# huyhoang17/DB_text_minimal

Measured on AMD Instinct MI355X. Metric: train images/sec @640x640 bs=16/GPU, higher is better.
Workload: dtype f32

## Files before the change

### db_text_minimal_amd/_lib.py

```python
import ctypes
import os
import subprocess

_HERE = os.path.dirname(os.path.abspath(__file__))
LIB_PATH = os.environ.get('DBN_LIB_PATH') or os.path.join(_HERE, 'libdbnet_hip.so')
CSRC = os.path.join(_HERE, 'csrc')

_P, _I, _L, _F, _D = ctypes.c_void_p, ctypes.c_int, ctypes.c_long, ctypes.c_float, ctypes.c_double

SIGNATURES = {
    'dbn_pack_weights': 'piiiiiipp',
    'dbn_igemm_panel_floats': 'iiiiii',
    'dbn_igemm_packed_floats': 'ii',
    'dbn_igemm_f32': 'pppp' + 'i' * 14 + 'p',
    'dbn_igemm_tile_config': 'ii',
    'dbn_igemm_tile_config_ns': 'iii',
    'dbn_conv_bn_ws_floats': 'iiiiii',
    'dbn_pack_weights_batched': 'piip',
    'dbn_igemm_splitk_plan': 'iiii',
    'dbn_igemm_splitk_plan_ns': 'iiiii',
    'dbn_igemm_splitk_f32': 'pppp' + 'i' * 16 + 'pp',
    'dbn_deform_im2col': 'ppp' + 'i' * 11 + 'p',
    'dbn_deform_col2im': 'ppppp' + 'i' + 'p' + 'i' * 11 + 'p',
    'dbn_deform_col2im_ws_bytes': 'i' * 8,
# ... 17 lines not shown
    'dbn_render_minmax': 'ppilplliifpp',
    'dbn_render_paint': 'ppppilplliifppfp',
    'dbn_minmax_scale_u8': 'piiippp',
    'dbn_words_to_input': 'ipllii' + 'ppp',
    'dbn_greedy_decode_ws_bytes': 'ii',
    'dbn_greedy_decode': 'ip' + 'iii' + 'pi' + 'ppppp',
    'dbn_jpeg_info': 'plp',
    'dbn_jpeg_coef_elems': 'ppip',
    'dbn_jpeg_entropy_batch': 'ppiplpppi',
    'dbn_jpeg_pixels': 'plppipipipplp',
    'dbn_jpeg_info_ex': 'plip',
    'dbn_jpeg_coef_elems_ex': 'ppiip',
    'dbn_jpeg_entropy_batch_ex': 'ppiplppppii',
    'dbn_jpeg_pixels_ex': 'plppipipippipplp',
    'dbn_jpeg_forward': 'plppipipipplp',
    'dbn_jpeg_encode_bound': 'piip',
    'dbn_jpeg_encode_batch': 'plppiiplpppi',
    'dbn_jpeg_optimal_table': 'pppp',
    'dbn_jpeg_encode_batch_opt': 'plppiiplpppii',
    'dbn_jpeg_huff_plan': 'ppilipppp',
    'dbn_jpeg_huff_hist': 'plpiplippp',
    'dbn_jpeg_huff_annex_k': 'pp',
    'dbn_jpeg_huff_tables': 'ppipppi',
    'dbn_jpeg_huff_code': 'plpippllipiplplpp',
    'dbn_jpeg_huff_headers': 'ppiipippp',
    'dbn_jpeg_stream_plan': 'ppipppppplpplp',
    'dbn_jpeg_dhuff_ws_bytes': 'l',
    'dbn_jpeg_dhuff': 'plppppppilliiplplpp',
    'dbn_detect_poly_ws_bytes': 'iiii',
    'dbn_detect_poly_verts_cap': 'iii',
    'dbn_detect_poly': 'piiiifi' + 'pppppp',
    'dbn_detect_poly_host': 'ppppp' + 'iiii' + 'pp' + 'pppi' + 'pppp',
    'dbn_det_eval_ws_bytes': 'i',
    'dbn_det_eval_overlaps': 'ppipilippppp',
    'dbn_det_eval_match_host': 'ii' + 'p' * 12,
    'dbn_pyramid_conv_ws_floats': 'iiii',
    'dbn_pyramid_conv_f32': 'p' * 10 + 'i' * 7 + 'pp' + 'ff' + 'ppppppp' + 'p',
    'dbn_conv_bn_f32': 'pppp' + 'i' * 15 + 'pp' + 'ff' + 'ppppppp' + 'p',
    'dbn_pack_weights_bf16s': 'piiiiiiipp',
    'dbn_igemm_bf16s_panel_floats': 'iiiiiii',
    'dbn_igemm_bf16s': 'pppp' + 'i' * 15 + 'p',
    'dbn_wgrad_bf16s': 'pppp' + 'i' * 12 + 'fip',
    'dbn_wgrad_splitk': 'iiiiiii',
    'dbn_wgrad_slab_floats': 'iiiiiii',
    'dbn_wgrad_splitk_hw': 'iiiiiiiii',
    'dbn_wgrad_slab_floats_hw': 'iiiiiiiiii',
    'dbn_set_index_limits': 'lll',
    'dbn_wgrad_f32': 'pppp' + 'i' * 12 + 'fp',
    'dbn_reduce_ws_floats': 'i',
    'dbn_bn_train_stats': 'piippffppppppp' + 'p',
    'dbn_bn_eval_coef': 'ippppfppp',
    'dbn_bn_apply': 'pppppppliip',
    'dbn_bn_backward': 'pppppppp' + 'pp' + 'i' + 'pp' + 'ii' + 'f' + 'pp',
    'dbn_bn_backward_from_sums': 'ppppppppp' + 'pp' + 'i' + 'pp' + 'ii' + 'f' + 'pp',
    'dbn_bn_backward_ex': 'ppppppppp' + 'pp' + 'i' + 'ppp' + 'ii' + 'f' + 'pp',
    'dbn_col_sum': 'piipfpp',
    'dbn_bnrelu_maxpool_fwd': 'ppppiiiip',
    'dbn_bnrelu_maxpool_bwd': 'ppppppiiiip',
    'dbn_nearest_up_fwd': 'ppp' + 'i' * 8 + 'p',
    'dbn_nearest_up_bwd': 'pp' + 'i' * 9 + 'p',
    'dbn_bilinear_fwd': 'ppliiiip',
    'dbn_bilinear_bwd': 'ppliiiip',
    'dbn_fpn_combine_weights': 'piiiipp',
    'dbn_fpn_scatter_wgrad': 'ppppiipp',
    'dbn_nchw3_to_nhwc4': 'ppiiip',
    'dbn_add_inplace': 'pplp',
    'dbn_head_tail_fwd': 'p' * 11 + 'iiii' + 'f' + 'p',
    'dbn_head_tail_bwd_ws_floats': '',
    'dbn_head_tail_bwd': 'p' * 21 + 'iiii' + 'ff' + 'pp',
    'dbn_db_loss_ws_bytes': '',
    'dbn_db_loss_fwd': 'pp' + 'iiii' + 'ffdf' + 'pppp',
    'dbn_db_loss_sum_fwd': 'pp' + 'iiii' + 'ffdf' + 'pppp',
    'dbn_db_loss_frac_fwd': 'pp' + 'iiii' + 'ffdf' + 'i' + 'pppp',
    'dbn_db_loss_bwd': 'pppp' + 'ff' + 'iiii' + 'pp',
    'dbn_db_loss_ohem_ws_bytes': 'iii',
    'dbn_db_loss_ohem_fwd': 'pp' + 'iiii' + 'ffdf' + 'pppp',
    'dbn_db_loss_ohem_bwd': 'ppppp' + 'ff' + 'iiii' + 'pp',
    'dbn_pixel_confusion': 'plppiiifpp',
    'dbn_adam_step': 'pppp' + 'l' + 'ffff' + 'i' + 'f' + 'p',
    'dbn_clock_probe': 'pip',
    'dbn_has_experiments': '',
    'dbn_wall_clock_khz': '',
}
SIGNATURES.update({
    'dbn_igemm_t': 'ii' + 'pppp' + 'i' * 14 + 'i' + 'p' + 'p',
    'dbn_conv_bn_t': 'i' + SIGNATURES['dbn_conv_bn_f32'],
    'dbn_pyramid_conv_t': 'i' + SIGNATURES['dbn_pyramid_conv_f32'],
    'dbn_pyramid_conv_from_t': 'ii' + SIGNATURES['dbn_pyramid_conv_f32'],
    'dbn_igemm_bn_rows': 'i' * 15,
    'dbn_igemm_bnsums_t': 'ii' + 'pppp' + 'i' * 14 + 'ppppppp' + 'pppp' + 'p' + 'p',
    'dbn_igemm_bn_final_counters': 'ii',
    'dbn_igemm_bn_final_group_floats': 'ii',
    'dbn_wgrad_t': 'ii' + 'pppp' + 'i' * 12 + 'f' + 'p',
    'dbn_wgrad_phase_t': 'iii' + 'pppp' + 'i' * 12 + 'f' + 'p',
    'dbn_wgrad_reduce_describe': 'ii' + 'pppp' + 'i' * 12 + 'f' + 'p',
    'dbn_wgrad_reduce_many': 'ppiiip',
    'dbn_wgrad_tile_config': 'ii',
    'dbn_set_wgrad_variant': 'i',
    'dbn_set_convt_kernel': 'i',
    'dbn_igemm_splitk_slab_floats': 'iiiii',
    'dbn_wgrad_kernel_config': 'iiiii',
    'dbn_wgrad_kernel_config_hw': 'i' * 12,
    'dbn_set_patch_conv': 'i',
    'dbn_set_wres16': 'i',
    'dbn_set_pyramid_wide': 'i',
    'dbn_pyramid_wide_would_run': 'iiiiii',
    'dbn_conv_bn_set_final': 'pp',
    'dbn_conv_bn_final_group_doubles': 'ii',
    'dbn_wres16_would_run': 'iiiiiiiii',
    'dbn_mfma_sustained': 'ippip',
    'dbn_mfma_sustained_flops': 'ii',
    'dbn_set_stagger': 'i',
    'dbn_winograd_eligible': 'iiiii',
    'dbn_winograd_panel_floats': 'ii',
    'dbn_winograd_pack': 'piiiipp',
    'dbn_winograd_rows': 'iii',
    'dbn_winograd_pack_batched': 'pip',
    'dbn_winograd_dgrad_bnsums_f32': 'ppp' + 'iiiiii' + 'pppp' + 'ppp' + 'pppp' + 'p' + 'p',
    'dbn_winograd_ws_floats': 'iiii',
    'dbn_winograd_wgrad_eligible': 'iiiiii',
    'dbn_winograd_wgrad_linear': 'ii',
    'dbn_winograd_wgrad_slab_floats': 'iiiii',
    'dbn_winograd_wgrad_f32': 'ipppppp' + 'iiiiii' + 'fp',
    'dbn_winograd_conv_bn_act_f32': 'pppppp' + 'iiiii' + 'pp' + 'ff' + 'ppppppp' + 'p',
    'dbn_winograd_conv_bn_f32': 'pppp' + 'iiiii' + 'pp' + 'ff' + 'ppppppp' + 'p',
    'dbn_set_phase_priority': 'i',
    'dbn_set_winograd_persistent': 'i',
    'dbn_set_winograd_stagger': 'i',
    'dbn_set_winograd_blocks_per_barrier': 'i',
    'dbn_fold_bn_eval': 'pilppppp' + 'f' + 'ppp',
    'dbn_igemm_act_t': 'ii' + 'pppp' + 'i' + 'p' + 'i' * 13 + 'p',
    'dbn_winograd_conv_act_f32': 'pppp' + 'i' + 'p' + 'iiiii' + 'p',
    'dbn_pyramid_conv_act_t': 'ii' + 'p' * 9 + 'i' + 'p' + 'i' * 6 + 'p',
    'dbn_set_trace': 'pl',
    'dbn_igemm_kernel_config': 'i' * 16,
    'dbn_split3': 'pplp',
    'dbn_deform_im2col_t': 'i' + SIGNATURES['dbn_deform_im2col'],
    'dbn_deform_col2im_t': 'i' + SIGNATURES['dbn_deform_col2im'],
    'dbn_deform_col2im_gather_t': 'i' + SIGNATURES['dbn_deform_col2im'],
    'dbn_deform_col2im_gather_ws_bytes': 'iii',
    'dbn_deform_offset_absmax_t': 'iplpp',
    'dbn_pw16_eligible': 'iiiiii',
    'dbn_pw16_panel_bytes': '',
    'dbn_pw16_pack': 'ipipp',
    'dbn_pw16_act_t': 'ipppipiiiip',
    'dbn_set_head_tail_wide': 'i',
    'dbn_stem16_pool_eligible': 'iiii',
    'dbn_stem16_conv_bn_relu_pool_t': 'ipppppiiip',
    'dbn_head16_eligible': 'iiii',
    'dbn_head16_tail_eval_t': 'i' + 'p' * 15 + 'iii' + 'p',
    'dbn_cast_f32': 'ipplp',
    'dbn_pack_weights_t': 'ip' + 'i' * 7 + 'pp',
    'dbn_igemm_panel_floats_t': 'i' * 8,
    'dbn_bn_train_stats_t': 'i' + SIGNATURES['dbn_bn_train_stats'],
    'dbn_bn_apply_t': 'i' + SIGNATURES['dbn_bn_apply'],
    'dbn_bn_backward_t': 'ipi' + SIGNATURES['dbn_bn_backward_ex'][1:],
    'dbn_col_sum_t': 'i' + SIGNATURES['dbn_col_sum'],
    'dbn_bnrelu_maxpool_fwd_t': 'i' + SIGNATURES['dbn_bnrelu_maxpool_fwd'],
    'dbn_bnrelu_maxpool_bwd_t': 'i' + SIGNATURES['dbn_bnrelu_maxpool_bwd'][:-1] + 'pppp',
    'dbn_maxpool_bwd_parts': 'iiii',
    'dbn_bnrelu_maxpool_fwd_arg_t': 'ipppppp' + 'iiii' + 'p',
    'dbn_maxpool_bn_backward_ws_floats': 'iiii',
    'dbn_maxpool_bn_backward_t': 'i' + 'p' * 10 + 'iiii' + 'f' + 'pp',
    'dbn_nearest_up_fwd_t': 'i' + SIGNATURES['dbn_nearest_up_fwd'],
    'dbn_nearest_up_bwd_t': 'i' + SIGNATURES['dbn_nearest_up_bwd'],
    'dbn_nchw3_to_nhwc4_t': 'i' + SIGNATURES['dbn_nchw3_to_nhwc4'],
    'dbn_nchw3_to_nhwc4_packed_t': 'i' + SIGNATURES['dbn_nchw3_to_nhwc4'],
    'dbn_nchw3_to_nhwc16_and_4_t': 'ipppiiip',
    'dbn_convt16_rows': '',
    'dbn_convt16_panel_bytes': '',
    'dbn_convt16_eligible': 'iiiiii',
    'dbn_convt16_pack': 'ippp',
    'dbn_convt16_bn_t': 'ippppiii' + 'pp' + 'ff' + 'ppppppp' + 'p',
    'dbn_stem16_padded_h': 'i',
    'dbn_stem16_padded_w': 'i',
    'dbn_stem16_rows': '',
    'dbn_stem16_panel_bytes': '',
    'dbn_stem16_eligible': 'iiii',
    'dbn_stem16_pack': 'ippp',
    'dbn_nchw3_to_padded4_t': 'ipppiiip',
    'dbn_stem16_conv_bn_t': 'ipppiii' + 'pp' + 'ff' + 'ppppppp' + 'p',
    'dbn_head_tail_fwd_t': 'i' + SIGNATURES['dbn_head_tail_fwd'],
    'dbn_head_tail_bwd_t': 'i' + SIGNATURES['dbn_head_tail_bwd'],
    'dbn_head_tail_bn_bwd_ws_floats': '',
    'dbn_head_tail_bn_bwd_t': 'ii' + 'p' * 28 + 'iiii' + 'ff' + 'pp',
})
LONG_RETURN = {'dbn_jpeg_coef_elems', 'dbn_jpeg_coef_elems_ex', 'dbn_jpeg_dhuff_ws_bytes', 'dbn_jpeg_encode_bound', 'dbn_greedy_decode_ws_bytes', 'dbn_det_eval_ws_bytes', 'dbn_detect_ws_bytes', 'dbn_detect_poly_ws_bytes', 'dbn_detect_poly_verts_cap', 'dbn_mfma_sustained_flops', 'dbn_conv_bn_final_group_doubles', 'dbn_maxpool_bn_backward_ws_floats', 'dbn_pw16_panel_bytes', 'dbn_stem16_panel_bytes', 'dbn_convt16_panel_bytes', 'dbn_winograd_panel_floats', 'dbn_winograd_wgrad_slab_floats', 'dbn_winograd_ws_floats', 'dbn_igemm_splitk_slab_floats', 'dbn_deform_col2im_ws_bytes', 'dbn_deform_col2im_gather_ws_bytes', 'dbn_igemm_bn_final_counters', 'dbn_igemm_bn_final_group_floats', 'dbn_igemm_panel_floats_t', 'dbn_wgrad_slab_floats_hw', 'dbn_wgrad_slab_floats', 'dbn_igemm_panel_floats', 'dbn_igemm_bf16s_panel_floats', 'dbn_db_loss_ohem_ws_bytes', 'dbn_conv_bn_ws_floats', 'dbn_pyramid_conv_ws_floats'}
_KIND = {'p': _P, 'i': _I, 'l': _L, 'f': _F, 'd': _D}


class HipLibraryError(RuntimeError):
    pass


class WgradReduceJob(ctypes.Structure):
    _fields_ = ([('slab', _P), ('grad', _P)] + [(f, _I) for f in ('splitk', 'O', 'J', 'Jp', 'BM', 'BN', 'Cb', 'I', 'RS', 'G', 'natural', 'blocks')]
                + [('scale', _F), ('smem_bytes', _I)])


class PackJob(ctypes.Structure):
    _fields_ = [('w', _P), ('out', _P)] + [(f, _I) for f in ('O', 'I', 'R', 'S', 'mode', 'Cs', 'Cd', 'f')]


class WinogradPackJob(ctypes.Structure):
    _fields_ = [('w', _P), ('out', _P)] + [(f, _I) for f in ('O', 'I', 'Cs', 'dgrad')]


class BnbFinal(ctypes.Structure):
    _fields_ = [('counters', _P), ('group', _P), ('c1c2', _P), ('dgamma', _P), ('dbeta', _P), ('c1c2_2', _P), ('dgamma_2', _P),
                ('dbeta_2', _P), ('grad_scale', _F)]


def build(verbose=False):
    res = subprocess.run(['make', '-C', CSRC, '-j8'], capture_output=True, text=True)
    if verbose or res.returncode != 0:
        print(res.stdout[-4000:])
        print(res.stderr[-4000:])
    if res.returncode != 0:
        raise HipLibraryError('building libdbnet_hip.so failed (see output above)')
    return LIB_PATH


def source_stamp():
    import hashlib
    h = hashlib.sha256()
    for name in sorted(os.listdir(CSRC)):
        if name.endswith(('.hip', '.h')) or name == 'Makefile':
            h.update(name.encode())
            with open(os.path.join(CSRC, name), 'rb') as f:
                h.update(f.read())
    return h.hexdigest()[:16]


_lib = None


def lib():
    global _lib
    if _lib is None:
        if not os.path.exists(LIB_PATH):
            raise HipLibraryError('%s not found: run `python -c "import __graft_entry__ as g; g.build()"` '
                                  '(there is no CPU fallback for the DBNet hot path)' % LIB_PATH)
        try:
            l = ctypes.CDLL(LIB_PATH)
        except OSError as e:
            raise HipLibraryError('cannot load %s: %s' % (LIB_PATH, e))
        for name, sig in SIGNATURES.items():
            fn = getattr(l, name)
            fn.argtypes = [_KIND[k] for k in sig]
            fn.restype = _L if name in LONG_RETURN else _I
        _lib = l
    return _lib


def check(rc, what=''):
    if rc != 0:
        if rc == 1:
            raise RuntimeError('libdbnet_hip: invalid argument in %s' % what)
        raise RuntimeError('libdbnet_hip: %s failed with hipError %d' % (what, rc - 1000))
```

### db_text_minimal_amd/csrc/conv.hip

```cpp
#include "igemm_common.h"
#include "../../include/dbnet_hip.h"

long dbn_g_pixel_limit = 1L << 24;
long dbn_g_byte_limit = 0xF0000000L;
long dbn_g_elem_limit = 1L << 32;

namespace {

__device__ __forceinline__ double block_sum_d(double v, double* red) {
    v = dbn_wave_sum_d(v);
    __syncthreads();
    if ((threadIdx.x & 63) == 0) red[threadIdx.x >> 6] = v;
    __syncthreads();
    double t = 0.0;
    for (int w = 0; w < (int)(blockDim.x >> 6); ++w) t += red[w];
    return t;
}

__global__ void bn_finalize_tiles_kernel(const float* __restrict__ stats, int rows, int C, const float* __restrict__ gamma,
                                         const float* __restrict__ beta, float eps, float momentum, float* __restrict__ run_mean,
                                         float* __restrict__ run_var, float* __restrict__ scale, float* __restrict__ shift,
                                         float* __restrict__ mean_out, float* __restrict__ rstd_out) {
    __shared__ double red[16];
    const int c = blockIdx.x;
// ... 68 lines not shown
int dbn_has_experiments(void) { return DBN_HAS_EXPERIMENTS; }


static int tile_config_for(int M, int Cd, int ns) {
    const int bm[4] = {128, 256, 128, 64}, bn[4] = {128, 64, 64, 64};
    static const int r2_env = dbn_env_int("DBN_TILE_EFF_R2", 1);
    const int r2_eff = ns == 0 ? r2_env : 0;
    const double eff_r1[4] = {0.89, 0.83, 0.80, 0.72}, eff_r2[4] = {0.89, 0.85, 0.845, 0.83}, eff_r3[4] = {0.80, 0.76, 0.86, 0.93};
    const double* eff = r2_eff == 2 ? eff_r3 : r2_eff ? eff_r2 : eff_r1;
    int best = 4;
    double best_t = 1e300;
    for (int c = 0; c < 4; ++c) {
        if (Cd % bn[c]) continue;
        const long blocks = (long)dbn_ceil_div(M, bm[c]) * (Cd / bn[c]);
        const long per_cu = (blocks + 255) / 256;
        double t = (double)per_cu * bm[c] * bn[c] / eff[c];
        if (blocks < 512) t *= 1.0 + 0.25 * (512 - blocks) / 512.0;
        if (t < best_t) {
            best_t = t;
            best = c + 1;
        }
    }
    return best;
}
int dbn_igemm_tile_config(int M, int Cd) { return tile_config_for(M, Cd, 0); }
int dbn_igemm_tile_config_ns(int M, int Cd, int ns) { return tile_config_for(M, Cd, ns); }

static int g_convt_enabled = 1;
int dbn_set_convt_kernel(int on) {
    const int old = g_convt_enabled;
    g_convt_enabled = on != 0;
    return old;
}
static bool convt_eligible(int mode, int ns, int at, int tile_hint, int R, int S, int stride, int pad, int Hs, int Ws, int Hd, int Wd, int Cs,
                           int Cd, int accumulate, int ksplit) {
    return g_convt_enabled && mode == 1 && ns == 0 && at == 0 && tile_hint == 0 && R == 2 && S == 2 && stride == 2 && pad == 0 && Hd == 2 * Hs &&
           Wd == 2 * Ws && (Cs == 16 || Cs == 32 || Cs == 48 || Cs == 64) && Cd % 64 == 0 && !accumulate && ksplit <= 1;
}

static bool convt_launch_ok(int n, int Hd, int Wd, int Cd) { return (long)n * Hd * Wd * Cd * 4 < (1L << 32); }

unsigned long long* dbn_g_trace = nullptr;
long dbn_g_trace_blocks = 0;
int dbn_set_trace(void* buf, long max_blocks) {
    dbn_g_trace = reinterpret_cast<unsigned long long*>(buf);
    dbn_g_trace_blocks = max_blocks;
    return DBN_TRACE;
}
int dbn_g_phase_prio = 0;
int dbn_set_phase_priority(int on) {
    const int old = dbn_g_phase_prio;
    dbn_g_phase_prio = on != 0;
    return old;
}
int dbn_g_stagger = 0;
int dbn_set_stagger(int permille) {
    const int old = dbn_g_stagger;
    dbn_g_stagger = permille < 0 ? 0 : permille;
    return old;
}

static bool patch_eligible_fwd(int mode, int at, int H, int W, int Cs);
int dbn_g_wres16 = getenv("DBN_WRES16") ? atoi(getenv("DBN_WRES16")) : 1;
int dbn_set_wres16(int on) {
    const int old = dbn_g_wres16;
    dbn_g_wres16 = on < 0 ? 0 : on > 2 ? 2 : on;
    return old;
}
int dbn_wres16_would_run(int at, int mode, int N, int H, int W, int Cs, int Cd, int bnb, int y2) {
    return patch_eligible_fwd(mode, at, H, W, Cs) && Cd % 64 == 0 && dbn_wres16_eligible(at, mode, N, H, W, Cs, Cd, bnb != 0, y2 != 0, false);
}
static int g_patch_enabled = 1;
static const int g_patch_bn64 = dbn_env_int("DBN_PATCH_BN64", 1);
int dbn_set_patch_conv(int on) {
    const int old = g_patch_enabled;
    g_patch_enabled = (on == 2 || on == 3) ? on : (on != 0);
    return old;
}
static bool patch_eligible(int kmode, int ns, int at, int cfg, int R, int S, int stride, int pad, int Hs, int Ws, int Hd, int Wd, int Cs,
                           int ksplit, int tile_hint = 0) {
    const bool geom = (kmode == 0 || kmode == 1) && R == 3 && S == 3 && stride == 1 && pad == 1 && Hs == Hd && Ws == Wd && Hd % 8 == 0 &&
                      Wd % 16 == 0 && Cs % 32 == 0 && ksplit <= 1;
    if (ns == 0) return (g_patch_enabled == 1 || g_patch_enabled == 3) && at == 0 && geom && (tile_hint == 3 || (tile_hint == 0 && g_patch_enabled == 3));
    return g_patch_enabled && ns > 0 && at != 3 && (cfg == 1 || cfg == 3) && geom;
}
static bool patch_eligible_fwd(int mode, int at, int H, int W, int Cs) {
    return patch_eligible(mode, 1, at, 3, 3, 3, 1, 1, H, W, H, W, Cs, 1, 0);
}
static int patch_cfg(int cfg, int ns = 1) { return (ns == 0 || (cfg == 1 && g_patch_bn64)) ? 3 : cfg; }

static int resolve_cfg(int M_total, int Cd, int tile_hint, int at = 0, int ns = 0, int mode = 0, int R = 0, int S = 0, int stride = 1,
                       int pad = 0, int Hs = 0, int Ws = 0, int Hd = 0, int Wd = 0, int Cs = 0, int ksplit = 1) {
    int cfg = tile_hint > 0 ? tile_hint : tile_config_for(M_total, Cd, ns);
    if (cfg == 1 && Cd % 128 != 0) cfg = 3;
    if (tile_hint == 0 && !(mode == 1 && stride > 1) && Cd % 64 == 0 && patch_eligible(mode, ns, at, 3, R, S, stride, pad, Hs, Ws, Hd, Wd, Cs, ksplit))
        cfg = 3;
    return cfg;
}

int dbn_igemm_kernel_config(int at, int ns, int kmode, int N, int Hs, int Ws, int Cs, int Hd, int Wd, int Cd, int R, int S, int stride,
                            int pad, int tile_hint, int ksplit) {
    const int cfg = resolve_cfg(N * Hd * Wd, Cd, tile_hint, at, ns, kmode >= 2 ? 1 : kmode, R, S, kmode == 2 && stride == 1 ? 2 : stride, pad, Hs,
                                Ws, Hd, Wd, Cs, ksplit);
    if (Cd % 64 == 0 && patch_eligible(kmode, ns, at, cfg, R, S, stride, pad, Hs, Ws, Hd, Wd, Cs, ksplit, tile_hint)) {
        const int wres = (ns == 1 && patch_cfg(cfg, ns) == 3 && dbn_wres16_eligible(at, kmode, N, Hd, Wd, Cs, Cd, false, false, false)) ? 64 : 0;
        return patch_cfg(cfg, ns) + 16 + wres;
    }
    if (kmode == 2 && convt_eligible(1, ns, at, tile_hint, R, S, stride, pad, Hs, Ws, Hd, Wd, Cs, Cd, 0, ksplit)) return cfg + 32;
    return cfg;
}

static int igemm_dispatch(IgemmParams& p, int kmode, int ns, int tile_hint, hipStream_t st, int at = 0) {
    int cfg = tile_hint > 0 ? tile_hint : tile_config_for(p.N * p.Hdf * p.Wdf, p.Cd, ns);
    if (cfg == 1 && p.Cd % 128 != 0) cfg = 3;
    p.patch = p.Cd % 64 == 0 && patch_eligible(kmode, ns, at, cfg, p.R, p.S, p.stride, p.pad, p.Hs, p.Ws, p.Hdf, p.Wdf, p.Cs, p.ksplit, tile_hint);
    if (p.patch) cfg = patch_cfg(cfg, ns);
    return launch_igemm(p, cfg, kmode, ns, st, at);
}

static inline int dst_esize(int at) { return (at == 0 || at == 3) ? 4 : 2; }
static inline int src_planes(int at) { return at == 3 ? 3 : 1; }

struct BnFin {
    int* cnt;
    double* grp;
    const float *gamma, *beta;
    float eps, momentum;
    float *run_mean, *run_var, *scale, *shift, *mean, *rstd;
};
static thread_local int* g_bnf_cnt = nullptr;
static thread_local double* g_bnf_grp = nullptr;
int dbn_conv_bn_set_final(int* counters, double* group) {
    g_bnf_cnt = counters;
    g_bnf_grp = counters ? group : nullptr;
    return (counters && !group) ? DBN_ERR_ARG : DBN_OK;
}
long dbn_conv_bn_final_group_doubles(int rows, int Cd) { return 4L * Cd * ((rows + 63) / 64); }

struct IgemmBnb {
    const void *y, *zmask;
    const float *msc, *msh, *mean, *rstd;
    float* part;
    const void* y2;
    const float *mean2, *rstd2;
    float* part2;
    const dbn_bnb_final* fin;
    int M_total;
};

static int igemm_run_one(const void* src, const float* wpk, const float* bias, void* dst, int N, int Hs, int Ws, int Cs, int Hd,
                         int Wd, int Cd, int R, int S, int stride, int pad, int mode, int accumulate, int cfg, int ns,
                         hipStream_t st, float* stats, int stat_rows, int stat_row0, int ksplit, float* slab, int* rows_out, int at,
                         long plane_bytes, const IgemmBnb* bnb = nullptr, int tile_hint = -1, const void* res = nullptr, int relu = 0,
                         const BnFin* bnf = nullptr) {
    IgemmParams p{};
    if (bnf) {
        p.bnf_cnt = bnf->cnt; p.bnf_grp = bnf->grp; p.bnf_gamma = bnf->gamma; p.bnf_beta = bnf->beta; p.bnf_eps = bnf->eps;
        p.bnf_momentum = bnf->momentum; p.bnf_run_mean = bnf->run_mean; p.bnf_run_var = bnf->run_var; p.bnf_scale = bnf->scale;
        p.bnf_shift = bnf->shift; p.bnf_mean = bnf->mean; p.bnf_rstd = bnf->rstd;
    }
    p.res = res; p.relu = relu;
    p.bnb_y = bnb ? bnb->y : nullptr; p.bnb_zmask = bnb ? bnb->zmask : nullptr;
    p.bnb_msc = bnb ? bnb->msc : nullptr; p.bnb_msh = bnb ? bnb->msh : nullptr;
    p.bnb_mean = bnb ? bnb->mean : nullptr; p.bnb_rstd = bnb ? bnb->rstd : nullptr;
    p.bnb_part = bnb ? bnb->part : nullptr;
    p.bnb_y2 = bnb ? bnb->y2 : nullptr; p.bnb_mean2 = bnb ? bnb->mean2 : nullptr; p.bnb_rstd2 = bnb ? bnb->rstd2 : nullptr;
    p.bnb_part2 = bnb ? bnb->part2 : nullptr;
    p.bnb_cnt = nullptr; p.bnb_grp = nullptr; p.bnb_gscale = 1.f; p.bnb_invM = 0.f;
    for (int b_ = 0; b_ < 2; ++b_) p.bnb_c1c2[b_] = p.bnb_dgamma[b_] = p.bnb_dbeta[b_] = nullptr;
    if (bnb && bnb->fin) {
        const dbn_bnb_final* f = bnb->fin;
        p.bnb_cnt = f->counters; p.bnb_grp = f->group; p.bnb_gscale = f->grad_scale; p.bnb_invM = 1.0f / (float)bnb->M_total;
        p.bnb_c1c2[0] = f->c1c2; p.bnb_dgamma[0] = f->dgamma; p.bnb_dbeta[0] = f->dbeta;
        p.bnb_c1c2[1] = f->c1c2_2; p.bnb_dgamma[1] = f->dgamma_2; p.bnb_dbeta[1] = f->dbeta_2;
    }
    p.src = src; p.wpk = wpk; p.bias = bias; p.dst = dst;
    p.N = N; p.Hs = Hs; p.Ws = Ws; p.Cs = Cs; p.Cd = Cd; p.Hdf = Hd; p.Wdf = Wd;
    p.R = R; p.S = S; p.stride = stride; p.pad = pad; p.accumulate = res ? 1 : accumulate;
    p.stats = stats; p.stat_rows = stat_rows; p.stat_row0 = stat_row0; p.launch_rows = 0;
    p.ksplit = 1; p.kt_per = 0;
    p.plane_bytes = (unsigned)plane_bytes;
    p.src_bytes = (unsigned)((long)N * Hs * Ws * Cs * dbn_esize(at) + (src_planes(at) - 1) * plane_bytes);
    if (!(mode == 1 && stride > 1)) {
        p.ncls = 1;
        if (ksplit <= 1) {
            const int rc = igemm_dispatch(p, mode, ns, cfg, st, at);
            *rows_out = p.launch_rows;
            return rc;
        }
        const int KT = (R * S * Cs + 15) / 16;
        DBN_REQUIRE(slab && !stats && !bnb && Cs % 16 == 0 && ksplit <= KT && ksplit <= 64);
        p.kt_per = dbn_ceil_div(KT, ksplit);
        p.ksplit = dbn_ceil_div(KT, p.kt_per);
        p.dst = slab; p.bias = nullptr; p.accumulate = 0;
        const int rc = igemm_dispatch(p, mode, ns, cfg, st, at);
        *rows_out = p.launch_rows;
        if (rc) return rc;
        const long total4 = (long)N * Hd * Wd * Cd / 4;
        DBN_DISPATCH_AT(at == 3 ? 0 : at, hipLaunchKernelGGL(splitk_sum_kernel<AT>, dim3(dbn_grid(total4)), dim3(256), 0, st, slab, p.ksplit,
                                                             total4, Cd, bias, accumulate, dst));
        return dbn_status();
    }
    DBN_REQUIRE(ksplit <= 1);
    p.ncls = stride * stride;
    long off = 0;
    int covered = 0;
    for (int c = 0; c < p.ncls; ++c) {
        const IgemmClass q = class_geom(c, stride, R, S, pad, N, Hd, Wd, Cs);
        p.wpk_off[c] = (int)off;
        if (q.K > 0 && q.M > 0) ++covered;
        off += panel_floats(q.K, Cd, ns);
    }
    DBN_REQUIRE(off < (1L << 31));
    DBN_REQUIRE(covered == p.ncls || !bias);
    DBN_REQUIRE(covered == p.ncls || !bnb);
    if (covered < p.ncls && !accumulate) {
        if (hipMemsetAsync(dst, 0, (size_t)N * Hd * Wd * Cd * dst_esize(at), st) != hipSuccess) return dbn_status();
        p.accumulate = 1;
    }
    *rows_out = 0;
    if (covered == 0) return DBN_OK;
    if (!bnb && convt_eligible(mode, ns, at, tile_hint, R, S, stride, pad, Hs, Ws, Hd, Wd, Cs, Cd, accumulate, ksplit) &&
        convt_launch_ok(N, Hd, Wd, Cd)) {
        const int rc = dbn_launch_convt_f32(p, st);
        *rows_out = p.launch_rows;
        return rc;
    }
    const int rc = igemm_dispatch(p, 2, ns, cfg, st, at);
    *rows_out = p.launch_rows;
    return rc;
}

static int bn_tile_rows_one(int n, int Hd, int Wd, int mode, int stride, int cfg) {
    const int bm_of[5] = {0, 128, 256, 128, 64};
    if (!(mode == 1 && stride > 1)) return dbn_ceil_div((long)n * Hd * Wd, bm_of[cfg]);
    int rows = 0;
    for (int c = 0; c < stride * stride; ++c) {
        const int ph = c / stride, pw = c % stride;
        const int Hc = ph < Hd ? (Hd - ph + stride - 1) / stride : 0, Wc = pw < Wd ? (Wd - pw + stride - 1) / stride : 0;
        if (Hc > 0 && Wc > 0) rows += dbn_ceil_div((long)n * Hc * Wc, bm_of[cfg]);
    }
    return rows;
}

static int igemm_run(const void* src, const float* wpk, const float* bias, void* dst, int N, int Hs, int Ws, int Cs, int Hd,
                     int Wd, int Cd, int R, int S, int stride, int pad, int mode, int accumulate, int tile_hint, int ns,
                     void* stream, float* stats = nullptr, int ksplit = 1, float* slab = nullptr, int stat_rows_total = 0, int at = 0,
                     const IgemmBnb* bnb = nullptr, const void* res = nullptr, int relu = 0, const BnFin* bnf = nullptr) {
    DBN_REQUIRE((!res && !relu) || (ksplit <= 1 && !stats && !bnb && !(mode == 1 && stride > 1)));
    DBN_REQUIRE(src && wpk && dst && (ns == 0 || ns == 1 || ns == 3));
    DBN_REQUIRE(at == 0 || ((at == 1 || at == 2) && ns == 1 && Cs % 16 == 0) || (at == 3 && ns == 3 && Cs % 16 == 0));
    DBN_REQUIRE(N > 0 && Hs > 0 && Ws > 0 && Hd > 0 && Wd > 0 && R > 0 && S > 0 && pad >= 0);
    DBN_REQUIRE(Cs % 4 == 0 && Cd % 64 == 0 && (mode == 0 || mode == 1));
    DBN_REQUIRE(stride == 1 || stride == 2 || stride == 4 || stride == 8 || (mode == 0 && stride >= 1));
    DBN_REQUIRE(tile_hint >= 0 && tile_hint <= 4);
    hipStream_t st = (hipStream_t)stream;
    const int es = dbn_esize(at), des = dst_esize(at);
    const long plane_bytes = at == 3 ? (long)N * Hs * Ws * Cs * 2 : 0;
    DBN_REQUIRE(3 * plane_bytes < dbn_g_byte_limit);
    const int nmax = chunk_images(N, (long)Hd * Wd, (long)Hs * Ws * Cs * es, (long)Hd * Wd * Cd);
    DBN_REQUIRE(nmax >= 1);
    DBN_REQUIRE(nmax >= N || ksplit <= 1);
    const int cfg = resolve_cfg((int)std::min<long>((long)N * Hd * Wd, 0x7FFFFFFF), Cd, tile_hint, at, ns, mode, R, S, stride, pad, Hs, Ws,
                                Hd, Wd, Cs, ksplit);
    int row0 = 0;
    for (int n0 = 0; n0 < N; n0 += nmax) {
        const int n = std::min(nmax, N - n0);
        int rows = 0;
        IgemmBnb b;
        if (bnb) {
            b = *bnb;
            b.y = reinterpret_cast<const char*>(bnb->y) + (long)n0 * Hd * Wd * Cd * des;
            if (bnb->zmask) b.zmask = reinterpret_cast<const char*>(bnb->zmask) + (long)n0 * Hd * Wd * Cd * des;
            if (bnb->y2) b.y2 = reinterpret_cast<const char*>(bnb->y2) + (long)n0 * Hd * Wd * Cd * des;
        }
        const int rc = igemm_run_one(reinterpret_cast<const char*>(src) + (long)n0 * Hs * Ws * Cs * es, wpk, bias,
                                     reinterpret_cast<char*>(dst) + (long)n0 * Hd * Wd * Cd * des, n, Hs, Ws, Cs, Hd, Wd, Cd, R, S, stride,
                                     pad, mode, accumulate, cfg, ns, st, stats, stat_rows_total, row0, ksplit, slab, &rows, at, plane_bytes,
                                     bnb ? &b : nullptr, tile_hint,
                                     res ? reinterpret_cast<const char*>(res) + (long)n0 * Hd * Wd * Cd * des : nullptr, relu, bnf);
        if (rc) return rc;
        row0 += rows;
    }
    return DBN_OK;
}

int dbn_igemm_t(int at, int ns, const void* src, const float* wpk, const float* bias, void* dst, int N, int Hs, int Ws, int Cs, int Hd,
                int Wd, int Cd, int R, int S, int stride, int pad, int mode, int accumulate, int tile_hint, int ksplit, float* slab,
                void* stream) {
    return igemm_run(src, wpk, bias, dst, N, Hs, Ws, Cs, Hd, Wd, Cd, R, S, stride, pad, mode, accumulate, tile_hint, ns, stream, nullptr,
                     ksplit < 1 ? 1 : ksplit, slab, 0, at);
}

int dbn_igemm_act_t(int at, int ns, const void* src, const float* wpk, const float* bias, const void* res, int relu, void* dst, int N,
                    int Hs, int Ws, int Cs, int Hd, int Wd, int Cd, int R, int S, int stride, int pad, int mode, int tile_hint,
                    void* stream) {
    return igemm_run(src, wpk, bias, dst, N, Hs, Ws, Cs, Hd, Wd, Cd, R, S, stride, pad, mode, 0, tile_hint, ns, stream, nullptr, 1, nullptr, 0,
                     at, nullptr, res, relu ? 1 : 0);
}

int dbn_igemm_f32(const float* src, const float* wpk, const float* bias, float* dst, int N, int Hs, int Ws, int Cs, int Hd,
                  int Wd, int Cd, int R, int S, int stride, int pad, int mode, int accumulate, int tile_hint, void* stream) {
    return igemm_run(src, wpk, bias, dst, N, Hs, Ws, Cs, Hd, Wd, Cd, R, S, stride, pad, mode, accumulate, tile_hint, 0, stream);
}

static int bn_tile_rows(int N, int Hs, int Ws, int Cs, int Hd, int Wd, int Cd, int mode, int stride, int tile_hint, int at, int ns, int R,
                        int S, int pad, bool conv_bn = false, int accumulate = 0) {
    const int nmax = chunk_images(N, (long)Hd * Wd, (long)Hs * Ws * Cs * dbn_esize(at), (long)Hd * Wd * Cd);
    if (nmax < 1) return 0;
    const bool convt = conv_bn && convt_eligible(mode, ns, at, tile_hint, R, S, stride, pad, Hs, Ws, Hd, Wd, Cs, Cd, accumulate, 1);
    const int cfg = resolve_cfg((int)std::min<long>((long)N * Hd * Wd, 0x7FFFFFFF), Cd, tile_hint, at, ns, mode, R, S, stride, pad, Hs, Ws,
                                Hd, Wd, Cs, 1);
    int rows = 0;
    for (int n0 = 0; n0 < N; n0 += nmax) {
        const int n = std::min(nmax, N - n0);
        rows += (convt && convt_launch_ok(n, Hd, Wd, Cd)) ? dbn_convt_f32_rows(n * Hs * Ws) : bn_tile_rows_one(n, Hd, Wd, mode, stride, cfg);
    }
    return rows;
}

int dbn_igemm_bn_rows(int at, int ns, int N, int Hs, int Ws, int Cs, int Hd, int Wd, int Cd, int R, int S, int stride, int pad, int mode,
                      int tile_hint) {
    return bn_tile_rows(N, Hs, Ws, Cs, Hd, Wd, Cd, mode, stride, tile_hint, at, ns, R, S, pad);
}

int dbn_igemm_bnsums_t(int at, int ns, const void* src, const float* wpk, const float* bias, void* dst, int N, int Hs, int Ws, int Cs, int Hd,
                       int Wd, int Cd, int R, int S, int stride, int pad, int mode, int accumulate, int tile_hint, const void* y,
                       const void* zmask, const float* mask_scale, const float* mask_shift, const float* save_mean,
                       const float* save_rstd, float* part, const void* y2, const float* save_mean2, const float* save_rstd2,
                       float* part2, const dbn_bnb_final* fin, void* stream) {
    DBN_REQUIRE(((at == 0 && (ns == 0 || ns == 1 || ns == 3)) || (at == 1 && ns == 1)) && y && save_mean && save_rstd && part &&
                (zmask || (mask_scale && mask_shift)));
    DBN_REQUIRE(!y2 || (zmask && save_mean2 && save_rstd2 && part2));
    DBN_REQUIRE(!fin || (fin->counters && fin->group && fin->c1c2 && fin->dgamma && fin->dbeta &&
                         (!y2 || (fin->c1c2_2 && fin->dgamma_2 && fin->dbeta_2))));
    const int rows = bn_tile_rows(N, Hs, Ws, Cs, Hd, Wd, Cd, mode, stride, tile_hint, at, ns, R, S, pad);
    DBN_REQUIRE(rows > 0);
    const IgemmBnb b{y, zmask, mask_scale, mask_shift, save_mean, save_rstd, part, y2, save_mean2, save_rstd2, part2, fin, N * Hd * Wd};
    return igemm_run(src, wpk, bias, dst, N, Hs, Ws, Cs, Hd, Wd, Cd, R, S, stride, pad, mode, accumulate, tile_hint, ns, stream, nullptr, 1,
                     nullptr, rows, at, &b);
}

long dbn_igemm_bn_final_counters(int rows, int Cd) { return (long)(Cd / 64) * ((rows + 63) / 64 + 1); }
long dbn_igemm_bn_final_group_floats(int rows, int Cd) { return 4L * Cd * ((rows + 63) / 64); }

long dbn_conv_bn_ws_floats(int N, int Hd, int Wd, int Cd, int mode, int stride) {
    long worst = 0;
    for (int t = 1; t <= 4; ++t) {
        const long r = (long)N * bn_tile_rows_one(1, Hd, Wd, mode, stride, t);
        worst = r > worst ? r : worst;
    }
    return (3L * Cd + 1) * worst;
}

int dbn_conv_bn_t(int at, const void* src, const float* wpk, const float* bias, void* dst, int N, int Hs, int Ws, int Cs, int Hd, int Wd,
                  int Cd, int R, int S, int stride, int pad, int mode, int accumulate, int tile_hint, int ns,
                  const float* gamma, const float* beta, float eps, float momentum, float* run_mean, float* run_var,
                  float* scale, float* shift, float* save_mean, float* save_rstd, float* ws, void* stream) {
    DBN_REQUIRE(gamma && beta && scale && shift && save_mean && save_rstd && ws);
    const int rows = bn_tile_rows(N, Hs, Ws, Cs, Hd, Wd, Cd, mode, stride, tile_hint, at, ns, R, S, pad, true, accumulate);
    DBN_REQUIRE(rows > 0);
    int* const fcnt = g_bnf_cnt;
    double* const fgrp = g_bnf_grp;
    g_bnf_cnt = nullptr;
    g_bnf_grp = nullptr;
    const bool fin = fcnt && !convt_eligible(mode, ns, at, tile_hint, R, S, stride, pad, Hs, Ws, Hd, Wd, Cs, Cd, accumulate, 1);
    const BnFin f{fcnt, fgrp, gamma, beta, eps, momentum, run_mean, run_var, scale, shift, save_mean, save_rstd};
    const int rc = igemm_run(src, wpk, bias, dst, N, Hs, Ws, Cs, Hd, Wd, Cd, R, S, stride, pad, mode, accumulate, tile_hint, ns, stream, ws,
                             1, nullptr, rows, at, nullptr, nullptr, 0, fin ? &f : nullptr);
    if (rc || fin) return rc;
    hipLaunchKernelGGL(bn_finalize_tiles_kernel, dim3(Cd), dim3(rows >= 2048 ? 1024 : 256), 0, (hipStream_t)stream, ws, rows, Cd, gamma,
                       beta, eps, momentum, run_mean, run_var, scale, shift, save_mean, save_rstd);
    return dbn_status();
}

int dbn_winograd_eligible(int N, int H, int W, int Cs, int Cd) {
    if (!(N > 0 && H > 0 && W > 0 && Cs > 0 && Cs % 16 == 0 && Cd > 0 && Cd % 64 == 0)) return 0;
    const long Hp = (H + 7) / 8 * 8, Wp = (W + 15) / 16 * 16;
    const long tiles = (long)((H + 1) / 2) * ((W + 1) / 2);
    const bool pays = dbn_winograd_linear(H, W) ? 5 * tiles >= 3 * ((tiles + 31) / 32 * 32) : 4L * H * W >= 3L * Hp * Wp;
    return pays && (long)N * H * W * std::max(Cs, Cd) * 4 < dbn_g_byte_limit && (long)N * Hp * Wp < dbn_g_pixel_limit;
}
long dbn_winograd_panel_floats(int O, int Cs) { return (long)Cs * 16 * O; }
int dbn_winograd_pack(const float* w_oihw, int O, int I, int Cs, int dgrad, float* out, void* stream) {
    DBN_REQUIRE(w_oihw && out && O > 0 && I > 0 && I <= Cs && Cs % 16 == 0 && O % 64 == 0 && (dgrad == 0 || dgrad == 1));
    return dbn_launch_winograd_pack(w_oihw, O, I, Cs, dgrad, out, (hipStream_t)stream);
}
int dbn_winograd_pack_batched(const void* jobs, int n, void* stream) {
    DBN_REQUIRE(jobs && n > 0);
    return dbn_launch_winograd_pack_many(jobs, n, (hipStream_t)stream);
}
long dbn_winograd_ws_floats(int N, int H, int W, int Cd) { return (3L * Cd + 1) * dbn_winograd_rows(N, H, W); }
int dbn_winograd_conv_bn_act_f32(const float* src, const float* in_scale, const float* in_shift, const float* upanel, const float* bias,
                                 float* dst, int N, int H, int W, int Cs, int Cd, const float* gamma, const float* beta, float eps,
                                 float momentum, float* run_mean, float* run_var, float* scale, float* shift, float* save_mean,
                                 float* save_rstd, float* ws, void* stream) {
    DBN_REQUIRE(src && upanel && dst && dbn_winograd_eligible(N, H, W, Cs, Cd) && !in_scale == !in_shift);
    DBN_REQUIRE(!gamma || (beta && scale && shift && save_mean && save_rstd && ws));
    IgemmParams p{};
    p.in_scale = in_scale; p.in_shift = in_shift;
    p.src = src; p.wpk = upanel; p.bias = bias; p.dst = dst;
    p.N = N; p.Hs = H; p.Ws = W; p.Cs = Cs; p.Cd = Cd; p.Hdf = H; p.Wdf = W; p.R = 3; p.S = 3; p.stride = 1; p.pad = 1;
    p.src_bytes = (unsigned)((long)N * H * W * Cs * 4);
    const int rows = dbn_winograd_rows(N, H, W);
    p.stats = gamma ? ws : nullptr; p.stat_rows = rows; p.stat_row0 = 0;
    int* const fcnt = g_bnf_cnt;
    double* const fgrp = g_bnf_grp;
    g_bnf_cnt = nullptr;
    g_bnf_grp = nullptr;
    const bool fin = gamma && fcnt;
    if (fin) {
        p.bnf_cnt = fcnt; p.bnf_grp = fgrp; p.bnf_gamma = gamma; p.bnf_beta = beta; p.bnf_eps = eps; p.bnf_momentum = momentum;
        p.bnf_run_mean = run_mean; p.bnf_run_var = run_var; p.bnf_scale = scale; p.bnf_shift = shift; p.bnf_mean = save_mean; p.bnf_rstd = save_rstd;
    }
    const int rc = dbn_launch_winograd_f32(p, (hipStream_t)stream);
    if (rc || !gamma || fin) return rc;
    hipLaunchKernelGGL(bn_finalize_tiles_kernel, dim3(Cd), dim3(rows >= 2048 ? 1024 : 256), 0, (hipStream_t)stream, ws, rows, Cd, gamma,
                       beta, eps, momentum, run_mean, run_var, scale, shift, save_mean, save_rstd);
    return dbn_status();
}

int dbn_winograd_conv_act_f32(const float* src, const float* upanel, const float* bias, const float* res, int relu, float* dst, int N,
                              int H, int W, int Cs, int Cd, void* stream) {
    DBN_REQUIRE(src && upanel && dst && dbn_winograd_eligible(N, H, W, Cs, Cd));
    IgemmParams p{};
    p.src = src; p.wpk = upanel; p.bias = bias; p.dst = dst; p.res = res; p.relu = relu ? 1 : 0; p.accumulate = res ? 1 : 0;
    p.N = N; p.Hs = H; p.Ws = W; p.Cs = Cs; p.Cd = Cd; p.Hdf = H; p.Wdf = W; p.R = 3; p.S = 3; p.stride = 1; p.pad = 1;
    p.src_bytes = (unsigned)((long)N * H * W * Cs * 4);
    p.stat_rows = dbn_winograd_rows(N, H, W);
    return dbn_launch_winograd_f32(p, (hipStream_t)stream);
}

int dbn_winograd_conv_bn_f32(const float* src, const float* upanel, const float* bias, float* dst, int N, int H, int W, int Cs, int Cd,
// ... 196 lines not shown
```

### db_text_minimal_amd/csrc/igemm_common.h

```cpp
#pragma once
#include "common.h"
#include <type_traits>
#include <utility>
#include <stdlib.h>
#include <algorithm>

struct IgemmClass {
    int Hd, Wd;
    int M, K, KT;
    int R, S;
    int pad_h, pad_w;
    int oh0, ow0;
};

constexpr int MAX_CLASSES = 64;

__host__ __device__ inline int taps_of_class(int R, int ph, int f) { return ph < R ? (R - ph + f - 1) / f : 0; }

__host__ __device__ inline IgemmClass class_geom(int c, int f, int R, int S, int pad, int N, int Hdf, int Wdf, int Cs) {
    IgemmClass q;
    const int ph = c / f, pw = c - ph * f;
    q.R = taps_of_class(R, ph, f);
    q.S = taps_of_class(S, pw, f);
    q.oh0 = (((ph - pad) % f) + f) % f;
    q.ow0 = (((pw - pad) % f) + f) % f;
    q.Hd = q.oh0 < Hdf ? (Hdf - q.oh0 + f - 1) / f : 0;
    q.Wd = q.ow0 < Wdf ? (Wdf - q.ow0 + f - 1) / f : 0;
    q.pad_h = (q.oh0 + pad - ph) / f;
    q.pad_w = (q.ow0 + pad - pw) / f;
    q.M = N * q.Hd * q.Wd;
    q.K = q.R * q.S * Cs;
    q.KT = (q.K + 15) / 16;
    return q;
}

struct IgemmParams {
    const void* src;
    const float* wpk;
    const float* bias;
    void* dst;
    int N, Hs, Ws, Cs, Cd, Hdf, Wdf, R, S, stride, pad, accumulate, ncls;
    const float *in_scale, *in_shift;
    const void* res;
    int relu;
    int work_items;
    int* work;
    unsigned long long wino_m_ntn, wino_m_tpi, wino_m_tw;
    int wino_tpi, wino_tw;
    int stat_rows;
    int stat_row0;
    float* stats;
    const void* bnb_y;
    const void* bnb_zmask;
    const float *bnb_msc, *bnb_msh, *bnb_mean, *bnb_rstd;
    float* bnb_part;
    const void* bnb_y2;
    const float *bnb_mean2, *bnb_rstd2;
    float* bnb_part2;
    int* bnb_cnt;
    float* bnb_grp;
    float *bnb_c1c2[2], *bnb_dgamma[2], *bnb_dbeta[2];
    float bnb_gscale, bnb_invM;
    int* bnf_cnt;
    double* bnf_grp;
    const float *bnf_gamma, *bnf_beta;
    float bnf_eps, bnf_momentum;
    float *bnf_run_mean, *bnf_run_var, *bnf_scale, *bnf_shift, *bnf_mean, *bnf_rstd;
    unsigned src_bytes;
    unsigned plane_bytes;
    int tile_end[MAX_CLASSES], row_base[MAX_CLASSES], wpk_off[MAX_CLASSES];
    int ksplit, kt_per;
    int stagger_units, stagger_blocks;
    int phase_prio;
    unsigned long long* trace;
    int launch_rows;
    int patch;
    const void* seg_src[4];
    const float* seg_wpk[4];
    unsigned seg_bytes[4];
    unsigned seg_plane_bytes[4];
    int first_level;
    int pyr_group;
};

extern "C" int dbn_g_stagger;
extern "C" int dbn_g_phase_prio;
extern "C" unsigned long long* dbn_g_trace;
extern "C" long dbn_g_trace_blocks;
#ifndef DBN_TRACE
#define DBN_TRACE 0
#endif
#if DBN_TRACE
#define DBN_TRACE_MARK(i)                                                                                      \
    do {                                                                                                       \
        if (p.trace && threadIdx.x == 0) p.trace[(long)blockIdx.x * 8 + (i)] = __builtin_amdgcn_s_memrealtime(); \
    } while (0)
#else
#define DBN_TRACE_MARK(i) ((void)0)
#endif

namespace {

constexpr unsigned OOB_OFFSET = 0xF8000000u;

__device__ __forceinline__ f32x4 buffer_load_f32x4(__amdgpu_buffer_rsrc_t rsrc, unsigned byte_off) {
    typedef unsigned u32x4 __attribute__((ext_vector_type(4)));
    const u32x4 v = __builtin_amdgcn_raw_buffer_load_b128(rsrc, (int)byte_off, 0, 0);
    return __builtin_bit_cast(f32x4, v);
}

__device__ __forceinline__ void divmod24(int p, int d, float rd, int& q, int& r) {
    q = (int)((float)p * rd);
    r = p - q * d;
    if (r < 0) {
        r += d;
        --q;
    } else if (r >= d) {
        r -= d;
        ++q;
    }
}


typedef __bf16 bf16x8 __attribute__((ext_vector_type(8)));
typedef unsigned u32x2 __attribute__((ext_vector_type(2)));

__device__ __forceinline__ unsigned bf16_bits_rne(float x) {
    unsigned u = __builtin_bit_cast(unsigned, x);
    u += 0x7FFFu + ((u >> 16) & 1u);
    return u >> 16;
}
__device__ __forceinline__ float bf16_bits_to_f32(unsigned b) { return __builtin_bit_cast(float, b << 16); }

typedef __bf16 bf16x2 __attribute__((ext_vector_type(2)));
template <int NS>
__device__ __forceinline__ void split4(const f32x4 v, u32x2 (&out)[NS > 0 ? NS : 1]) {
    float r[4] = {v[0], v[1], v[2], v[3]};
#pragma unroll
    for (int s = 0; s < NS; ++s) {
        const bf16x2 lo = {(__bf16)r[0], (__bf16)r[1]};
        const bf16x2 hi = {(__bf16)r[2], (__bf16)r[3]};
        const unsigned ulo = __builtin_bit_cast(unsigned, lo), uhi = __builtin_bit_cast(unsigned, hi);
        out[s] = u32x2{ulo, uhi};
        if (s + 1 < NS) {
            r[0] -= __builtin_bit_cast(float, ulo << 16);
            r[1] -= __builtin_bit_cast(float, ulo & 0xFFFF0000u);
            r[2] -= __builtin_bit_cast(float, uhi << 16);
            r[3] -= __builtin_bit_cast(float, uhi & 0xFFFF0000u);
        }
    }
}

typedef _Float16 f16x8 __attribute__((ext_vector_type(8)));
template <int NS, int MI, int NI, int F16 = 0>
__device__ __forceinline__ void mfma_split(const bf16x8 (&af)[NS > 0 ? NS : 1][MI], const bf16x8 (&bf)[NS > 0 ? NS : 1][NI],
                                           f32x16 (&acc)[MI][NI]) {
    if constexpr (F16) {
#pragma unroll
        for (int a = 0; a < MI; ++a)
#pragma unroll
            for (int b = 0; b < NI; ++b)
                acc[a][b] = __builtin_amdgcn_mfma_f32_32x32x16_f16(__builtin_bit_cast(f16x8, af[0][a]), __builtin_bit_cast(f16x8, bf[0][b]),
                                                                   acc[a][b], 0, 0, 0);
        return;
    }
    constexpr int NPROD = NS == 3 ? 6 : 1;
    constexpr int pi[6] = {2, 0, 1, 1, 0, 0};
    constexpr int pj[6] = {0, 2, 1, 0, 1, 0};
#pragma unroll
    for (int t = 0; t < NPROD; ++t) {
        const int i = NS == 3 ? pi[t] : 0, j = NS == 3 ? pj[t] : 0;
#pragma unroll
        for (int a = 0; a < MI; ++a)
#pragma unroll
            for (int b = 0; b < NI; ++b) acc[a][b] = __builtin_amdgcn_mfma_f32_32x32x16_bf16(af[i][a], bf[j][b], acc[a][b], 0, 0, 0);
    }
}

struct BnStatFinal {
    float* stats;
    int stat_rows, Cd;
    int* bnf_cnt;
    double* bnf_grp;
    const float *bnf_gamma, *bnf_beta;
    float bnf_eps, bnf_momentum;
    float *bnf_run_mean, *bnf_run_var, *bnf_scale, *bnf_shift, *bnf_mean, *bnf_rstd;
};
#define DBN_BNF_ARGS(p)                                                                                                              \
    BnStatFinal {                                                                                                                    \
        (p).stats, (p).stat_rows, (p).Cd, (p).bnf_cnt, (p).bnf_grp, (p).bnf_gamma, (p).bnf_beta, (p).bnf_eps, (p).bnf_momentum,        \
            (p).bnf_run_mean, (p).bnf_run_var, (p).bnf_scale, (p).bnf_shift, (p).bnf_mean, (p).bnf_rstd                                \
    }
__device__ __forceinline__ void dbn_stat_put(bool fin, float* ptr, float v) {
    if (fin) __hip_atomic_store(ptr, v, __ATOMIC_RELAXED, __HIP_MEMORY_SCOPE_AGENT);
    else *ptr = v;
}
__device__ __forceinline__ void dbn_bn_stats_finish(const BnStatFinal p, int trow, int nt, int n0, int BN, int* s_flag, double* sd) {
    if (!p.bnf_cnt) return;
    constexpr int G = 64;
    const int rows = p.stat_rows, NG = (rows + G - 1) / G, g = trow / G;
    const int tid = threadIdx.x, NT = blockDim.x, parts = NT / BN;
    const int cl = tid % BN, part = tid / BN;
    const long c = n0 + cl;
    int* const cnt = p.bnf_cnt + nt * (NG + 1);
    auto xld = [](const float* q) { return (double)__hip_atomic_load(q, __ATOMIC_RELAXED, __HIP_MEMORY_SCOPE_AGENT); };
    auto xldd = [](const double* q) { return __hip_atomic_load(q, __ATOMIC_RELAXED, __HIP_MEMORY_SCOPE_AGENT); };
    auto xstd = [](double* q, double v) { __hip_atomic_store(q, v, __ATOMIC_RELAXED, __HIP_MEMORY_SCOPE_AGENT); };
    auto combine = [&](double& n, double& a1, double& a2) {
        __syncthreads();
        sd[tid] = n;
        sd[NT + tid] = a1;
        sd[2 * NT + tid] = a2;
        __syncthreads();
        if (part == 0)
            for (int q = 1; q < parts; ++q) {
                n += sd[q * BN + cl];
                a1 += sd[NT + q * BN + cl];
                a2 += sd[2 * NT + q * BN + cl];
            }
    };
    asm volatile("s_waitcnt vmcnt(0)" ::: "memory");
    __syncthreads();
    DBN_RACE_JITTER();
    if (tid == 0) {
        const int gsize = min(G, rows - g * G);
        const int last = __hip_atomic_fetch_add(cnt + 1 + g, 1, __ATOMIC_RELAXED, __HIP_MEMORY_SCOPE_AGENT) == gsize - 1;
        if (last) __hip_atomic_store(cnt + 1 + g, 0, __ATOMIC_RELAXED, __HIP_MEMORY_SCOPE_AGENT);
        *s_flag = last;
    }
// ... 135 lines not shown
```

### db_text_minimal_amd/csrc/igemm_kernel.h

```cpp
#pragma once
#include "igemm_common.h"

#ifndef DBN_DBG
#define DBN_DBG 0
#endif

namespace {

#define DBN_IGEMM_OCC(BM, BN, NS, MODE, PATCH, EPI, AT) \
    __attribute__((amdgpu_waves_per_eu(((MODE) == 3 && (BN) == 256) ? 2 : ((PATCH) && (NS) == 3 && (BN) == 64) ? 2 : ((EPI) == 1 && (NS) == 0 && (BM) * (BN) == 16384) ? 3 : \
                                       ((EPI) == 1 && (AT) == 1 && (PATCH) && (BN) == 64) ? 4 : \
                                       ((EPI) == 0 && (NS) == 0 && (AT) == 0 && (BM) * (BN) == 4096 && (MODE) < 2) ? 7 : 1, 8)))

template <int BM, int BN, int WM, int WN, int MODE, int NS, int AT = 0, bool PATCH = false, int EPI = 0, bool BLK = true>
__global__ __launch_bounds__(WM* WN * 64) DBN_IGEMM_OCC(BM, BN, NS, MODE, PATCH, EPI, AT) void igemm_f32_kernel(const IgemmParams p) {
    static_assert(EPI == 0 || ((AT == 0 || AT == 1) && MODE < 3), "BatchNorm-backward sums: fp32 or bf16 storage, no pyramid form");
    static_assert(BLK || (AT == 0 && MODE == 0 && !PATCH && EPI == 0), "non-blocked K walk: forward conv on fp32 tensors");
    static_assert(AT == 0 || ((AT == 1 || AT == 2) && NS == 1) || (AT == 3 && NS == 3), "storage type / matrix math combination");
    static_assert(!PATCH || (BM == 128 && WM == 2 && WN == 2 && MODE < 2 && (NS > 0 || AT == 0) && AT != 3), "patch form");
    constexpr int NT = WM * WN * 64;
    constexpr int TM = BM / WM, TN = BN / WN;
    constexpr int MI = TM / 32, NI = TN / 32;
    constexpr int ES = AT == 0 ? 4 : 2;
    constexpr bool DST_F32 = AT == 0 || AT == 3;
#ifndef DBN_BUFST
#define DBN_BUFST 1
#endif
    constexpr bool BUFST = DBN_BUFST && DST_F32 && MODE < 2;
    constexpr int NP = AT == 3 ? 3 : 1;
    constexpr int A_SH = AT == 0 ? 2 : 1;
    constexpr int A_CH = AT == 0 ? 4 : 8;
    constexpr int A_PIECES = (BM << A_SH) * NP;
    constexpr int A_LD = (A_PIECES + NT - 1) / NT;
    constexpr bool A_FULL = A_PIECES % NT == 0;
    constexpr int AS = NS == 0 ? BM + 2 : BM + 4, BS = NS == 0 ? BN + 2 : BN + 4;
    constexpr int A_IMG = NS == 0 ? 4 * AS : NS * 2 * AS, B_IMG = NS == 0 ? 4 * BS : NS * 2 * BS;
    constexpr int B_PIECES = NS == 0 ? 4 * BN : NS * 2 * BN;
    constexpr int B_LD = (B_PIECES + NT - 1) / NT;
    constexpr bool B_FULL = B_PIECES % NT == 0;
    constexpr int KU = 1;
#ifndef DBN_DIRECTB
#define DBN_DIRECTB 1
#endif
#ifndef DBN_DIRECTB_NS
#define DBN_DIRECTB_NS 1
#endif
    constexpr bool DIRECTB = DBN_DIRECTB && (NS == 0 || DBN_DIRECTB_NS) && AT == 0 && !PATCH;
    constexpr int NF = NS == 0 ? 2 : NS;
    constexpr int UNIT = A_IMG + (DIRECTB ? 0 : B_IMG);
    constexpr int STAGE = KU * UNIT;
    constexpr int NSX = NS > 0 ? NS : 1;
    static_assert(A_LD >= 1 && B_LD >= 1, "tile too small for the workgroup");
    constexpr int DMA_SU = 2;
#ifndef DBN_DBG16
#define DBN_DBG16 0
#endif
#ifndef DBN_DIRECTB16
#define DBN_DIRECTB16 1
#endif
#ifndef DBN_DIRECTB16_PYR
#define DBN_DIRECTB16_PYR 1
#endif
    constexpr bool DB16 = DBN_DIRECTB16 && AT != 0 && AT != 3 && (MODE != 3 || DBN_DIRECTB16_PYR) && !PATCH;
    constexpr int DMA_UNIT = NP * 2 * BM + (DB16 ? 0 : NSX * 2 * BN);
    constexpr int DMA_STAGE = DMA_SU * DMA_UNIT;
#ifndef DBN_PYR_NSTG
#define DBN_PYR_NSTG 4
#endif
#ifndef DBN_PYR_NSTG_WIDE
#define DBN_PYR_NSTG_WIDE 4
#endif
    constexpr int DMA_NSTG = (DB16 && MODE == 3 && BN == 256 && DMA_STAGE * 16 * DBN_PYR_NSTG_WIDE <= 64 * 1024) ? DBN_PYR_NSTG_WIDE :
                             (DB16 && MODE == 3 && DMA_STAGE * 16 * DBN_PYR_NSTG <= 48 * 1024) ? DBN_PYR_NSTG :
                             DMA_STAGE * 16 * 4 <= 64 * 1024 ? 4 : DMA_STAGE * 16 * 3 <= 160 * 1024 ? 3 : 2;
    constexpr int P_PATCH = NSX * 4 * 180;
    constexpr int P_BUNIT = NSX * 2 * BN, P_BSTAGE = 2 * P_BUNIT;
#ifndef DBN_P_NSTG
#define DBN_P_NSTG 4
#endif
    constexpr int P_NSTG = NSX == 1 ? DBN_P_NSTG : 3;
    constexpr int P_NBUF = NSX == 1 ? 2 : 1;
#ifndef DBN_DIRECTBP
#define DBN_DIRECTBP 1
#endif
#ifndef DBN_DBP_NS1
#define DBN_DBP_NS1 0
#endif
    constexpr bool DBP = DBN_DIRECTBP && PATCH && (NS == 3 || (DBN_DBP_NS1 && NS == 1));
    constexpr int LOOP_SMEM = PATCH ? P_NBUF * P_PATCH + ((DBP || NS == 0) ? 0 : P_NSTG * P_BSTAGE) : AT != 0 ? DMA_NSTG * DMA_STAGE : 2 * STAGE;
    constexpr int EPI_SMEM = (EPI == 1 && DST_F32) ? BM * BN / (4 * (MI >= 2 ? 2 : 1)) : 0;
    constexpr int OUT_SMEM = DST_F32 ? 0 : (BM * (BN + 8) * 2 + 15) / 16;
    constexpr int SMEM_A = LOOP_SMEM > EPI_SMEM ? LOOP_SMEM : EPI_SMEM;
    constexpr int FIN_SMEM = (3 * NT * 8 + 15) / 16;
    constexpr int SMEM_B = SMEM_A > OUT_SMEM ? SMEM_A : OUT_SMEM;
    __shared__ f32x4 smem[(SMEM_B > FIN_SMEM ? SMEM_B : FIN_SMEM) + 1];

    const int tid = threadIdx.x;
    const int lane = tid & 63, wave = tid >> 6;
    const int wm = wave / WN, wn = wave % WN;
    const int li = lane & 31, lh = lane >> 5;

    if (p.phase_prio) __builtin_amdgcn_s_setprio(3);
    DBN_TRACE_MARK(0);
#if DBN_TRACE
    if (p.trace && threadIdx.x == 0) p.trace[(long)blockIdx.x * 8 + 7] = __builtin_amdgcn_s_getreg((31 << 11) | 4);
#endif
    if (p.stagger_units > 0 && (int)blockIdx.x < p.stagger_blocks) {
        const unsigned slot = __builtin_amdgcn_s_getreg((3 << 11) | (0 << 6) | 4) & 15u;
        const unsigned n = __builtin_amdgcn_readfirstlane(slot * (unsigned)p.stagger_units);
        for (unsigned i = 0; i < n; ++i) __builtin_amdgcn_s_sleep(16);
    }

    int tile = dbn_xcd_remap(blockIdx.x, gridDim.x);
    IgemmClass q;
    int q_row_base = 0, q_wpk_off = 0;
    if (MODE == 3) {
        q.Hd = p.Hdf >> 3; q.Wd = p.Wdf >> 3; q.M = p.N * q.Hd * q.Wd;
        const int mtiles = (q.M + BM - 1) / BM, ntn_ = p.Cd / BN;
        int mt_ = tile / (64 * ntn_), rem_ = tile - mt_ * (64 * ntn_);
        int c = rem_ / ntn_;
        if (p.pyr_group > 0) {
            const int G = p.pyr_group, per = G * 64 * ntn_;
            const int blk = tile / per, t = tile - blk * per;
            const int cr = t / (G * 8 * ntn_), t2 = t - cr * (G * 8 * ntn_);
            const int g = t2 / (8 * ntn_), t3 = t2 - g * (8 * ntn_);
            const int cc = t3 / ntn_;
            mt_ = blk * G + g;
            c = cr * 8 + cc;
            rem_ = c * ntn_ + (t3 - cc * ntn_);
            if (mt_ >= mtiles) return;
        }
        tile = mt_ * ntn_ + (rem_ - c * ntn_);
        q.oh0 = c >> 3; q.ow0 = c & 7;
        q_row_base = c * mtiles;
        q.R = q.S = q.K = q.KT = q.pad_h = q.pad_w = 0;
    } else if (MODE == 2) {
        const int slot = tile / p.ncls;
        const int c = (tile + (slot >> 3)) % p.ncls;
        tile = slot;
        if (tile >= p.tile_end[c]) return;
        q = class_geom(c, p.stride, p.R, p.S, p.pad, p.N, p.Hdf, p.Wdf, p.Cs);
        q_row_base = p.row_base[c];
        q_wpk_off = p.wpk_off[c];
    } else {
        q.Hd = p.Hdf; q.Wd = p.Wdf; q.M = p.N * p.Hdf * p.Wdf; q.R = p.R; q.S = p.S;
        q.K = p.R * p.S * p.Cs; q.KT = (q.K + 15) / 16;
        q.pad_h = q.pad_w = p.pad; q.oh0 = q.ow0 = 0;
    }
    const int ntn = p.Cd / BN;
    const int mt = tile / ntn, nt = tile - mt * ntn;
    const int m0 = mt * BM, n0 = nt * BN;
    const int qM = q.M, qHd = q.Hd, qWd = q.Wd;
    int pn = 0, ph0 = 0, pw0 = 0;
    if constexpr (PATCH) {
        const int tw = qWd >> 4, tpi = (qHd >> 3) * tw;
        pn = mt / tpi;
        const int t = mt - pn * tpi, ty = t / tw;
        ph0 = ty * 8;
        pw0 = (t - ty * tw) * 16;
    }
    int qK = q.K, qKT = q.KT, qS = q.S, qR = q.R;
    int gHs = p.Hs, gWs = p.Ws;

    __amdgpu_buffer_rsrc_t rsrc = __builtin_amdgcn_make_buffer_rsrc(const_cast<void*>(p.src), 0, p.src_bytes, 0x00020000);

    const int a_chunk = tid & ((1 << A_SH) - 1);
    auto a_row = [&](int j) { return AT == 0 ? (tid >> 2) + j * (NT / 4) : ((tid + j * NT) >> 1) % BM; };
    auto a_plane = [&](int j) { return AT == 0 ? 0 : ((tid + j * NT) >> 1) / BM; };
    auto a_on = [&](int j) { return A_FULL || tid + j * NT < A_PIECES; };
    int a_hb[A_LD], a_wb[A_LD], a_nb[A_LD];
    constexpr bool SOFF = BLK && AT == 0 && !PATCH;
    unsigned a_org[A_LD];
    unsigned a_pl[A_LD];
    unsigned plane_bytes = p.plane_bytes;
    int a_n[MODE == 3 ? A_LD : 1], a_hd[MODE == 3 ? A_LD : 1], a_wd[MODE == 3 ? A_LD : 1];
    const int HWd = qHd * qWd;
#pragma unroll
    for (int j = 0; j < A_LD; ++j) {
        const int row = a_row(j);
        const int m = m0 + row;
        const bool ok = m < qM && a_on(j);
        a_pl[j] = (unsigned)a_plane(j) * plane_bytes;
        const int mm = ok ? m : 0;
        int n, rem, hd, wd;
        divmod24(mm, HWd, 1.0f / (float)HWd, n, rem);
        divmod24(rem, qWd, 1.0f / (float)qWd, hd, wd);
        a_nb[j] = n * p.Hs * p.Ws * p.Cs;
        a_org[j] = 0;
        if (MODE == 3) {
            a_n[j] = n;
            a_hd[j] = ok ? hd : -(1 << 20);
            a_wd[j] = wd;
        } else if (MODE == 0) {
            a_hb[j] = ok ? hd * p.stride - q.pad_h : -(1 << 20);
            a_wb[j] = wd * p.stride - q.pad_w;
            if (SOFF) a_org[j] = (unsigned)(a_nb[j] + (hd * p.stride * p.Ws + wd * p.stride) * p.Cs + A_CH * a_chunk) * (unsigned)ES;
        } else {
            a_hb[j] = ok ? hd + q.pad_h : -(1 << 20);
            a_wb[j] = wd + q.pad_w;
            if (SOFF) a_org[j] = (unsigned)(a_nb[j] + ((hd + q.pad_h) * p.Ws + wd + q.pad_w) * p.Cs + A_CH * a_chunk) * (unsigned)ES;
        }
    }
    auto soff_rsrc = [&](const void* base, unsigned bytes, int Ws_, int R_, int S_, int padh, int padw) {
        const unsigned shift = (unsigned)((MODE == 0 ? padh * Ws_ + padw : (R_ - 1) * Ws_ + (S_ - 1)) * p.Cs) * (unsigned)ES;
        const unsigned margin = (unsigned)((padh * Ws_ + padw + 1) * p.Cs) * (unsigned)ES;
        return __builtin_amdgcn_make_buffer_rsrc(const_cast<char*>(reinterpret_cast<const char*>(base) - shift), 0, bytes + shift + margin,
                                                 0x00020000);
    };
    if (SOFF && MODE != 3) rsrc = soff_rsrc(p.src, p.src_bytes, p.Ws, q.R, q.S, q.pad_h, q.pad_w);
    constexpr bool blocked = BLK;
    int kidx = A_CH * a_chunk;
    int k_ci, k_r, k_s;
    int kt_begin = 0, kt_end = qKT;
    if (MODE < 2 && p.ksplit > 1) {
        kt_begin = blockIdx.y * p.kt_per;
        kt_end = min(qKT, kt_begin + p.kt_per);
    }
    int k_cb = 0;
    if (blocked) {
        const int rs = max(1, q.R * qS), cb = kt_begin / rs, tap = kt_begin - cb * rs;
        kidx += 16 * kt_begin;
        k_ci = 16 * cb + A_CH * a_chunk;
        k_cb = 16 * cb;
        k_r = tap / qS;
        k_s = tap - k_r * qS;
    } else {
        const int k_tap = kidx / p.Cs;
        k_ci = kidx - k_tap * p.Cs;
        k_r = k_tap / qS;
        k_s = k_tap - k_r * qS;
    }

    unsigned aoff[KU][A_LD];
    unsigned asoff[KU];
    int kend = (MODE < 2 && p.ksplit > 1) ? min(qK, 16 * kt_end) : qK;
    auto next_offsets = [&](int u = 0) {
        if constexpr (SOFF) {
            const int tr = MODE == 0 ? k_r : qR - 1 - k_r, ts = MODE == 0 ? k_s : qS - 1 - k_s;
            asoff[u] = (unsigned)((tr * gWs + ts) * p.Cs + k_cb) * (unsigned)ES;
            const bool kv = kidx - A_CH * a_chunk < kend;
#pragma unroll
            for (int j = 0; j < A_LD; ++j) {
                const int hs = MODE == 0 ? a_hb[j] + k_r : a_hb[j] - k_r;
                const int ws = MODE == 0 ? a_wb[j] + k_s : a_wb[j] - k_s;
                const bool v = kv && (unsigned)hs < (unsigned)gHs && (unsigned)ws < (unsigned)gWs;
                aoff[u][j] = v ? a_org[j] : OOB_OFFSET;
            }
        } else {
#pragma unroll
            for (int j = 0; j < A_LD; ++j) {
                const int hs = MODE == 0 ? a_hb[j] + k_r : a_hb[j] - k_r;
                const int ws = MODE == 0 ? a_wb[j] + k_s : a_wb[j] - k_s;
                const bool v = kidx < kend && (unsigned)hs < (unsigned)gHs && (unsigned)ws < (unsigned)gWs;
                const unsigned off = (unsigned)(a_nb[j] + (hs * gWs + ws) * p.Cs + k_ci) * (unsigned)ES + (AT == 3 ? a_pl[j] : 0u);
                aoff[u][j] = v ? off : OOB_OFFSET;
            }
            asoff[u] = 0;
        }
        kidx += 16;
        if (blocked) {
            ++k_s;
            const bool ws_ = k_s == qS;
            k_s = ws_ ? 0 : k_s;
            k_r += ws_ ? 1 : 0;
            const bool wr_ = k_r == qR;
            k_r = wr_ ? 0 : k_r;
            k_ci += wr_ ? 16 : 0;
            k_cb += wr_ ? 16 : 0;
        } else {
            k_ci += 16;
            while (k_ci >= p.Cs) {
                k_ci -= p.Cs;
                if (++k_s == qS) {
                    k_s = 0;
                    ++k_r;
                }
            }
        }
    };
    unsigned b_voff[B_LD];
    unsigned bf_voff[NF][NI];
    int b_lds[B_LD];
    bool b_on[B_LD];
    __amdgpu_buffer_rsrc_t rsrcB;
    int b_kt = 0, b_ktmax = 0;
    const unsigned b_step_bytes = (unsigned)((NS == 0 ? 4 : 2 * NS) * p.Cd) * 16u;
    auto panel_setup = [&](const float* panel, int ktiles) {
#pragma unroll
        for (int j = 0; j < B_LD; ++j) {
            const int idx = tid + j * NT;
            b_on[j] = B_FULL || idx < B_PIECES;
            const int c = b_on[j] ? idx / BN : 0, n = idx - (idx / BN) * BN;
            b_voff[j] = (unsigned)(c * p.Cd + n0 + n) * 16u;
            b_lds[j] = c * BS + n;
        }
#pragma unroll
        for (int s2 = 0; s2 < NF; ++s2)
#pragma unroll
            for (int b = 0; b < NI; ++b) bf_voff[s2][b] = (unsigned)((2 * s2 + lh) * p.Cd + n0 + wn * TN + b * 32 + li) * 16u;
        rsrcB = __builtin_amdgcn_make_buffer_rsrc(const_cast<float*>(panel), 0, (unsigned)ktiles * b_step_bytes, 0x00020000);
    };
    if (MODE != 3) {
        panel_setup(p.wpk + q_wpk_off, qKT);
        b_kt = kt_begin;
        b_ktmax = max(kt_end - 1, kt_begin);
    }
    auto level_setup = [&](int g) {
        const int f = 1 << g, kk = f + 2;
        const int oh0g = q.oh0 & (f - 1), ow0g = q.ow0 & (f - 1);
        const int ph = (oh0g + 1) & (f - 1), pw = (ow0g + 1) & (f - 1);
        qR = taps_of_class(kk, ph, f);
        qS = taps_of_class(kk, pw, f);
        const int padh = (oh0g + 1 - ph) >> g, padw = (ow0g + 1 - pw) >> g;
        qK = qR * qS * p.Cs;
        qKT = qK >> 4;
        gHs = p.Hdf >> g;
        gWs = p.Wdf >> g;
        rsrc = __builtin_amdgcn_make_buffer_rsrc(const_cast<void*>(p.seg_src[g]), 0, p.seg_bytes[g], 0x00020000);
        if (AT == 3) {
            plane_bytes = p.seg_plane_bytes[g];
#pragma unroll
            for (int j = 0; j < A_LD; ++j) a_pl[j] = (unsigned)a_plane(j) * plane_bytes;
        }
        long krows = 0;
        for (int d = 0; d < ph * f + pw; ++d) krows += taps_of_class(kk, d >> g, f) * taps_of_class(kk, d & (f - 1), f) * p.Cs;
        panel_setup(p.seg_wpk[g] + (NS == 0 ? krows * p.Cd : krows * p.Cd * NS / 2), qKT);
        b_kt = 0;
        b_ktmax = max(qKT - 1, 0);
#pragma unroll
        for (int j = 0; j < A_LD; ++j) {
            a_nb[j] = a_n[MODE == 3 ? j : 0] * gHs * gWs * p.Cs;
            a_hb[j] = a_hd[MODE == 3 ? j : 0] * (8 >> g) + (q.oh0 >> g) + padh;
            a_wb[j] = a_wd[MODE == 3 ? j : 0] * (8 >> g) + (q.ow0 >> g) + padw;
            const int hb_ = a_hd[MODE == 3 ? j : 0] < 0 ? 0 : a_hb[j];
            if (SOFF) a_org[j] = (unsigned)(a_nb[j] + (hb_ * gWs + a_wb[j]) * p.Cs + A_CH * a_chunk) * (unsigned)ES;
        }
        if (SOFF) rsrc = soff_rsrc(p.seg_src[g], p.seg_bytes[g], gWs, qR, qS, padh, padw);
        kidx = A_CH * a_chunk;
        k_ci = A_CH * a_chunk;
        k_cb = 0;
        k_r = k_s = 0;
    };

    f32x4 ra_[2][KU][A_LD], rb_[2][KU][B_LD];
    f32x4 rbf_[2][NF][NI];
    auto issue_b_frag = [&](auto SET) {
        constexpr int st_ = decltype(SET)::value;
        const unsigned bso = (unsigned)min(b_kt, b_ktmax) * b_step_bytes;
        ++b_kt;
#pragma unroll
        for (int s2 = 0; s2 < NF; ++s2)
#pragma unroll
            for (int b = 0; b < NI; ++b) {
                typedef unsigned u32x4_ __attribute__((ext_vector_type(4)));
                const u32x4_ v_ = __builtin_amdgcn_raw_buffer_load_b128(rsrcB, (int)bf_voff[s2][b], (int)bso, 0);
                rbf_[st_][s2][b] = __builtin_bit_cast(f32x4, v_);
            }
    };
    auto issue_loads = [&](auto SET) {
        constexpr int st_ = decltype(SET)::value;
#pragma unroll
        for (int u = 0; u < KU; ++u) {
#pragma unroll
            for (int j = 0; j < A_LD; ++j)
                if (!(DBN_DBG & 1)) {
                    typedef unsigned u32x4_ __attribute__((ext_vector_type(4)));
                    const u32x4_ v_ = __builtin_amdgcn_raw_buffer_load_b128(rsrc, (int)aoff[u][j], (int)asoff[u], 0);
                    ra_[st_][u][j] = __builtin_bit_cast(f32x4, v_);
                }
            if constexpr (DIRECTB) continue;
            const unsigned bso = (unsigned)min(b_kt, b_ktmax) * b_step_bytes;
            ++b_kt;
#pragma unroll
            for (int j = 0; j < B_LD; ++j)
                if (!(DBN_DBG & 2) && (B_FULL || b_on[j])) {
                    typedef unsigned u32x4_ __attribute__((ext_vector_type(4)));
                    const u32x4_ v_ = __builtin_amdgcn_raw_buffer_load_b128(rsrcB, (int)b_voff[j], (int)bso, 0);
                    rb_[st_][u][j] = __builtin_bit_cast(f32x4, v_);
                }
        }
    };
    auto stage_unit = [&](int buf, auto SET, auto UU) {
        constexpr int st_ = decltype(SET)::value;
        constexpr int u_ = decltype(UU)::value;
        f32x4 (&ra)[A_LD] = ra_[st_][u_];
        f32x4 (&rb)[B_LD] = rb_[st_][u_];
        f32x4* As = smem + buf * STAGE + u_ * UNIT;
        f32x4* Bs = As + A_IMG;
        if (DBN_DBG & 4) return;
        if constexpr (NS == 0) {
#pragma unroll
            for (int j = 0; j < A_LD; ++j) As[a_chunk * AS + (tid >> 2) + j * (NT / 4)] = ra[j];
        } else if constexpr (AT != 0) {
#pragma unroll
            for (int j = 0; j < A_LD; ++j)
                if (a_on(j)) As[(a_plane(j) * 2 + a_chunk) * AS + a_row(j)] = ra[j];
        } else {
#pragma unroll
            for (int j = 0; j < A_LD; ++j) {
                u32x2 sp[NSX];
                split4<NS>(ra[j], sp);
                const int row = (tid >> 2) + j * (NT / 4);
#pragma unroll
                for (int t = 0; t < NS; ++t)
                    reinterpret_cast<u32x2*>(As + (t * 2 + (a_chunk >> 1)) * AS + row)[a_chunk & 1] = sp[t];
            }
        }
        if constexpr (!DIRECTB) {
#pragma unroll
            for (int j = 0; j < B_LD; ++j)
                if (B_FULL || b_on[j]) Bs[b_lds[j]] = rb[j];
        }
    };
    auto stage = [&](int buf, auto SET) {
        stage_unit(buf, SET, std::integral_constant<int, 0>{});
        if constexpr (KU > 1) {
            stage_unit(buf, SET, std::integral_constant<int, 1>{});
            stage_unit(buf, SET, std::integral_constant<int, 2>{});
            stage_unit(buf, SET, std::integral_constant<int, 3>{});
        }
    };
    static_assert(KU == 1 || KU == 4, "stage() spells the units out");

    f32x16 acc[MI][NI];
#pragma unroll
    for (int a = 0; a < MI; ++a)
#pragma unroll
        for (int b = 0; b < NI; ++b)
#pragma unroll
            for (int r = 0; r < 16; ++r) acc[a][b][r] = 0.f;

    if constexpr (PATCH) {
    constexpr int PPX = 180, PROW = 18;
    constexpr int CB = NS == 0 ? 16 : 32;
    constexpr int CHUNKS = NS == 0 ? 4 : AT == 0 ? 8 : 4;
    constexpr int PL = (PPX * CHUNKS + NT - 1) / NT;
    constexpr int B_I = NSX * 2 * (BN / 64);
    static_assert((2 * B_I) % 4 == 0 && NT == 256, "weight DMA is dealt evenly to four waves");
    constexpr int PWB = 2 * B_I / 4;
    f32x4* const patch = smem;
    f32x4* const ring = smem + P_NBUF * P_PATCH;
    const int wave_u = __builtin_amdgcn_readfirstlane(wave);

    unsigned poff[PL];
    int pslot[PL];
#pragma unroll
    for (int j = 0; j < PL; ++j) {
        const int idx = tid + j * NT;
        const bool on = idx < PPX * CHUNKS;
        const int chunk = idx % CHUNKS, pix = on ? idx / CHUNKS : 0;
        const int py = pix / PROW, px = pix - py * PROW;
        const int hs = ph0 - 1 + py, ws = pw0 - 1 + px;
        const bool v = on && (unsigned)hs < (unsigned)p.Hs && (unsigned)ws < (unsigned)p.Ws;
        poff[j] = v ? (unsigned)(((pn * p.Hs + hs) * p.Ws + ws) * p.Cs) * (unsigned)ES + (unsigned)chunk * 16u : OOB_OFFSET;
        pslot[j] = !on ? -1 : NS == 0 ? chunk * PPX + pix : AT == 0 ? ((chunk >> 1) * PPX + pix) * 2 + (chunk & 1) : chunk * PPX + pix;
    }
    f32x4 pr[PL];
    const int ncb = p.Cs / CB;
    auto load_patch = [&](int cb) {
        const unsigned add = (unsigned)(cb * CB * ES);
#pragma unroll
        for (int j = 0; j < PL; ++j) pr[j] = buffer_load_f32x4(rsrc, poff[j] == OOB_OFFSET ? OOB_OFFSET : poff[j] + add);
    };
    auto store_patch = [&](int buf) {
        f32x4* const P = patch + buf * P_PATCH;
#pragma unroll
        for (int j = 0; j < PL; ++j) {
            if (pslot[j] < 0) continue;
            if constexpr (NS == 0) {
                P[pslot[j]] = pr[j];
            } else if constexpr (AT == 0) {
                u32x2 sp[NSX];
                split4<NS>(pr[j], sp);
#pragma unroll
                for (int t = 0; t < NS; ++t) reinterpret_cast<u32x2*>(P + t * 4 * PPX)[pslot[j]] = sp[t];
            } else {
                P[pslot[j]] = pr[j];
            }
        }
    };
    int b_lds[PWB], b_u[PWB];
    unsigned b_add[PWB];
#pragma unroll
    for (int i = 0; i < PWB; ++i) {
        const int t = wave_u + 4 * i, u = t / B_I, rr = t - u * B_I, c = rr & 1, gp = rr >> 1;
        const int g = gp % (BN / 64), plane = gp / (BN / 64);
        b_u[i] = u;
        b_lds[i] = u * P_BUNIT + (plane * 2 + c) * BN + 64 * g;
        b_add[i] = (unsigned)((plane * 2 + c) * p.Cd + n0 + 64 * g + lane) * 16u;
    }
    const unsigned bstep_bytes = (unsigned)(2 * NSX * p.Cd) * 16u;
    const __amdgpu_buffer_rsrc_t rsrcB = __builtin_amdgcn_make_buffer_rsrc(const_cast<float*>(p.wpk + q_wpk_off), 0,
                                                                           (unsigned)qKT * bstep_bytes, 0x00020000);
    int g_kt = 0;
    auto issue_b = [&](int slot_) {
#pragma unroll
        for (int i = 0; i < PWB; ++i) {
            auto* dst = (__attribute__((address_space(3))) void*)(ring + slot_ * P_BSTAGE + b_lds[i]);
            const int kt = g_kt + b_u[i];
            const unsigned off = kt < qKT ? (unsigned)kt * bstep_bytes + b_add[i] : OOB_OFFSET;
            __builtin_amdgcn_raw_ptr_buffer_load_lds(rsrcB, dst, 16, (int)off, 0, 0, 0);
        }
        g_kt += 2;
    };
    const int q4 = li >> 2;
    const int a_pix = (2 * wm * MI + (__builtin_popcount(q4) & 1)) * PROW + (q4 >> 1) * 4 + (li & 3) + lh * PPX;

    if constexpr (NS == 0) {
        unsigned bvo[2][NI];
#pragma unroll
        for (int s2 = 0; s2 < 2; ++s2)
#pragma unroll
            for (int b = 0; b < NI; ++b) bvo[s2][b] = (unsigned)((2 * s2 + lh) * p.Cd + n0 + wn * TN + b * 32 + li) * 16u;
        const unsigned bstep32 = (unsigned)(4 * p.Cd) * 16u;
        const __amdgpu_buffer_rsrc_t rsrcW = __builtin_amdgcn_make_buffer_rsrc(const_cast<float*>(p.wpk + q_wpk_off), 0,
                                                                               (unsigned)qKT * bstep32, 0x00020000);
        int w_kt = 0;
        f32x4 rw[3][2][NI];
        auto issue_w = [&](auto SET) {
            constexpr int st_ = decltype(SET)::value;
            const unsigned so = (unsigned)min(w_kt, qKT - 1) * bstep32;
            ++w_kt;
#pragma unroll
            for (int s2 = 0; s2 < 2; ++s2)
#pragma unroll
                for (int b = 0; b < NI; ++b) {
                    typedef unsigned u32x4_ __attribute__((ext_vector_type(4)));
                    const u32x4_ v_ = __builtin_amdgcn_raw_buffer_load_b128(rsrcW, (int)bvo[s2][b], (int)so, 0);
                    rw[st_][s2][b] = __builtin_bit_cast(f32x4, v_);
                }
        };
        load_patch(0);
        issue_w(std::integral_constant<int, 0>{});
        issue_w(std::integral_constant<int, 1>{});
        store_patch(0);
        asm volatile("s_waitcnt lgkmcnt(0)" ::: "memory");
        __builtin_amdgcn_s_barrier();
        asm volatile("" ::: "memory");
        DBN_TRACE_MARK(1);
        if (p.phase_prio) __builtin_amdgcn_s_setprio(0);
        auto block = [&](int cb, auto ODD) {
            constexpr int odd = decltype(ODD)::value;
            const f32x4* const P = patch + odd * P_PATCH;
// ... 1048 lines not shown
                            t2 += r2[w * BN + cl];
                        }
                        const long c = n0 + cl;
                        if (p.bnb_cnt) {
                            xst(part + (0L * p.Cd + c) * p.stat_rows + trow_, t1);
                            xst(part + (1L * p.Cd + c) * p.stat_rows + trow_, t2);
                        } else {
                            part[(0L * p.Cd + c) * p.stat_rows + trow_] = t1;
                            part[(1L * p.Cd + c) * p.stat_rows + trow_] = t2;
                        }
                    }
                };
                fold16(s1, s2, p.bnb_part);
                if (y2b) fold16(s1, s4, p.bnb_part2);
                bnb_finish(trow_);
                return;
            }
#pragma unroll
            for (int ps = 0; ps < BM / RPP; ++ps) {
                const int row = ps * RPP + tid / LPR;
                const f32x4 v = *reinterpret_cast<const f32x4*>(T + row * PITCH + piece * 8);
                bool ok;
                long doff;
                tile_row(row, ok, doff);
                if (ok) *reinterpret_cast<f32x4*>(reinterpret_cast<unsigned short*>(dstv) + doff + n0 + piece * 8) = v;
            }
            fin_stats();
            return;
        }
    }
    if (DBN_DBG & 64) {
        float s_ = 0.f;
#pragma unroll
        for (int a = 0; a < MI; ++a)
#pragma unroll
            for (int b = 0; b < NI; ++b)
#pragma unroll
                for (int r = 0; r < 16; ++r) s_ += acc[a][b][r];
        if (s_ == 12345.678f) st_dst(dcol, s_);
        return;
    }
    if constexpr (BUFST) {
        const __amdgpu_buffer_rsrc_t rsrcD =
            __builtin_amdgcn_make_buffer_rsrc(slabp, 0, (unsigned)((long)(PATCH ? p.N * p.Hdf * p.Wdf : qM) * p.Cd * 4), 0x00020000);
        const unsigned pitch = (unsigned)p.Cd * 4u;
        const unsigned colb = (unsigned)(n0 + wn * TN + li) * 4u;
#pragma unroll
        for (int a = 0; a < MI; ++a) {
            if constexpr (PATCH) {
                const unsigned row0 = (unsigned)((pn * p.Hdf + ph0 + 2 * (wm * MI + a)) * p.Wdf + pw0);
                const unsigned base0 = (row0 + (unsigned)(lh ? p.Wdf : 0)) * pitch + colb;
                const unsigned base1 = (row0 + (unsigned)(lh ? 0 : p.Wdf)) * pitch + colb;
#pragma unroll
                for (int r = 0; r < 16; ++r) {
                    const unsigned off = ((__builtin_popcount(r >> 2) & 1) ? base1 : base0) + (unsigned)((r >> 2) * 4 + (r & 3)) * pitch;
#pragma unroll
                    for (int b = 0; b < NI; ++b)
                        __builtin_amdgcn_raw_buffer_store_b32(__builtin_bit_cast(unsigned, acc[a][b][r] + bv[b]), rsrcD, (int)off + b * 128, 0, 0);
                }
            } else {
                const unsigned base = (unsigned)(m0 + wm * TM + a * 32 + 4 * lh) * pitch + colb;
#pragma unroll
                for (int r = 0; r < 16; ++r) {
                    const unsigned off = base + (unsigned)((r & 3) + 8 * (r >> 2)) * pitch;
#pragma unroll
                    for (int b = 0; b < NI; ++b)
                        __builtin_amdgcn_raw_buffer_store_b32(__builtin_bit_cast(unsigned, acc[a][b][r] + bv[b]), rsrcD, (int)off + b * 128, 0, 0);
                }
            }
        }
    } else {
#pragma unroll
    for (int a = 0; a < MI; ++a)
        for_rows(a, [&](int r, bool ok, long doff) {
            if (ok) {
#pragma unroll
                for (int b = 0; b < NI; ++b) st_dst(dcol + doff + b * 32, acc[a][b][r] + bv[b]);
            }
        });
    }
    DBN_TRACE_MARK(3);
#if DBN_TRACE
    asm volatile("s_waitcnt vmcnt(0)" ::: "memory");
    DBN_TRACE_MARK(4);
#endif
    fin_stats();
}

template <int BM, int BN, int WM, int WN, int NS, int AT = 0>
int launch_igemm_ns(IgemmParams& p, int mode, hipStream_t st) {
    int grid = 0, rows = 0;
    if (mode == 3) {
        rows = 64 * dbn_ceil_div(p.N * (p.Hdf >> 3) * (p.Wdf >> 3), BM);
        grid = rows * (p.Cd / BN);
    } else if (mode == 2) {
        for (int c = 0; c < p.ncls; ++c) {
            const IgemmClass q = class_geom(c, p.stride, p.R, p.S, p.pad, p.N, p.Hdf, p.Wdf, p.Cs);
            const int mtiles = (q.K > 0 && q.M > 0) ? dbn_ceil_div(q.M, BM) : 0;
            p.row_base[c] = rows;
            rows += mtiles;
            p.tile_end[c] = mtiles * (p.Cd / BN);
            grid = p.tile_end[c] > grid ? p.tile_end[c] : grid;
        }
        grid *= p.ncls;
    } else {
        rows = dbn_ceil_div(p.N * p.Hdf * p.Wdf, BM);
        grid = rows * (p.Cd / BN);
    }
    if (p.stat_rows <= 0) p.stat_rows = rows;
    p.launch_rows = rows;
    if (grid == 0) return DBN_OK;
    p.stagger_units = p.stagger_blocks = 0;
    p.phase_prio = dbn_g_phase_prio;
    p.trace = (DBN_TRACE && dbn_g_trace && grid <= dbn_g_trace_blocks) ? dbn_g_trace : nullptr;
    if (dbn_g_stagger > 0 && NS == 0 && AT == 0 && mode < 2 && p.ksplit <= 1) {
        constexpr int MI_ = BM / WM / 32, NI_ = BN / WN / 32;
        const int slots = (BM * BN <= 4096) ? 7 : (BM * BN <= 8192) ? 4 : 3;
        const long kt = ((long)p.R * p.S * p.Cs + 15) / 16;
        const long units = kt * MI_ * NI_ * 8 * 64 / 1024 * dbn_g_stagger / 1000;
        if (grid > 256 * slots && units > 0) {
            p.stagger_units = (int)std::min<long>(units, 4096);
            p.stagger_blocks = 256 * slots;
        }
    }
    const int gy = (mode < 2 && p.ksplit > 1) ? p.ksplit : 1;
    const bool epi_ok = gy == 1 && p.bnb_y && p.bnb_mean && p.bnb_rstd && (p.bnb_zmask || (p.bnb_msc && p.bnb_msh)) &&
                        (!p.bnb_y2 || (p.bnb_zmask && p.bnb_mean2 && p.bnb_rstd2 && p.bnb_part2));
    if constexpr (BM == 128 && WM == 2 && WN == 2 && (NS > 0 || BN == 64) && AT != 3) {
        if (p.patch && mode < 2) {
            if constexpr (NS == 1 && (AT == 1 || AT == 2)) {
                if (gy == 1 && (!p.bnb_part || epi_ok) &&
                    dbn_wres16_eligible(AT, mode, p.N, p.Hdf, p.Wdf, p.Cs, p.Cd, p.bnb_part != nullptr, p.bnb_y2 != nullptr, p.stats != nullptr))
                    return dbn_launch_wres16(p, mode, AT, st);
            }
            if constexpr (AT == 0 || AT == 1) {
                if (p.bnb_part) {
                    if (!epi_ok) return DBN_ERR_ARG;
                    if (mode == 0)
                        hipLaunchKernelGGL((igemm_f32_kernel<BM, BN, WM, WN, 0, NS, AT, true, 1>), dim3(grid), dim3(256), 0, st, p);
                    else
                        hipLaunchKernelGGL((igemm_f32_kernel<BM, BN, WM, WN, 1, NS, AT, true, 1>), dim3(grid), dim3(256), 0, st, p);
                    return dbn_status();
                }
            }
            if (p.bnb_part) return DBN_ERR_ARG;
            if (mode == 0)
                hipLaunchKernelGGL((igemm_f32_kernel<BM, BN, WM, WN, 0, NS, AT, true>), dim3(grid), dim3(256), 0, st, p);
            else
                hipLaunchKernelGGL((igemm_f32_kernel<BM, BN, WM, WN, 1, NS, AT, true>), dim3(grid), dim3(256), 0, st, p);
            return dbn_status();
        }
    }
    if (p.patch) return DBN_ERR_ARG;
    if ((p.Cs & 15) != 0) {
        if constexpr (AT == 0) {
            if (mode != 0 || p.bnb_part || gy != 1) return DBN_ERR_ARG;
            hipLaunchKernelGGL((igemm_f32_kernel<BM, BN, WM, WN, 0, NS, AT, false, 0, false>), dim3(grid), dim3(WM * WN * 64), 0, st, p);
            return dbn_status();
        } else {
            return DBN_ERR_ARG;
        }
    }
    if (p.bnb_part) {
        if constexpr (AT == 0 || AT == 1) {
            if (!epi_ok) return DBN_ERR_ARG;
            if (mode == 0)
                hipLaunchKernelGGL((igemm_f32_kernel<BM, BN, WM, WN, 0, NS, AT, false, 1>), dim3(grid), dim3(WM * WN * 64), 0, st, p);
            else if (mode == 1)
                hipLaunchKernelGGL((igemm_f32_kernel<BM, BN, WM, WN, 1, NS, AT, false, 1>), dim3(grid), dim3(WM * WN * 64), 0, st, p);
            else if (mode == 2)
                hipLaunchKernelGGL((igemm_f32_kernel<BM, BN, WM, WN, 2, NS, AT, false, 1>), dim3(grid), dim3(WM * WN * 64), 0, st, p);
            else
                return DBN_ERR_ARG;
            return dbn_status();
        } else {
            return DBN_ERR_ARG;
        }
    }
    if (mode == 0)
        hipLaunchKernelGGL((igemm_f32_kernel<BM, BN, WM, WN, 0, NS, AT>), dim3(grid, gy), dim3(WM * WN * 64), 0, st, p);
    else if (mode == 1)
        hipLaunchKernelGGL((igemm_f32_kernel<BM, BN, WM, WN, 1, NS, AT>), dim3(grid, gy), dim3(WM * WN * 64), 0, st, p);
    else if (mode == 2)
        hipLaunchKernelGGL((igemm_f32_kernel<BM, BN, WM, WN, 2, NS, AT>), dim3(grid), dim3(WM * WN * 64), 0, st, p);
    else if constexpr (BM == 128 && BN == 128)
        hipLaunchKernelGGL((igemm_f32_kernel<BM, BN, WM, WN, 3, NS, AT>), dim3(grid), dim3(WM * WN * 64), 0, st, p);
    else
        return DBN_ERR_ARG;
    return dbn_status();
}

#ifndef DBN_WIDE_WM
#define DBN_WIDE_WM 1
#endif
template <int AT>
int launch_wide(IgemmParams& p, int mode, hipStream_t st) {
    constexpr int WM_ = DBN_WIDE_WM, WN_ = 4 / DBN_WIDE_WM;
    static_assert(AT == 1 || AT == 2, "16-bit storage");
    const int rows = mode == 3 ? 64 * dbn_ceil_div(p.N * (p.Hdf >> 3) * (p.Wdf >> 3), 128) : dbn_ceil_div(p.N * p.Hdf * p.Wdf, 128);
    int grid = rows * (p.Cd / 256);
    p.pyr_group = 0;
    if (mode == 3 && dbn_g_pyr_group > 0) {
        p.pyr_group = dbn_g_pyr_group;
        grid = dbn_ceil_div(rows / 64, p.pyr_group) * p.pyr_group * 64 * (p.Cd / 256);
    }
    if (p.stat_rows <= 0) p.stat_rows = rows;
    p.launch_rows = rows;
    if (grid == 0) return DBN_OK;
    p.stagger_units = p.stagger_blocks = 0;
    p.phase_prio = dbn_g_phase_prio;
    p.trace = nullptr;
    if (mode == 3) hipLaunchKernelGGL((igemm_f32_kernel<128, 256, WM_, WN_, 3, 1, AT>), dim3(grid), dim3(256), 0, st, p);
    else if (mode == 0) hipLaunchKernelGGL((igemm_f32_kernel<128, 256, WM_, WN_, 0, 1, AT>), dim3(grid), dim3(256), 0, st, p);
    else hipLaunchKernelGGL((igemm_f32_kernel<128, 256, WM_, WN_, 1, 1, AT>), dim3(grid), dim3(256), 0, st, p);
    return dbn_status();
}
static inline bool wide_tile_ok(const IgemmParams& p, int mode) {
    if (p.bnb_part || p.patch || p.ksplit > 1) return false;
    return dbn_wide_tile_geom_ok(mode, p.N, p.Hdf, p.Wdf, p.Cs, p.Cd);
}

#ifndef DBN_CFG1_WM
#define DBN_CFG1_WM 1
#endif
template <int NS, int AT>
int launch_igemm_cfg(IgemmParams& p, int cfg, int mode, hipStream_t st) {
    if constexpr (NS == 1 && (AT == 1 || AT == 2)) {
        if (cfg == 1 && wide_tile_ok(p, mode)) return launch_wide<AT>(p, mode, st);
    }
    switch (cfg) {
        case 1:
            if constexpr (NS == 1 && (AT == 1 || AT == 2) && DBN_CFG1_WM == 1) return launch_igemm_ns<128, 128, 1, 4, NS, AT>(p, mode, st);
            else return launch_igemm_ns<128, 128, 2, 2, NS, AT>(p, mode, st);
        case 2: return launch_igemm_ns<256, 64, 4, 1, NS, AT>(p, mode, st);
        case 3: return launch_igemm_ns<128, 64, 2, 2, NS, AT>(p, mode, st);
        default: return launch_igemm_ns<64, 64, 2, 2, NS, AT>(p, mode, st);
    }
}

}
```

### db_text_minimal_amd/csrc/pack.hip

```cpp
#include "igemm_common.h"

namespace {

struct PackClass {
    int Rp, Sp, r0, s0, rstep, K, Kpad;
    long krow0;
};
__device__ inline PackClass pack_class(int f, int R, int S, int Cs) {
    PackClass q;
    q.krow0 = 0;
    if (f <= 1) {
        q.Rp = R; q.Sp = S; q.r0 = q.s0 = 0; q.rstep = 1;
    } else {
        const int c = blockIdx.y;
        for (int d = 0; d < c; ++d)
            q.krow0 += (taps_of_class(R, d / f, f) * taps_of_class(S, d % f, f) * Cs + 15) / 16 * 16;
        q.r0 = c / f; q.s0 = c % f; q.rstep = f;
        q.Rp = taps_of_class(R, q.r0, f);
        q.Sp = taps_of_class(S, q.s0, f);
    }
    q.K = q.Rp * q.Sp * Cs;
    q.Kpad = (q.K + 15) / 16 * 16;
    return q;
}

__global__ void pack_weights_kernel(const float* __restrict__ w, int O, int I, int R, int S, int mode, int Cs, int Cd, int f,
                                    float* __restrict__ out) {
    const PackClass q = pack_class(f, R, S, Cs);
    const int K = q.K, Rp = q.Rp, Sp = q.Sp, r0 = q.r0, s0 = q.s0, rstep = q.rstep;
    out += q.krow0 * Cd;
    const long total = (long)q.Kpad * Cd;
    for (long idx = blockIdx.x * (long)blockDim.x + threadIdx.x; idx < total; idx += (long)gridDim.x * blockDim.x) {
        const int e = (int)(idx & 3);
        const long qd = idx >> 2;
        const int cd = (int)(qd % Cd);
        const int kc = (int)(qd / Cd);
        const int k = 4 * kc + e;
        float v = 0.f;
        if (k < K) {
            int tap, cs;
            if ((Cs & 15) == 0) {
                const int blk = k >> 4;
                tap = blk % (Rp * Sp);
                cs = (blk / (Rp * Sp)) * 16 + (k & 15);
            } else {
                tap = k / Cs;
                cs = k - tap * Cs;
            }
            const int rp = tap / Sp, sp = tap - rp * Sp;
            const int r = r0 + rstep * rp, sx = s0 + rstep * sp;
            if (mode == 0) {
                if (cs < I) v = w[(((long)cd * I + cs) * R + r) * S + sx];
            } else {
                v = w[(((long)cs * I + cd) * R + r) * S + sx];
            }
        }
        out[idx] = v;
    }
}

__device__ __forceinline__ unsigned f16_bits(float x) { return (unsigned)__builtin_bit_cast(unsigned short, (_Float16)x); }

__global__ void pack_weights_bf16s_kernel(const float* __restrict__ w, int O, int I, int R, int S, int mode, int Cs, int Cd, int f,
                                          int NS, int f16, unsigned short* __restrict__ out) {
    const PackClass q = pack_class(f, R, S, Cs);
    const int K = q.K, Rp = q.Rp, Sp = q.Sp, r0 = q.r0, s0 = q.s0, rstep = q.rstep;
    out += q.krow0 * Cd * NS;
    const long total = (long)q.Kpad * Cd;
    for (long idx = blockIdx.x * (long)blockDim.x + threadIdx.x; idx < total; idx += (long)gridDim.x * blockDim.x) {
        const int e = (int)(idx & 7);
        const long qd = idx >> 3;
        const int cd = (int)(qd % Cd);
        const int k8g = (int)(qd / Cd);
        const int k = 8 * k8g + e;
        float v = 0.f;
        if (k < K) {
            int tap, cs;
            if ((Cs & 15) == 0) {
                const int blk = k >> 4;
                tap = blk % (Rp * Sp);
                cs = (blk / (Rp * Sp)) * 16 + (k & 15);
            } else {
                tap = k / Cs;
                cs = k - tap * Cs;
            }
            const int rp = tap / Sp, sp = tap - rp * Sp;
            const int r = r0 + rstep * rp, sx = s0 + rstep * sp;
            if (mode == 0) {
                if (cs < I) v = w[(((long)cd * I + cs) * R + r) * S + sx];
            } else {
                v = w[(((long)cs * I + cd) * R + r) * S + sx];
            }
        }
        const int kt = k8g >> 1, k8 = k8g & 1;
        if (f16) {
            out[(((long)kt * 2 + k8) * Cd + cd) * 8 + e] = (unsigned short)f16_bits(v);
            continue;
        }
        for (int t = 0; t < NS; ++t) {
            const unsigned bits = bf16_bits_rne(v);
            out[((((long)kt * NS + t) * 2 + k8) * Cd + cd) * 8 + e] = (unsigned short)bits;
            v -= bf16_bits_to_f32(bits);
        }
    }
}

struct PackJob {
    const float* w;
    void* out;
    int O, I, R, S, mode, Cs, Cd, f;
};

#ifndef DBN_PACK_GRID
#define DBN_PACK_GRID 512
#endif
template <int BF16>
__global__ void pack_many_kernel(const PackJob* __restrict__ jobs, int NS) {
    const PackJob j = jobs[blockIdx.y];
    const float* __restrict__ w = j.w;
    const int ncls = j.f > 1 ? j.f * j.f : 1;
    long krow0 = 0;
    for (int c = 0; c < ncls; ++c) {
        int Rp = j.R, Sp = j.S, r0 = 0, s0 = 0, rstep = 1;
        if (j.f > 1) {
            r0 = c / j.f; s0 = c % j.f; rstep = j.f;
            Rp = taps_of_class(j.R, r0, j.f);
            Sp = taps_of_class(j.S, s0, j.f);
        }
        const int K = Rp * Sp * j.Cs, Kpad = (K + 15) / 16 * 16;
        constexpr int G = BF16 ? 8 : 4;
        const int total = (Kpad / G) * j.Cd;
        const int RSp = Rp * Sp;
        for (int q = blockIdx.x * blockDim.x + threadIdx.x; q < total; q += gridDim.x * blockDim.x) {
            const int kg = q / j.Cd, cd = q - kg * j.Cd;
            const int k0 = G * kg;
            float v[G];
            if ((j.Cs & 15) == 0) {
                const int blk = k0 >> 4;
                const int cb = blk / RSp, tap = blk - cb * RSp;
                const int rp = tap / Sp, sp = tap - rp * Sp;
                const int r = r0 + rstep * rp, sx = s0 + rstep * sp;
                const int cs0 = cb * 16 + (k0 & 15);
#pragma unroll
                for (int e = 0; e < G; ++e) {
                    const int cs = cs0 + e;
                    float t = 0.f;
                    if (k0 + e < K) {
                        if (j.mode == 0) {
                            if (cs < j.I) t = w[(((long)cd * j.I + cs) * j.R + r) * j.S + sx];
                        } else {
                            t = w[(((long)cs * j.I + cd) * j.R + r) * j.S + sx];
                        }
                    }
                    v[e] = t;
                }
            } else {
#pragma unroll
                for (int e = 0; e < G; ++e) {
                    const int k = k0 + e;
                    float t = 0.f;
                    if (k < K) {
                        const int tap = k / j.Cs, cs = k - tap * j.Cs;
                        const int rp = tap / Sp, sp = tap - rp * Sp;
                        const int r = r0 + rstep * rp, sx = s0 + rstep * sp;
                        if (j.mode == 0) {
                            if (cs < j.I) t = w[(((long)cd * j.I + cs) * j.R + r) * j.S + sx];
                        } else {
                            t = w[(((long)cs * j.I + cd) * j.R + r) * j.S + sx];
                        }
                    }
                    v[e] = t;
                }
            }
            if constexpr (BF16 == 2) {
                unsigned short* out = reinterpret_cast<unsigned short*>(j.out) + krow0 * j.Cd;
                const int kt = kg >> 1, k8 = kg & 1;
                unsigned short h[8];
#pragma unroll
                for (int e = 0; e < 8; ++e) h[e] = (unsigned short)f16_bits(v[e]);
                f32x4 pk;
                __builtin_memcpy(&pk, h, 16);
                *reinterpret_cast<f32x4*>(out + (((long)kt * 2 + k8) * j.Cd + cd) * 8) = pk;
            } else if constexpr (BF16 == 1) {
                unsigned short* out = reinterpret_cast<unsigned short*>(j.out) + krow0 * j.Cd * NS;
                const int kt = kg >> 1, k8 = kg & 1;
                for (int t = 0; t < NS; ++t) {
                    unsigned short h[8];
#pragma unroll
                    for (int e = 0; e < 8; ++e) {
                        const unsigned bits = bf16_bits_rne(v[e]);
                        h[e] = (unsigned short)bits;
                        v[e] -= bf16_bits_to_f32(bits);
                    }
                    f32x4 pk;
                    __builtin_memcpy(&pk, h, 16);
                    *reinterpret_cast<f32x4*>(out + ((((long)kt * NS + t) * 2 + k8) * j.Cd + cd) * 8) = pk;
                }
            } else {
                f32x4 pk = {v[0], v[1], v[2], v[3]};
                *reinterpret_cast<f32x4*>(reinterpret_cast<float*>(j.out) + krow0 * j.Cd + (long)q * 4) = pk;
            }
        }
        krow0 += Kpad;
    }
}

#if DBN_HAS_EXPERIMENTS
__global__ __launch_bounds__(256) void split3_kernel(const float* __restrict__ src, unsigned short* __restrict__ planes, long n4,
                                                     long plane_elems) {
    const long stride = (long)gridDim.x * blockDim.x;
    for (long i = blockIdx.x * (long)blockDim.x + threadIdx.x; i < n4; i += stride) {
        const f32x4 v = reinterpret_cast<const f32x4*>(src)[i];
        u32x2 sp[3];
        split4<3>(v, sp);
#pragma unroll
        for (int t = 0; t < 3; ++t) reinterpret_cast<u32x2*>(planes + t * plane_elems)[i] = sp[t];
    }
}

#endif

}

extern "C" {

int dbn_split3(const float* src, void* planes, long n, void* stream) {
#if DBN_HAS_EXPERIMENTS
    DBN_REQUIRE(src && planes && n > 0 && n % 4 == 0);
    hipLaunchKernelGGL(split3_kernel, dim3(dbn_grid(n / 4, 256, 2048)), dim3(256), 0, (hipStream_t)stream, src,
                       reinterpret_cast<unsigned short*>(planes), n / 4, n);
    return dbn_status();
#else
    return DBN_ERR_ARG;
#endif
}

static long panel_floats_all(int O, int I, int R, int S, int mode, int stride, int ns, int cs = 0) {
    if (mode == 0) return panel_floats(R * S * (cs > 0 ? cs : (I + 3) / 4 * 4), O, ns);
    if (stride == 1) return panel_floats(R * S * O, I, ns);
    long tot = 0;
    for (int c = 0; c < stride * stride; ++c)
        tot += panel_floats(taps_of_class(R, c / stride, stride) * taps_of_class(S, c % stride, stride) * O, I, ns);
    return tot;
}

long dbn_igemm_panel_floats(int O, int I, int R, int S, int mode, int stride) { return panel_floats_all(O, I, R, S, mode, stride, 0); }
long dbn_igemm_bf16s_panel_floats(int O, int I, int R, int S, int mode, int stride, int ns) {
    return panel_floats_all(O, I, R, S, mode, stride, ns);
}
long dbn_igemm_panel_floats_t(int kind, int O, int I, int R, int S, int mode, int stride, int cs) {
    return panel_floats_all(O, I, R, S, mode, stride, kind == 2 ? 1 : kind, cs);
}

#ifndef DBN_PACKF_CAP
#define DBN_PACKF_CAP 16
#endif
static int pack_run(const float* w_oihw, int O, int I, int R, int S, int mode, int stride, int ns, float* out, void* stream, int cs = 0,
                    int f16 = 0) {
    DBN_REQUIRE(w_oihw && out && O > 0 && I > 0 && R > 0 && S > 0 && (mode == 0 || mode == 1));
    DBN_REQUIRE(stride == 1 || stride == 2 || stride == 4 || stride == 8 || (mode == 0 && stride >= 1));
    DBN_REQUIRE(cs == 0 || (mode == 0 && cs >= I && cs % 4 == 0));
    const int Cs = (mode == 0) ? (cs > 0 ? cs : ((I + 3) / 4) * 4) : O;
    const int Cd = (mode == 0) ? O : I;
    DBN_REQUIRE(Cs % 4 == 0 && Cd % 64 == 0);
    hipStream_t st = (hipStream_t)stream;
    const int f = (mode == 1 && stride > 1) ? stride : 1;
    const long total = (long)(((dbn_ceil_div(R, f) * dbn_ceil_div(S, f) * Cs + 15) / 16) * 16) * Cd;
    const dim3 grid(dbn_grid(total, 256, f > 2 ? DBN_PACKF_CAP : 1024), f * f);
    if (ns == 0)
        hipLaunchKernelGGL(pack_weights_kernel, grid, dim3(256), 0, st, w_oihw, O, I, R, S, mode, Cs, Cd, f, out);
    else
        hipLaunchKernelGGL(pack_weights_bf16s_kernel, grid, dim3(256), 0, st, w_oihw, O, I, R, S, mode, Cs, Cd, f, ns, f16,
                           reinterpret_cast<unsigned short*>(out));
    return dbn_status();
}

int dbn_pack_weights_t(int kind, const float* w_oihw, int O, int I, int R, int S, int mode, int stride, int cs, float* out, void* stream) {
    DBN_REQUIRE(kind == 0 || kind == 1 || kind == 2 || kind == 3);
    return pack_run(w_oihw, O, I, R, S, mode, stride, kind == 2 ? 1 : kind, out, stream, cs, kind == 2);
}

int dbn_pack_weights_batched(const void* jobs, int n, int ns, void* stream) {
    DBN_REQUIRE(jobs && n > 0 && (ns == 0 || ns == 1 || ns == 2 || ns == 3));
    const dim3 grid(DBN_PACK_GRID, n);
    if (ns == 0)
        hipLaunchKernelGGL(pack_many_kernel<0>, grid, dim3(256), 0, (hipStream_t)stream, reinterpret_cast<const PackJob*>(jobs), 0);
    else if (ns == 2)
        hipLaunchKernelGGL(pack_many_kernel<2>, grid, dim3(256), 0, (hipStream_t)stream, reinterpret_cast<const PackJob*>(jobs), 1);
    else
        hipLaunchKernelGGL(pack_many_kernel<1>, grid, dim3(256), 0, (hipStream_t)stream, reinterpret_cast<const PackJob*>(jobs), ns);
    return dbn_status();
}

int dbn_pack_weights(const float* w_oihw, int O, int I, int R, int S, int mode, int stride, float* out, void* stream) {
    return pack_run(w_oihw, O, I, R, S, mode, stride, 0, out, stream);
}
int dbn_pack_weights_bf16s(const float* w_oihw, int O, int I, int R, int S, int mode, int stride, int ns, float* out, void* stream) {
    DBN_REQUIRE(ns == 1 || ns == 3);
    return pack_run(w_oihw, O, I, R, S, mode, stride, ns, out, stream);
}

}
```

### db_text_minimal_amd/engine.py

```python
import contextlib
import ctypes
import os

import torch

from . import _lib
from ._lib import check

DEAD_PREFIXES = ('backbone.fc.', 'backbone.smooth.')
K_STEP_DEFAULT = 50.0


def _p(t):
    return None if t is None else t.data_ptr()


def _out_hw(conv, H, W):
    k, s, p = conv.k, conv.stride, conv.padding
    return (H + 2 * p - k) // s + 1, (W + 2 * p - k) // s + 1


NO_BN = (None, None, 0.0, 0.0) + (None, ) * 7


def flat_layout(numels):
    offs, total = [], 0
    for n in numels:
        offs.append(total)
        total += (n + 3) // 4 * 4
    return offs, total


IGEMM_TILE_NAMES = {1: 'igemm_f32_kernel<128,128,2,2,%d,%d,%d,%s,%d,%s>', 2: 'igemm_f32_kernel<256,64,4,1,%d,%d,%d,%s,%d,%s>',
                    3: 'igemm_f32_kernel<128,64,2,2,%d,%d,%d,%s,%d,%s>', 4: 'igemm_f32_kernel<64,64,2,2,%d,%d,%d,%s,%d,%s>'}
WGRAD_TILE_NAMES = {1: 'wgrad_f32_kernel<64,192,2,2,%d,%d,%d>', 2: 'wgrad_f32_kernel<128,128,2,2,%d,%d,%d>',
                    3: 'wgrad_f32_kernel<64,128,2,2,%d,%d,%d>', 4: 'wgrad_f32_kernel<64,64,2,2,%d,%d,%d>'}
ACT_DTYPES = {0: torch.float32, 1: torch.bfloat16, 2: torch.float16}


POISON = os.environ.get('DBN_POISON', '')
_poison_count = [0]


def device_empty(shape, device, dtype=torch.float32):
    t = torch.empty(shape, device=device, dtype=dtype)
    if POISON and t.numel():
        if POISON == 'nan':
            t.view(torch.uint8).fill_(0xFF) if not t.is_floating_point() else t.fill_(float('nan'))
        elif POISON == 'rand':
            _poison_count[0] += 1
            g = torch.Generator(device=t.device).manual_seed(1000 + _poison_count[0])
            if t.is_floating_point():
                t.copy_((torch.rand(t.shape, device=t.device, generator=g) * 2000.0 - 1000.0).to(t.dtype))
            else:
                t.view(torch.uint8).copy_(torch.randint(0, 255, (t.numel() * t.element_size(), ), device=t.device, generator=g,
                                                        dtype=torch.uint8).view(t.view(torch.uint8).shape))
        else:
            raise ValueError('DBN_POISON: nan | rand')
    return t


class KernelTimer:

    def __init__(self, labels=None):
        self.labels = labels
        self.records = []
        self._open = None

    def begin(self, label, flops=0.0, nbytes=0.0, tag=''):
        if self.labels is not None and not label.startswith(self.labels):
            return
        e0 = torch.cuda.Event(enable_timing=True)
        e1 = torch.cuda.Event(enable_timing=True)
        e0.record()
        self._open = (label, flops, nbytes, e0, e1, tag)

    def end(self):
        if self._open is not None:
            self._open[4].record()
            self.records.append(self._open)
            self._open = None

    def summary(self, peak_tflops=None, hbm_gbs=None):
        out = {}
        for label, flops, nbytes, e0, e1, _ in self.records:
            d = out.setdefault(label, dict(launches=0, ms=0.0, flops=0.0, bytes=0.0, roof_ms=0.0, hbm_bound=0))
            d['launches'] += 1
            d['ms'] += e0.elapsed_time(e1)
            d['flops'] += flops
            d['bytes'] += nbytes
            if peak_tflops and hbm_gbs and flops > 0:
                t_m, t_h = flops / (peak_tflops * 1e9), nbytes / (hbm_gbs * 1e6)
                d['roof_ms'] += max(t_m, t_h)
                d['hbm_bound'] += int(t_h > t_m)
        return out


class _VirtualConv:

    def __init__(self, cin, cout, k, stride, padding, weight, bias):
        self.cin, self.cout, self.k, self.stride, self.padding, self.weight, self.bias = cin, cout, k, stride, padding, weight, bias


class ConvPlan(object):
    __slots__ = ('winograd', 'winograd_wgrad', 'apply_on_load', 'fold', 'pw16')


class _Shape:

    def __init__(self, *shape):
        self.shape = shape


class Engine:
    def __init__(self, model):
        self.model = model
        self.L = _lib.lib()
        if 'DBN_PATCH_F32' in os.environ:
            self.L.dbn_set_patch_conv(2 if os.environ['DBN_PATCH_F32'] == '0' else 3)
        if 'DBN_WINO_PERSISTENT' in os.environ:
            self.L.dbn_set_winograd_persistent(int(os.environ['DBN_WINO_PERSISTENT']))
        if 'DBN_WINO_CBS' in os.environ:
            self.L.dbn_set_winograd_blocks_per_barrier(int(os.environ['DBN_WINO_CBS']))
        if 'DBN_WINO_STAGGER' in os.environ:
            self.L.dbn_set_winograd_stagger(int(os.environ['DBN_WINO_STAGGER']))
        if 'DBN_PHASE_PRIO' in os.environ:
            self.L.dbn_set_phase_priority(int(os.environ['DBN_PHASE_PRIO']))
        if 'DBN_STAGGER' in os.environ:
            self.L.dbn_set_stagger(int(os.environ['DBN_STAGGER']))
        self.bufs = {}
        self.packs = {}
        self.pack_src = {}
        self._pack_jobs = None
        self.param_epoch = 0
        self.generation = 0
        self.saved_generation = -1
        self.flat = None
        self.flat_grad = None
        self.offsets = None
        self.views = {}
        self.grad_views = {}
        self._dcn_slots, self._dcn_E = {}, {}
        self._plans = {}
        self.dcn_forms = {'gather': 0, 'scatter': 0}
        self.grad_scale = 1.0
        self._live = None
        self.nbt_pending = {}
        self._bias_done = set()
        self._bnb_sums = {}
        self._reduce_pending = []
        self._wgrad_fifo = []
        self._wino_src = {}
        self._wino_jobs = None
        self._reduce_job_cache = {}
        self._reduce_tables = {}
        self._by_ptr = {}
        self._plane_cache = {}
        self.presplit = os.environ.get('DBN_PRESPLIT', '0') == '1' and bool(self.L.dbn_has_experiments())
        self.prof = None
        self.grad_ready_hook = None
        self.ns = 0
        self.at = 0
        self.overlap_wgrad = True
        self.overlap_head_branches = os.environ.get('DBN_OVERLAP_HEAD', '0') == '1'
        self.side_priority = None
        self._side = None
        self._side_used = False
        self._slab_free = [None, None]

    @property
    def live_params(self):
        if self._live is None:
            self._live = [(n, p) for n, p in self.model.named_parameters() if not n.startswith(DEAD_PREFIXES)]
        return self._live

    def ensure_flat(self):
        params = self.live_params
        dev = params[0][1].device
        if dev.type != 'cuda':
            raise RuntimeError('DBTextModel parameters must live on a HIP device (model.to("cuda")); '
                               'there is no CPU path')
        if self.flat is not None and self.flat.device == dev:
            base = self.flat.data_ptr()
            if all(p.data_ptr() == base + 4 * off for (_, p), off in zip(params, self.offsets)):
                return
        offs, total = flat_layout([p.numel() for _, p in params])
        flat = torch.zeros(total, device=dev, dtype=torch.float32)
        grad = torch.zeros(total, device=dev, dtype=torch.float32)
        self.views, self.grad_views = {}, {}
        for (n, p), off in zip(params, offs):
            if p.dtype != torch.float32:
                raise RuntimeError('fp32 parameters expected, got %s for %s' % (p.dtype, n))
            v = flat[off:off + p.numel()].view(p.shape)
            v.copy_(p.data)
            p.data = v
            self.views[n] = v
            self.grad_views[n] = grad[off:off + p.numel()].view(p.shape)
        self.flat, self.flat_grad, self.offsets = flat, grad, offs
        self._reset_caches()
        self.param_epoch += 1

    def _reset_caches(self):
        self.bufs, self.packs, self.pack_src, self._pack_jobs = {}, {}, {}, None
        self._by_ptr, self._plane_cache = {}, {}
        self._reduce_pending, self._reduce_job_cache, self._reduce_tables = [], {}, {}

    def flush_counters(self):
        if not self.nbt_pending:
            return
        mods = dict(self.model.named_modules())
        for name, cnt in self.nbt_pending.items():
            mods[name].num_batches_tracked += cnt
        self.nbt_pending = {}

    MATH_MODES = {'f32': (0, 0), 'bf16x3': (3, 0), 'bf16c': (1, 0), 'bf16': (1, 1), 'fp16': (1, 2)}

    def set_conv_math(self, mode):
        ns, at = self.MATH_MODES[mode]
        if at != self.at:
            self._reset_caches()
            self.saved_generation = -1
        self.ns, self.at = ns, at
        self.math_mode = mode

    math_mode = 'f32'

    @property
    def kind(self):
        return 2 if self.at == 2 else self.ns

    def mark_params_dirty(self):
        self.param_epoch += 1

    def buf(self, name, *shape, dtype=None):
        dtype = ACT_DTYPES[self.at] if dtype is None else dtype
        t = self.bufs.get(name)
        dev = self.flat.device
        if t is None or tuple(t.shape) != tuple(shape) or t.device != dev or t.dtype != dtype:
            t = device_empty(shape, dev, dtype)
            self.bufs[name] = t
            self._by_ptr[t.data_ptr()] = t
        return t

    def _drop_buf(self, name):
        t = self.bufs.pop(name, None)
        if t is not None:
            self._by_ptr.pop(t.data_ptr(), None)
            self._plane_cache.pop(t.data_ptr(), None)

    def fbuf(self, name, *shape):
        return self.buf(name, *shape, dtype=torch.float32)

    def scratch(self, name, numel):
        if self._in_side:
            name += '#side'
        t = self.bufs.get(name)
        if t is None or t.numel() < numel or t.device != self.flat.device:
            t = device_empty(int(numel), self.flat.device)
# ... 109 lines not shown
        if self.prof is not None and self.prof.labels is None and not self.prof_fused:
            return False
        return not (self.splitk and self.L.dbn_igemm_splitk_plan_ns(N * Hd * Wd, Cd, R * S * Cs, Cs, self.ns) > 1)

    prof_fused = True

    def _igemm(self, what, *args, consumer=None):
        N, Hs, Ws, Cs, Hd, Wd, Cd, R, S, stride, pad, mode = args[4:16]
        at, srcp = self._src(args[0], Cs)
        if consumer is not None and self._bnb_eligible(args):
            bn_name, y, zmask = consumer[:3]
            second = consumer[3] if len(consumer) > 3 else None
            assert tuple(y.shape) == (N, Hd, Wd, Cd) and (zmask is None or zmask.shape == y.shape), (what, bn_name)
            hint = args[17]
            rows = self.L.dbn_igemm_bn_rows(at, self.ns, N, Hs, Ws, Cs, Hd, Wd, Cd, R, S, stride, pad, mode, hint)
            part = self.fbuf(bn_name + '/bnb_part', 2 * Cd * rows)
            msc = msh = None
            if zmask is None:
                msc, msh = self.bufs[bn_name + '/scale'], self.bufs[bn_name + '/shift']
            y2 = mean2 = rstd2 = part2 = None
            if second is not None:
                assert zmask is not None and second[1].shape == y.shape
                y2, mean2, rstd2 = second[1], self.bufs[second[0] + '/mean'], self.bufs[second[0] + '/rstd']
                part2 = self.fbuf(second[0] + '/bnb_part', 2 * Cd * rows)
            fin = None
            if self.bnb_finalize_in_kernel:
                G = self.grad_views
                cnt = self.bufs.get(bn_name + '/bnb_cnt')
                ncnt = self.L.dbn_igemm_bn_final_counters(rows, Cd)
                if cnt is None or cnt.numel() != ncnt or cnt.device != self.flat.device:
                    cnt = torch.zeros(ncnt, device=self.flat.device, dtype=torch.int32)
                    self.bufs[bn_name + '/bnb_cnt'] = cnt
                grp = self.fbuf(bn_name + '/bnb_grp', self.L.dbn_igemm_bn_final_group_floats(rows, Cd))
                c1c2 = self.fbuf(bn_name + '/bnb_c1c2', 2 * Cd)
                fin = _lib.BnbFinal(cnt.data_ptr(), grp.data_ptr(), c1c2.data_ptr(), G[bn_name + '.weight'].data_ptr(),
                                    G[bn_name + '.bias'].data_ptr(), None, None, None, self.grad_scale)
                if second is not None:
                    c1c2b = self.fbuf(second[0] + '/bnb_c1c2', 2 * Cd)
                    fin.c1c2_2, fin.dgamma_2, fin.dbeta_2 = (c1c2b.data_ptr(), G[second[0] + '.weight'].data_ptr(),
                                                             G[second[0] + '.bias'].data_ptr())
            check(self.L.dbn_igemm_bnsums_t(at, self.ns, srcp, *args[1:], y.data_ptr(), _p(zmask), _p(msc), _p(msh),
                                            self.bufs[bn_name + '/mean'].data_ptr(), self.bufs[bn_name + '/rstd'].data_ptr(),
                                            part.data_ptr(), _p(y2), _p(mean2), _p(rstd2), _p(part2),
                                            ctypes.byref(fin) if fin is not None else None, self.stream), what)
            self._bnb_sums[bn_name] = (c1c2, -1) if fin is not None else (part, rows)
            if second is not None:
                self._bnb_sums[second[0]] = (c1c2b, -1) if fin is not None else (part2, rows)
            return
        ks, slab = 1, None
        if self.splitk and (mode == 0 or stride == 1):
            ks = self.L.dbn_igemm_splitk_plan_ns(N * Hd * Wd, Cd, R * S * Cs, Cs, self.ns)
            if ks > 1:
                slab = self.scratch('_splitk_slab', self.L.dbn_igemm_splitk_slab_floats(ks, N, Hd, Wd, Cd))
        check(self.L.dbn_igemm_t(at, self.ns, srcp, *args[1:], ks, _p(slab), self.stream), what)

    batched_repack = True
    overlap_repack = True
    _repack_pending = False
    STEM = 'backbone.conv1'

    def _join_repack(self):
        if self._repack_pending:
            assert not self._in_side
            self.join_side()
            self._repack_pending = False

    def repack_params(self):
        if not self.batched_repack:
            return
        ns = self.kind
        beside = self.overlap_repack and self.overlap_wgrad
        stale = []
        for key, (w, cs) in self.pack_src.items():
            if key[3] != ns or (beside and key[0] == self.STEM):
                continue
            ent = self.packs.get(key)
            stamp = self._weight_stamp(w)
            if ent is not None and ent[1] != stamp:
                stale.append((key, w, ent[0], stamp, cs))
        if len(stale) < 8:
            return
        sig = tuple((k, w.data_ptr(), out.data_ptr()) for k, w, out, _, _ in stale)
        if self._pack_jobs is None or self._pack_jobs[0] != sig:
            arr = (_lib.PackJob * len(stale))()
            for i, ((name, mode, stride, _), w, out, _, cs) in enumerate(stale):
                O, I, R, S = w.shape
                arr[i] = _lib.PackJob(w.data_ptr(), out.data_ptr(), O, I, R, S, mode, cs if mode == 0 else O,
                                      O if mode == 0 else I, stride if (mode == 1 and stride > 1) else 1)
            self._pack_jobs = (sig, self._device_table(arr), len(stale))
        _, table, n = self._pack_jobs
        self._launch_repack(beside, lambda: check(self.L.dbn_pack_weights_batched(table.data_ptr(), n, ns, self.stream), 'pack_weights_batched'))
        for key, _, out, stamp, _ in stale:
            self.packs[key] = (out, stamp)
        self._repack_winograd(beside)

    def _device_table(self, arr):
        return torch.frombuffer(bytearray(bytes(arr)), dtype=torch.uint8).to(self.flat.device)

    def _launch_repack(self, beside, launch):
        if beside:
            with self.side_stream():
                launch()
            self._repack_pending = True
        else:
            launch()

    def _repack_fpn(self):
        src = self._fpn_src
        beside = self.overlap_repack and self.overlap_wgrad
        on = self.fpn_repack_early == '1' or (self.fpn_repack_early == '' and self.at != 0)
        if not on or src is None or not beside or self._in_side:
            return
        name, conv, Cg = src
        ent = self.packs.get((name, 'combined'))
        if ent is None or ent[1] == self._weight_stamp(conv.weight):
            return
        derived = [k for k in self.packs if isinstance(k[0], str) and k[0].startswith(name + '#') and '#fold' not in k[0]]

        def run():
            wds, wver = self._fpn_combined_weights(name, conv, Cg)
            for k in derived:
                g = int(k[0][-1])
                if k[1] == 'winograd':
                    self._winograd_panel(k[0], wds[g], k[2], dgrad=k[3], version=wver)
                elif k[3] == self.kind:
                    self.pack(k[0], wds[g], k[1], k[2], version=wver)
        with self.side_stream():
            run()

    fpn_repack_early = os.environ.get('DBN_FPN_REPACK_EARLY', '')
    _fpn_src = None

    def _repack_winograd(self, beside):
        items = [(k, v) for k, v in self._wino_src.items() if k in self.packs]
        if len(items) < 4:
            return
        sig = tuple((k, v[0].data_ptr(), v[1].data_ptr()) for k, v in items)
        if self._wino_jobs is None or self._wino_jobs[0] != sig:
            arr = (_lib.WinogradPackJob * len(items))()
            for i, (_, (w, out, O, I, cs, dgrad)) in enumerate(items):
                arr[i] = _lib.WinogradPackJob(w.data_ptr(), out.data_ptr(), O, I, cs, dgrad)
            self._wino_jobs = (sig, self._device_table(arr), len(items))
        _, table, n = self._wino_jobs
        self._launch_repack(beside, lambda: check(self.L.dbn_winograd_pack_batched(table.data_ptr(), n, self.stream), 'winograd_pack_batched'))
        for k, (w, out, *_r) in items:
            self.packs[k] = (out, self._weight_stamp(w))

    winograd = os.environ.get('DBN_WINOGRAD', '1') == '1'

    def plan(self, conv, shape, train=False, fp32_tensors=True):
        N, H, W, C = shape
        dcn = bool(getattr(conv, 'with_dcn', False))
        key = (conv.cin, conv.cout, conv.k, conv.stride, conv.padding, dcn, N, H, W, C, bool(train), bool(fp32_tensors), self.at, self.ns,
               self.winograd, self.winograd_wgrad, self.fold_eval_bn, self._use_planes, self.splitk, self.pw16, self.apply_on_load)
        pl = self._plans.get(key)
        if pl is None:
            L = self.L
            k, s_, p_ = conv.k, conv.stride, conv.padding
            Ho, Wo = _out_hw(conv, H, W)
            pl = ConvPlan()
            exact = self.ns == 0 and self.at == 0 and fp32_tensors
            s1 = (k, s_, p_) == (3, 1, 1)
            pl.winograd = bool(self.winograd and exact and s1 and L.dbn_winograd_eligible(N, H, W, C, conv.cout))
            pl.winograd_wgrad = bool(self.winograd_wgrad and exact and s1 and L.dbn_winograd_wgrad_eligible(N, H, W, conv.cout, C, conv.cin))
            pl.apply_on_load = bool(self.apply_on_load and not self._use_planes and not dcn and pl.winograd and (not train or pl.winograd_wgrad)
                                    and not (not train and self.fold_eval_bn))
            pl.fold = bool(not train and self.fold_eval_bn and not self._use_planes and not dcn
                           and not (self.splitk and L.dbn_igemm_splitk_plan_ns(N * Ho * Wo, conv.cout, k * k * C, C, self.ns) > 1))
            pl.pw16 = bool(pl.fold and self.pw16 and self.at != 0 and (k, s_, p_) == (1, 1, 0) and C == conv.cin
                           and L.dbn_pw16_eligible(self.at, N, H, W, C, conv.cout))
            self._plans[key] = pl
        return pl

    def _winograd_ok(self, x, conv):
        return self.plan(conv, x.shape, fp32_tensors=x.dtype == torch.float32).winograd

    def _winograd_panel(self, name, w, cs, dgrad=0, version=None):
        if self._repack_pending:
            self._join_repack()
        key = (name, 'winograd', cs, dgrad)
        O, I = (w.shape[1], w.shape[0]) if dgrad else (w.shape[0], w.shape[1])

        def fill(out):
            if version is None:
                self._wino_src[key] = (w, out, O, I, cs, dgrad)
            check(self.L.dbn_winograd_pack(w.data_ptr(), O, I, cs, dgrad, out.data_ptr(), self.stream), 'winograd pack ' + name)
        return self._derived(key, self._weight_stamp(w, version), lambda: device_empty(self.L.dbn_winograd_panel_floats(O, cs), w.device), fill)

    def _winograd_conv(self, name, x, conv, y, bn=None, bn_name=None, x_act=None):
        N, H, W, C = x.shape
        up = self._winograd_panel(name, conv.weight, C)
        asc, ash = (x_act[0].data_ptr(), x_act[1].data_ptr()) if x_act is not None else (None, None)
        if self.prof:
            self.prof.begin('winograd_f32_kernel', 2.0 * N * H * W * conv.cout * conv.cin * 4, 4.0 * N * H * W * (C + conv.cout), 'fwd ' + name)
        sc, sh, bnargs = None, None, NO_BN
        if bn is not None:
            sc, sh, bnargs = self._bn_train_args(bn_name, bn, conv.cout, self.L.dbn_winograd_ws_floats(N, H, W, conv.cout))
            self._announce_bn_final(bn_name, self.L.dbn_winograd_rows(N, H, W), conv.cout)
        check(self.L.dbn_winograd_conv_bn_act_f32(x.data_ptr(), asc, ash, up.data_ptr(), _p(conv.bias), y.data_ptr(), N, H, W, C, conv.cout,
                                                  *bnargs, self.stream), ('winograd ' if bn is None else 'winograd+bn ') + name)
        if self.prof:
            self.prof.end()
        return sc, sh

    def conv_fwd(self, name, x, conv, out_name, version=None, x_act=None):
        N, H, W, C = x.shape
        k, s, p = conv.k, conv.stride, conv.padding
        Ho, Wo = _out_hw(conv, H, W)
        assert C >= conv.cin and C % 4 == 0, (name, C, conv.cin)
        if version is None and self._winograd_ok(x, conv):
            y = self.buf(out_name, N, Ho, Wo, conv.cout)
            self._winograd_conv(name, x, conv, y, x_act=x_act)
            return y
        assert x_act is None, name
        wpk = self.pack(name, conv.weight, 0, version=version, cs=C)
        y = self.buf(out_name, N, Ho, Wo, conv.cout)
        if self.prof:
            self._prof_igemm(N * Ho * Wo, conv.cout, 2.0 * N * Ho * Wo * conv.cout * conv.cin * k * k, 'fwd ' + name, 0,
                             (N, H, W, C, Ho, Wo, k, s, p))
        self._igemm('igemm fwd ' + name, x.data_ptr(), wpk.data_ptr(), _p(conv.bias), y.data_ptr(), N, H, W, C, Ho, Wo, conv.cout, k,
                    k, s, p, 0, 0, 0)
        if self.prof:
            self.prof.end()
        return y

    splitk = True
    fuse_bn_stats = True
    bn_final_in_kernel = os.environ.get('DBN_BN_FINAL', '0') == '1'

    def _announce_bn_final(self, bn_name, rows, C):
        if not self.bn_final_in_kernel or rows <= 0:
            return
        ncnt = self.L.dbn_igemm_bn_final_counters(rows, C)
        cnt = self.bufs.get(bn_name + '/bnf_cnt')
        if cnt is None or cnt.numel() != ncnt or cnt.device != self.flat.device:
            cnt = torch.zeros(ncnt, device=self.flat.device, dtype=torch.int32)
            self.bufs[bn_name + '/bnf_cnt'] = cnt
        ng = self.L.dbn_conv_bn_final_group_doubles(rows, C)
        grp = self.bufs.get(bn_name + '/bnf_grp')
        if grp is None or grp.numel() != ng or grp.device != self.flat.device:
            grp = torch.empty(ng, device=self.flat.device, dtype=torch.float64)
            self.bufs[bn_name + '/bnf_grp'] = grp
        check(self.L.dbn_conv_bn_set_final(cnt.data_ptr(), grp.data_ptr()), 'conv_bn_set_final')

    def _bn_train_args(self, bn_name, bn, C, ws_floats):
        sc, sh = self.fbuf(bn_name + '/scale', C), self.fbuf(bn_name + '/shift', C)
        mu, rs = self.fbuf(bn_name + '/mean', C), self.fbuf(bn_name + '/rstd', C)
        ws = self.scratch('_conv_bn_ws', ws_floats)
        self.nbt_pending[bn_name] = self.nbt_pending.get(bn_name, 0) + 1
        return sc, sh, (bn.weight.data_ptr(), bn.bias.data_ptr(), bn.eps, bn.momentum, bn.running_mean.data_ptr(), bn.running_var.data_ptr(),
                        sc.data_ptr(), sh.data_ptr(), mu.data_ptr(), rs.data_ptr(), ws.data_ptr())

    def _conv_bn_call(self, what, bn_name, bn, y, args, mode, stride, accumulate=0):
        N, Hd, Wd, C = y.shape
        sc, sh, bnargs = self._bn_train_args(bn_name, bn, C, self.L.dbn_conv_bn_ws_floats(N, Hd, Wd, C, mode, stride))
        at, srcp = self._src(args[0], args[7])
        self._announce_bn_final(bn_name, self.L.dbn_igemm_bn_rows(at, self.ns, *args[4:15], mode, 0), C)
        check(self.L.dbn_conv_bn_t(at, srcp, *args[1:], accumulate, 0, self.ns, *bnargs, self.stream), what)
        return sc, sh

    def conv_bn(self, name, x, conv, out_name, bn_name, bn, train, version=None, x_act=None):
        N, H, W, C = x.shape
        k, s, p = conv.k, conv.stride, conv.padding
        Ho, Wo = _out_hw(conv, H, W)
        wino = version is None and self._winograd_ok(x, conv)
        split = self.splitk and self.L.dbn_igemm_splitk_plan_ns(N * Ho * Wo, conv.cout, k * k * C, C, self.ns) > 1
        if not (train and self.fuse_bn_stats) or split:
            y = self.conv_fwd(name, x, conv, out_name, version=version, x_act=x_act)
            sc, sh = self.bn_coef(bn_name, bn, y, train)
            return y, sc, sh
        assert C >= conv.cin and C % 4 == 0, (name, C, conv.cin)
        if wino:
            y = self.buf(out_name, N, Ho, Wo, conv.cout)
            sc, sh = self._winograd_conv(name, x, conv, y, bn, bn_name, x_act=x_act)
            return y, sc, sh
        assert x_act is None, name
        wpk = self.pack(name, conv.weight, 0, version=version, cs=C)
        y = self.buf(out_name, N, Ho, Wo, conv.cout)
        if self.prof:
            self._prof_igemm(N * Ho * Wo, conv.cout, 2.0 * N * Ho * Wo * conv.cout * conv.cin * k * k, 'fwd ' + name, 0,
                             (N, H, W, C, Ho, Wo, k, s, p))
        sc, sh = self._conv_bn_call('conv+bn ' + name, bn_name, bn, y,
                                    (x.data_ptr(), wpk.data_ptr(), _p(conv.bias), y.data_ptr(), N, H, W, C, Ho, Wo, conv.cout, k, k,
                                     s, p, 0), 0, s)
        if self.prof:
            self.prof.end()
        return y, sc, sh

    stem16_pool = os.environ.get('DBN_STEM16_POOL', '1') == '1'
    pw16 = os.environ.get('DBN_PW16', '1') == '1'
    convt16 = os.environ.get('DBN_CONVT16', '1') == '1'

    def _convt16_panel(self, name, ct):
        w = ct.weight
        return self._derived((name, 'convt16', self.kind), self._weight_stamp(w),
                             lambda: torch.empty(self.L.dbn_convt16_panel_bytes(), device=w.device, dtype=torch.uint8),
                             lambda panel: check(self.L.dbn_convt16_pack(self.kind, w.data_ptr(), panel.data_ptr(), self.stream), 'convt16_pack'))

    head16 = os.environ.get('DBN_HEAD16', '1') == '1'

    def _convt16(self, name, x, ct, out_name, bn_name=None, bn=None):
        N, H, W, C = x.shape
        L = self.L
        if not (self.convt16 and self.at != 0 and ct.k == 2 and ct.stride == 2 and bool(L.dbn_convt16_eligible(self.at, N, H, W, C, ct.cout))
                and ct.cin == C):
            return None
        panel = self._convt16_panel(name, ct)
        y = self.buf(out_name, N, 2 * H, 2 * W, ct.cout)
        if self.prof:
            self.prof.begin('convt2x2_b16_kernel<%d>' % self.at, 2.0 * N * H * W * C * ct.cout * 4, float(2 * (x.numel() + y.numel())), 'convT fwd ' + name)
        sc, sh, bnargs = None, None, NO_BN
        if bn is not None:
            sc, sh, bnargs = self._bn_train_args(bn_name, bn, ct.cout, (3 * 64 + 1) * L.dbn_convt16_rows())
        check(L.dbn_convt16_bn_t(self.at, x.data_ptr(), panel.data_ptr(), _p(ct.bias), y.data_ptr(), N, H, W, *bnargs, self.stream),
              ('convt16 ' if bn is None else 'convt16+bn ') + name)
        if self.prof:
            self.prof.end()
        return y, sc, sh

    def convT_bn(self, name, x, ct, out_name, bn_name, bn, train):
        if train and self.fuse_bn_stats:
            got = self._convt16(name, x, ct, out_name, bn_name, bn)
            if got is not None:
                return got
        if not (train and self.fuse_bn_stats):
            y = self.convT_fwd(name, x, ct, out_name)
            sc, sh = self.bn_coef(bn_name, bn, y, train)
            return y, sc, sh
        N, H, W, C = x.shape
        wpk = self.pack(name, ct.weight, 1, 2)
        y = self.buf(out_name, N, 2 * H, 2 * W, ct.cout)
        if self.prof:
            self._prof_convT(N, H, W, C, ct.cout, name)
        sc, sh = self._conv_bn_call('convT+bn ' + name, bn_name, bn, y,
                                    (x.data_ptr(), wpk.data_ptr(), _p(ct.bias), y.data_ptr(), N, H, W, C, 2 * H, 2 * W, ct.cout, 2,
                                     2, 2, 0, 1), 1, 2)
        if self.prof:
            self.prof.end()
        return y, sc, sh

    def _prof_convT(self, N, H, W, C, Co, name):
        flops = 2.0 * N * H * W * C * Co * 4
        at = 3 if self._use_planes else self.at
        if self.L.dbn_igemm_kernel_config(at, self.ns, 2, N, H, W, C, 2 * H, 2 * W, Co, 2, 2, 2, 0, 0, 1) & 32:
            self.prof.begin('convt2x2_f32_kernel<%d>' % C, flops, 0.0, 'convT fwd ' + name)
        else:
            self._prof_igemm(N * 4 * H * W, Co, flops, 'convT fwd ' + name, 2)

    def _prof_igemm(self, M, Cd, flops, tag='', mode=0, geom=None, epi=0):
        cfg = self.L.dbn_igemm_tile_config_ns(M, Cd, self.ns)
        at = 3 if self._use_planes else self.at
        if geom is not None and mode < 2:
            N, Hs, Ws, Cs, Hd, Wd, R, stride, pad = geom
            ks = self.L.dbn_igemm_splitk_plan_ns(N * Hd * Wd, Cd, R * R * Cs, Cs, self.ns) if self.splitk else 1
            cfg = self.L.dbn_igemm_kernel_config(at, self.ns, mode, N, Hs, Ws, Cs, Hd, Wd, Cd, R, R, stride, pad, 0, ks)
        blk = 'false' if (geom is not None and mode == 0 and geom[3] % 16 != 0) else 'true'
        nbytes = 0.0
        if geom is not None:
            N, Hs, Ws, Cs, Hd, Wd = geom[:6]
            nbytes = float(N) * (Hs * Ws * Cs + Hd * Wd * Cd) * (4 if self.at == 0 else 2)
        if geom is not None and mode < 2 and geom[6] == 3 and geom[7] == 1 and geom[8] == 1 and self.ns == 1 and \
                self.L.dbn_wres16_would_run(at, mode, geom[0], geom[4], geom[5], geom[3], Cd, epi, 0):
            self.prof.begin('conv3x3_wres16_kernel<%d,%d,%d,%d>' % (at, geom[3], Cd, mode), flops, nbytes, tag)
            return
        label = IGEMM_TILE_NAMES[cfg & 15] % (mode, self.ns, at, 'true' if cfg & 16 else 'false', epi, blk)
        if (cfg & 15) == 1 and at in (1, 2) and self.ns == 1:
            label = label.replace('<128,128,2,2,', '<128,128,1,4,')
        self.prof.begin(label, flops, nbytes, tag)

    def _winograd_dgrad(self, name, dy, conv, dx, accumulate, consumer, panel=None):
        N, H, W, O = dy.shape
        Cd = dx.shape[3]
        up = panel if panel is not None else self._winograd_panel(name, conv.weight, O, dgrad=1)
        L = self.L
        rows = L.dbn_winograd_rows(N, H, W)
        a = dict(y=None, zmask=None, msc=None, msh=None, mean=None, rstd=None, part=None, y2=None, mean2=None, rstd2=None, part2=None)
        fin = None
        if consumer is not None:
            bn_name, y, zmask = consumer[:3]
            second = consumer[3] if len(consumer) > 3 else None
            assert tuple(y.shape) == (N, H, W, Cd) and (zmask is None or zmask.shape == y.shape), (name, bn_name)
            a.update(y=y, zmask=zmask, mean=self.bufs[bn_name + '/mean'], rstd=self.bufs[bn_name + '/rstd'],
                     part=self.fbuf(bn_name + '/bnb_part', 2 * Cd * rows))
            if zmask is None:
                a.update(msc=self.bufs[bn_name + '/scale'], msh=self.bufs[bn_name + '/shift'])
            if second is not None:
                assert zmask is not None and second[1].shape == y.shape
                a.update(y2=second[1], mean2=self.bufs[second[0] + '/mean'], rstd2=self.bufs[second[0] + '/rstd'],
                         part2=self.fbuf(second[0] + '/bnb_part', 2 * Cd * rows))
            if self.bnb_finalize_in_kernel:
                G = self.grad_views
                cnt = self.bufs.get(bn_name + '/bnb_cnt')
                ncnt = L.dbn_igemm_bn_final_counters(rows, Cd)
                if cnt is None or cnt.numel() != ncnt or cnt.device != self.flat.device:
                    cnt = torch.zeros(ncnt, device=self.flat.device, dtype=torch.int32)
                    self.bufs[bn_name + '/bnb_cnt'] = cnt
                grp = self.fbuf(bn_name + '/bnb_grp', L.dbn_igemm_bn_final_group_floats(rows, Cd))
                c1c2 = self.fbuf(bn_name + '/bnb_c1c2', 2 * Cd)
                fin = _lib.BnbFinal(cnt.data_ptr(), grp.data_ptr(), c1c2.data_ptr(), G[bn_name + '.weight'].data_ptr(),
                                    G[bn_name + '.bias'].data_ptr(), None, None, None, self.grad_scale)
                if second is not None:
                    c1c2b = self.fbuf(second[0] + '/bnb_c1c2', 2 * Cd)
                    fin.c1c2_2, fin.dgamma_2, fin.dbeta_2 = (c1c2b.data_ptr(), G[second[0] + '.weight'].data_ptr(),
                                                             G[second[0] + '.bias'].data_ptr())
        if self.prof:
            extra = sum(a[k] is not None for k in ('y', 'zmask', 'y2')) + int(bool(accumulate))
            self.prof.begin('winograd_f32_kernel', 2.0 * N * H * W * O * Cd * 4, 4.0 * N * H * W * (O + Cd * (1 + extra)), 'dgrad ' + name)
        check(L.dbn_winograd_dgrad_bnsums_f32(dy.data_ptr(), up.data_ptr(), dx.data_ptr(), N, H, W, O, Cd, int(accumulate), _p(a['y']),
                                              _p(a['zmask']), _p(a['msc']), _p(a['msh']), _p(a['mean']), _p(a['rstd']), _p(a['part']),
                                              _p(a['y2']), _p(a['mean2']), _p(a['rstd2']), _p(a['part2']),
                                              ctypes.byref(fin) if fin is not None else None, self.stream), 'winograd dgrad ' + name)
        if self.prof:
            self.prof.end()
        if consumer is not None:
            self._bnb_sums[consumer[0]] = (c1c2, -1) if fin is not None else (a['part'], rows)
            if len(consumer) > 3 and consumer[3] is not None:
                self._bnb_sums[consumer[3][0]] = (c1c2b, -1) if fin is not None else (a['part2'], rows)

    def conv_dgrad(self, name, dy, conv, dx, accumulate, version=None, consumer=None):
        N, Ho, Wo, O = dy.shape
        _, H, W, I = dx.shape
        if (version is None and self.winograd and self.ns == 0 and self.at == 0 and conv.k == 3 and conv.stride == 1 and conv.padding == 1
                and (Ho, Wo) == (H, W) and dy.dtype == torch.float32 and I == conv.cin and O == conv.cout
                and bool(self.L.dbn_winograd_eligible(N, H, W, O, I))):
            if consumer is not None and not (self.fuse_bn_bwd_sums and not (self.prof is not None and self.prof.labels is None and not self.prof_fused)):
                consumer = None
            self._winograd_dgrad(name, dy, conv, dx, accumulate, consumer)
            return
        wpk = self.pack(name, conv.weight, 1, conv.stride, version=version)
        args = (dy.data_ptr(), wpk.data_ptr(), None, dx.data_ptr(), N, Ho, Wo, O, H, W, I, conv.k, conv.k, conv.stride, conv.padding, 1,
                int(accumulate), 0)
        if consumer is not None and not self._bnb_eligible(args):
            consumer = None
        if self.prof:
            self._prof_igemm(N * H * W, I, 2.0 * N * Ho * Wo * O * I * conv.k * conv.k, 'dgrad ' + name, 2 if conv.stride == 2 else 1,
                             (N, Ho, Wo, O, H, W, conv.k, conv.stride, conv.padding), epi=int(consumer is not None))
        self._igemm('igemm dgrad ' + name, *args, consumer=consumer)
        if self.prof:
            self.prof.end()

    defer_wgrad_reduce = os.environ.get('DBN_DEFER_REDUCE', '0') == '1'
    winograd_wgrad = os.environ.get('DBN_WINOGRAD_WGRAD', '1') == '1'

    def wgrad(self, name, sm, big, O, I, k, stride, pad, gview, defer=False, big_act=None):
        N, Ho, Wo, _ = sm.shape
        _, H, W, Cb = big.shape
        if ((k, stride, pad) == (3, 1, 1) and (Ho, Wo) == (H, W)
                and self.plan(_VirtualConv(I, O, k, stride, pad, None, None), big.shape, True,
                              fp32_tensors=sm.dtype == torch.float32 and big.dtype == torch.float32).winograd_wgrad):
            slab = self.scratch('_wgrad_slab', self.L.dbn_winograd_wgrad_slab_floats(N, H, W, O, Cb))
            asc, ash = (big_act[0].data_ptr(), big_act[1].data_ptr()) if big_act is not None else (None, None)
            wargs = (sm.data_ptr(), big.data_ptr(), asc, ash, slab.data_ptr(), gview.data_ptr(), N, H, W, O, Cb, I, self.grad_scale, self.stream)
            if self.prof:
                self.prof.begin('winograd_wgrad_f32_kernel', 2.0 * N * ((H + 1) // 2) * ((W + 1) // 2) * 16 * O * Cb, 0.0, 'wgrad ' + name)
                check(self.L.dbn_winograd_wgrad_f32(1, *wargs), 'winograd wgrad ' + name)
                self.prof.end()
                self.prof.begin('wgrad_reduce_kernel', 0.0, 0.0, 'wgrad reduce ' + name)
                check(self.L.dbn_winograd_wgrad_f32(2, *wargs), 'winograd wgrad reduce ' + name)
                self.prof.end()
            else:
                check(self.L.dbn_winograd_wgrad_f32(3, *wargs), 'winograd wgrad ' + name)
            return
        assert big_act is None, name
        async_reduce = (defer and self.reduce_stream and self._in_side and self.prof is None and not self.defer_wgrad_reduce
                        and not torch.cuda.is_current_stream_capturing())
        defer = defer and self.defer_wgrad_reduce and self.prof is None and Cb % 64 == 0
        slab = self.scratch('_wgrad_slab/' + name if defer else ('_wgrad_slab@%d' % self._slab_k if async_reduce else '_wgrad_slab'),
                            self.L.dbn_wgrad_slab_floats_hw(N, Ho, Wo, O, H, W, Cb, k, k, 4 if self.at == 0 else 2))
        at, smp, bigp = self.at, sm.data_ptr(), big.data_ptr()
        if self._use_planes and sm.dtype == torch.float32 and big.dtype == torch.float32:
            at, smp, bigp = 3, self._planes(sm).data_ptr(), self._planes(big).data_ptr()
        args = (at, self.ns, smp, bigp, slab.data_ptr(), gview.data_ptr(), N, Ho, Wo, O, H, W, Cb, I, k, k, stride,
                pad, self.grad_scale, self.stream)
        if self.prof:
            cfg = self.L.dbn_wgrad_kernel_config_hw(at, self.ns, O, Cb, k, k, stride, pad, Ho, Wo, H, W)
            wname = WGRAD_TILE_NAMES[cfg & 15] % (self.ns, at, (cfg >> 6) & 1)
            if cfg & 32:
                wname = 'wgrad_patch_kernel<%d,%d>' % (self.ns, at)
            elif cfg & 16:
                wname = 'wgrad_tr_kernel<' + wname.split('<')[1].rsplit(',', 3)[0] + '>'
            self.prof.begin(wname,
                            2.0 * N * Ho * Wo * O * I * k * k, 0.0, 'wgrad ' + name)
            check(self.L.dbn_wgrad_phase_t(1, *args), 'wgrad ' + name)
            self.prof.end()
            self.prof.begin('wgrad_reduce_kernel', 0.0, 0.0, 'wgrad reduce ' + name)
            check(self.L.dbn_wgrad_phase_t(2, *args), 'wgrad reduce ' + name)
            self.prof.end()
        elif defer:
            check(self.L.dbn_wgrad_phase_t(1, *args), 'wgrad ' + name)
            key = (name, args[:-1])
            job = self._reduce_job_cache.get(key)
            if job is None:
                job = _lib.WgradReduceJob()
                check(self.L.dbn_wgrad_reduce_describe(*args[:-1], ctypes.byref(job)), 'wgrad reduce describe ' + name)
                self._reduce_job_cache[key] = job
            self._reduce_pending.append((key, job))
        elif async_reduce:
            side = torch.cuda.current_stream(self.flat.device)
            free = self._slab_free[self._slab_k]
            if free is not None:
                side.wait_event(free)
            check(self.L.dbn_wgrad_phase_t(1, *args), 'wgrad ' + name)
# ... 1066 lines not shown
```

### include/dbnet_hip.h

```cpp
#ifndef DBNET_HIP_H
#define DBNET_HIP_H
#ifdef __cplusplus
extern "C" {
#endif


int dbn_pack_weights(const float* w_oihw, int O, int I, int R, int S, int mode, int stride, float* out, void* stream);
long dbn_igemm_panel_floats(int O, int I, int R, int S, int mode, int stride);
int dbn_igemm_packed_floats(int K, int Cd);

int dbn_igemm_f32(const float* src, const float* wpk, const float* bias, float* dst, int N, int Hs, int Ws, int Cs, int Hd,
                  int Wd, int Cd, int R, int S, int stride, int pad, int mode, int accumulate, int tile_hint, void* stream);

int dbn_pack_weights_bf16s(const float* w_oihw, int O, int I, int R, int S, int mode, int stride, int ns, float* out, void* stream);
int dbn_pack_weights_batched(const void* jobs, int n, int ns, void* stream);
long dbn_igemm_bf16s_panel_floats(int O, int I, int R, int S, int mode, int stride, int ns);
int dbn_igemm_bf16s(const float* src, const float* wpk, const float* bias, float* dst, int N, int Hs, int Ws, int Cs, int Hd,
                    int Wd, int Cd, int R, int S, int stride, int pad, int mode, int accumulate, int tile_hint, int ns,
                    void* stream);
int dbn_wgrad_bf16s(const float* sm, const float* big, float* slab, float* grad_oihw, int N, int Ho, int Wo, int O, int H, int W,
                    int Cb, int I, int R, int S, int stride, int pad, float scale, int ns, void* stream);

int dbn_igemm_bn_rows(int at, int ns, int N, int Hs, int Ws, int Cs, int Hd, int Wd, int Cd, int R, int S, int stride, int pad, int mode,
                      int tile_hint);
// ... 83 lines not shown

int dbn_nearest_up_fwd(const float* src, const float* addend, float* dst, int N, int Hs, int Ws, int C, int H, int W, int Cdst,
                       int coff, void* stream);
int dbn_nearest_up_bwd(const float* dbig, float* dsrc, int N, int Hs, int Ws, int C, int H, int W, int Cbig, int coff,
                       int accumulate, void* stream);

int dbn_bilinear_fwd(const float* src, float* dst, long planes, int Hs, int Ws, int H, int W, void* stream);
int dbn_bilinear_bwd(const float* ddst, float* dsrc, long planes, int Hs, int Ws, int H, int W, void* stream);

int dbn_fpn_combine_weights(const float* w, int Co, int Cin, int group, int Cg, float* wd, void* stream);
int dbn_fpn_scatter_wgrad(const float* t0, const float* t1, const float* t2, const float* t3, int Co, int Cg, float* dw,
                          void* stream);

int dbn_nchw3_to_nhwc4(const float* x, float* out, int N, int H, int W, void* stream);
int dbn_add_inplace(const float* x, float* y, long n, void* stream);

int dbn_head_tail_fwd(const float* xb, const float* xt, const float* wb, const float* wt, const float* bias_b,
                      const float* bias_t, const float* bn_scale_b, const float* bn_shift_b, const float* bn_scale_t,
                      const float* bn_shift_t, float* out, int N, int Hq, int Wq, int channels, float kstep, void* stream);
int dbn_head_tail_bwd_ws_floats(void);
int dbn_head_tail_bwd(const float* xb, const float* xt, const float* wb, const float* wt, const float* preds,
                      const float* dpreds, const float* bn_scale_b, const float* bn_shift_b, const float* bn_scale_t,
                      const float* bn_shift_t, const float* bn_mean_b, const float* bn_rstd_b, const float* bn_mean_t,
                      const float* bn_rstd_t, float* bn_sums, float* dxb, float* dxt, float* dw_b, float* dbias_b, float* dw_t,
                      float* dbias_t, int N, int Hq, int Wq, int channels, float kstep, float grad_scale, float* ws, void* stream);

int dbn_set_winograd_persistent(int on);
int dbn_set_winograd_stagger(int permille);
int dbn_set_winograd_blocks_per_barrier(int n);
int dbn_winograd_eligible(int N, int H, int W, int Cs, int Cd);
long dbn_winograd_panel_floats(int O, int Cs);
int dbn_winograd_pack(const float* w_oihw, int O, int I, int Cs, int dgrad, float* out, void* stream);
int dbn_winograd_pack_batched(const void* jobs, int n, void* stream);
int dbn_winograd_rows(int N, int H, int W);
int dbn_winograd_dgrad_bnsums_f32(const float* dy, const float* upanel, float* dx, int N, int H, int W, int Cs, int Cd, int accumulate,
                                  const void* y, const void* zmask, const float* mask_scale, const float* mask_shift,
                                  const float* save_mean, const float* save_rstd, float* part, const void* y2, const float* save_mean2,
                                  const float* save_rstd2, float* part2, const dbn_bnb_final* fin, void* stream);
long dbn_winograd_ws_floats(int N, int H, int W, int Cd);
int dbn_winograd_conv_bn_act_f32(const float* src, const float* in_scale, const float* in_shift, const float* upanel, const float* bias,
                                 float* dst, int N, int H, int W, int Cs, int Cd, const float* gamma, const float* beta, float eps,
                                 float momentum, float* run_mean, float* run_var, float* scale, float* shift, float* save_mean,
                                 float* save_rstd, float* ws, void* stream);
int dbn_winograd_conv_bn_f32(const float* src, const float* upanel, const float* bias, float* dst, int N, int H, int W, int Cs, int Cd,
                             const float* gamma, const float* beta, float eps, float momentum, float* run_mean, float* run_var,
                             float* scale, float* shift, float* save_mean, float* save_rstd, float* ws, void* stream);

int dbn_winograd_wgrad_eligible(int N, int H, int W, int O, int Cb, int I);
int dbn_winograd_wgrad_linear(int H, int W);
long dbn_winograd_wgrad_slab_floats(int N, int H, int W, int O, int Cb);
int dbn_winograd_wgrad_f32(int phases, const float* dy, const float* x, const float* x_scale, const float* x_shift, float* slab, float* grad,
                           int N, int H, int W, int O, int Cb, int I, float scale, void* stream);

int dbn_db_loss_ws_bytes(void);
int dbn_db_loss_fwd(const float* preds, const float* gts, int N, int H, int W, int channels, float alpha, float beta,
                    double negative_ratio, float eps, float* losses, float* coef, void* ws, void* stream);
int dbn_db_loss_bwd(const float* preds, const float* gts, const float* coef, const float* grad_losses, float alpha, float beta,
                    int N, int H, int W, int channels, float* dpreds, void* stream);
int dbn_db_loss_sum_fwd(const float* preds, const float* gts, int N, int H, int W, int channels, float alpha, float beta,
                        double negative_ratio, float eps, float* losses, float* coef, void* ws, void* stream);
int dbn_db_loss_frac_fwd(const float* preds, const float* gts, int N, int H, int W, int channels, float alpha, float beta,
                         double negative_ratio, float eps, int sum, float* losses, float* coef, void* ws, void* stream);

long dbn_db_loss_ohem_ws_bytes(int N, int H, int W);
int dbn_db_loss_ohem_fwd(const float* preds, const float* gts, int N, int H, int W, int channels, float alpha, float beta,
                         double negative_ratio, float eps, float* losses, float* coef, void* ws, void* stream);
int dbn_db_loss_ohem_bwd(const float* preds, const float* gts, const float* coef, const float* grad_losses, const void* ws,
                         float alpha, float beta, int N, int H, int W, int channels, float* dpreds, void* stream);

int dbn_pixel_confusion(const float* preds, long batch_stride, const float* gt, const float* mask, int N, int H, int W, float thresh,
                        double* hist, void* stream);

int dbn_adam_step(float* p, const float* g, float* m, float* v, long n, float lr, float beta1, float beta2, float eps, int step,
                  float grad_scale, void* stream);

int dbn_has_experiments(void);

int dbn_clock_probe(void* out2, int microseconds, void* stream);
int dbn_wall_clock_khz(void);

int dbn_deform_im2col(const float* x, const float* offset, float* cols, int N, int H, int W, int C, int Ho, int Wo, int R, int S,
                      int stride, int pad, int off_stride, void* stream);
long dbn_deform_col2im_ws_bytes(int N, int H, int W, int C, int Ho, int Wo, int R, int S);
int dbn_deform_col2im(const float* dcols, const float* x, const float* offset, float* dx, float* doffset, int accumulate, void* ws, int N,
                      int H, int W, int C, int Ho, int Wo, int R, int S, int stride, int pad, int off_stride, void* stream);
int dbn_permute_weight(const float* src, float* dst, int O, int C, int T, int to_ohwi, float scale, void* stream);

int dbn_binarize_u8(const float* pred, int N, int channels, int H, int W, float thresh, unsigned char* out, void* stream);
int dbn_box_scores(const float* bitmap, int H, int W, const float* boxes, int K, int P, float* scores, void* stream);

int dbn_gt_maps(const double* verts, const double* dist, const int* meta, const int* img_off, const int* ixy, int N, int P, int S,
                int max_verts, int max_off_pts, float scale, float tmin, float* out, void* stream);
int dbn_normalize_u8(const unsigned char* in, int N, int H, int W, float m0, float m1, float m2, float* out, void* stream);
int dbn_poly_offset(const double* xy, int n, const double* delta, int* out_xy, int cap, int* out_n);
int dbn_poly_offset_paths(const double* xy, int n, const double* delta, int* out_xy, int cap, int* out_n, int* out_paths);

int dbn_warp_affine_u8(const unsigned char* src, long src_bytes, const long long* desc, const double* coef, int N, int max_h, int max_w,
                       unsigned char* dst, long dst_bytes, void* stream);
int dbn_resize_cubic_u8(const unsigned char* src, long src_bytes, const long long* desc, const double* coef, int N, int max_h, int max_w,
                        unsigned char* dst, long dst_bytes, void* stream);
int dbn_resize_linear_norm_u8(const unsigned char* src, long src_bytes, const long long* desc, const double* coef, int N, int CH, int CW,
                              float m0, float m1, float m2, float* out, void* stream);

int dbn_perspective_maps(const float* quads, int K, int out_h, int out_w, double* fwd, double* inv);
int dbn_warp_perspective_u8(const unsigned char* src, long src_bytes, const long long* desc, const double* inv, int K, int out_h, int out_w,
                            unsigned char* dst, long dst_bytes, void* stream);

int dbn_draw_strokes(const unsigned char* src, unsigned char* dst, long bytes, const long long* desc, int N, const int* edges, long E,
                     int thickness, int c0, int c1, int c2, void* stream);
int dbn_draw_glyphs(const unsigned char* src, unsigned char* dst, long bytes, const long long* desc, int N, const int* edges, long E,
                    const int* glyphs, int G, const int* recs, long R, int size64, int rows, int c0, int c1, int c2, void* stream);
int dbn_render_minmax(const long long* desc, const double* coef, int N, long n_px, const float* prob, long map_elems, long img_stride,
                      int row_stride, int binary, float thresh, void* mm, void* stream);
int dbn_render_paint(const unsigned char* src, unsigned char* dst, const long long* desc, const double* coef, int N, long n_px, const float* prob,
                     long map_elems, long img_stride, int row_stride, int binary, float thresh, const void* mm, const void* lut, float alpha,
                     void* stream);
int dbn_minmax_scale_u8(const float* x, int N, int H, int W, void* mm, unsigned char* out, void* stream);

int dbn_words_to_input(int at, const unsigned char* crops, long n_px, long hw, int rgb, int bgr, const float* lut, void* out, void* stream);
long dbn_greedy_decode_ws_bytes(int B, int T);
int dbn_greedy_decode(int at, const void* logits, int B, int T, int C, const int* lengths, int mode, void* ws, int* codes, int* count,
                      float* score, void* stream);

long dbn_detect_ws_bytes(int N, int H, int W, int max_candidates);
int dbn_detect(const float* pred, int N, int channels, int H, int W, float thresh, int max_candidates, void* ws, int* labels, void* recs,
               int* counts, void* stream);
int dbn_detect_host(const void* recs, const int* counts, int N, int max_candidates, int H, int W, const double* params, const int* dest_hw,
                    short* boxes, float* scores, float* info);

long dbn_detect_poly_ws_bytes(int N, int H, int W, int max_candidates);
long dbn_detect_poly_verts_cap(int N, int H, int W);
int dbn_detect_poly(const float* pred, int N, int channels, int H, int W, float thresh, int max_candidates, void* ws, void* poly_ws,
                    int* labels, void* table, short* verts, void* stream);
int dbn_detect_poly_host(const void* recs, const int* counts, const int* nv, const int* voff, const short* verts, int N, int max_candidates,
                         int H, int W, const double* params, const int* dest_hw, int* poly_n, int* poly_off, int* poly_xy, int poly_cap,
                         int* poly_total, double* scores, double* info, int* approx_xy);

long dbn_det_eval_ws_bytes(int n_polys);
int dbn_det_eval_overlaps(const double* verts, const int* poff, int n_polys, const long long* img, int N, long n_pairs, int cull, void* ws,
                          double* inter, double* area, int* nonsimple, void* stream);
int dbn_det_eval_match_host(int protocol, int N, const int* sizes, const double* inter, const double* gt_area, const double* det_area,
                            const unsigned char* gt_ignore, const double* gt_cd, const double* det_cd, const double* params, double* stats,
                            unsigned char* det_dc, int* rows, int* n_rows);


#define DBN_AT_F32 0
#define DBN_AT_BF16 1
#define DBN_AT_F16 2
#define DBN_AT_SPLIT3 3
int dbn_split3(const float* src, void* planes, long n, void* stream);

long dbn_igemm_panel_floats_t(int kind, int O, int I, int R, int S, int mode, int stride, int cs);
int dbn_pack_weights_t(int kind, const float* w_oihw, int O, int I, int R, int S, int mode, int stride, int cs, float* out, void* stream);

int dbn_igemm_t(int at, int ns, const void* src, const float* wpk, const float* bias, void* dst, int N, int Hs, int Ws, int Cs, int Hd,
                int Wd, int Cd, int R, int S, int stride, int pad, int mode, int accumulate, int tile_hint, int ksplit, float* slab,
                void* stream);
int dbn_conv_bn_t(int at, const void* src, const float* wpk, const float* bias, void* dst, int N, int Hs, int Ws, int Cs, int Hd, int Wd,
                  int Cd, int R, int S, int stride, int pad, int mode, int accumulate, int tile_hint, int ns,
                  const float* gamma, const float* beta, float eps, float momentum, float* run_mean, float* run_var,
                  float* scale, float* shift, float* save_mean, float* save_rstd, float* ws, void* stream);
int dbn_pyramid_conv_t(int at, const void* s0, const void* s1, const void* s2, const void* s3, const float* w0, const float* w1,
                       const float* w2, const float* w3, const float* bias, void* dst, int N, int H, int W, int Cs, int Cd,
                       int tile_hint, int ns, const float* gamma, const float* beta, float eps, float momentum, float* run_mean,
                       float* run_var, float* scale, float* shift, float* save_mean, float* save_rstd, float* ws, void* stream);
int dbn_pyramid_conv_from_t(int first_level, int at, const void* s0, const void* s1, const void* s2, const void* s3, const float* w0,
                            const float* w1, const float* w2, const float* w3, const float* bias, void* dst, int N, int H, int W, int Cs,
                            int Cd, int tile_hint, int ns, const float* gamma, const float* beta, float eps, float momentum,
                            float* run_mean, float* run_var, float* scale, float* shift, float* save_mean, float* save_rstd, float* ws,
                            void* stream);
int dbn_wgrad_t(int at, int ns, const void* sm, const void* big, float* slab, float* grad_oihw, int N, int Ho, int Wo, int O, int H, int W,
                int Cb, int I, int R, int S, int stride, int pad, float scale, void* stream);

int dbn_set_wgrad_variant(int variant);
int dbn_set_convt_kernel(int on);
int dbn_wgrad_kernel_config(int at, int ns, int O, int J, int Cb);
int dbn_wgrad_kernel_config_hw(int at, int ns, int O, int Cb, int R, int S, int stride, int pad, int Ho, int Wo, int H, int W);
int dbn_set_patch_conv(int on);
int dbn_set_wres16(int on);
int dbn_set_pyramid_wide(int on);
int dbn_pyramid_wide_would_run(int at, int N, int H, int W, int Cs, int Cd);
int dbn_wres16_would_run(int at, int mode, int N, int H, int W, int Cs, int Cd, int bnb, int y2);

int dbn_mfma_sustained(int kind, const void* operands, float* out, int iters, void* stream);
long dbn_mfma_sustained_flops(int kind, int iters);
int dbn_set_stagger(int permille);
int dbn_set_phase_priority(int on);
int dbn_set_trace(void* buf, long max_blocks);
int dbn_igemm_kernel_config(int at, int ns, int kmode, int N, int Hs, int Ws, int Cs, int Hd, int Wd, int Cd, int R, int S, int stride,
                            int pad, int tile_hint, int ksplit);
typedef struct dbn_wgrad_reduce_job {
    const float* slab;
    float* grad;
    int splitk, O, J, Jp, BM, BN, Cb, I, RS, G, natural, blocks;
    float scale;
    int smem_bytes;
} dbn_wgrad_reduce_job;
int dbn_wgrad_reduce_describe(int at, int ns, const void* sm, const void* big, float* slab, float* grad_oihw, int N, int Ho, int Wo, int O,
                              int H, int W, int Cb, int I, int R, int S, int stride, int pad, float scale, void* job);
int dbn_wgrad_reduce_many(const void* jobs, const int* first, int n_jobs, int total_blocks, int max_smem, void* stream);
int dbn_wgrad_tile_config(int O, int J);
int dbn_wgrad_phase_t(int phase, int at, int ns, const void* sm, const void* big, float* slab, float* grad_oihw, int N, int Ho, int Wo,
                      int O, int H, int W, int Cb, int I, int R, int S, int stride, int pad, float scale, void* stream);

int dbn_deform_im2col_t(int at, const void* x, const void* offset, void* cols, int N, int H, int W, int C, int Ho, int Wo, int R, int S,
                        int stride, int pad, int off_stride, void* stream);
int dbn_deform_col2im_t(int at, const void* dcols, const void* x, const void* offset, void* dx, void* doffset, int accumulate, void* ws,
                        int N, int H, int W, int C, int Ho, int Wo, int R, int S, int stride, int pad, int off_stride, void* stream);
long dbn_deform_col2im_gather_ws_bytes(int N, int Ho, int Wo);
int dbn_deform_col2im_gather_t(int at, const void* dcols, const void* x, const void* offset, void* dx, void* doffset, int accumulate,
                               void* ws, int N, int H, int W, int C, int Ho, int Wo, int R, int S, int stride, int pad, int off_stride,
                               void* stream);
int dbn_deform_offset_absmax_t(int at, const void* offset, long n, unsigned* out_bits, void* stream);
int dbn_cast_f32(int at, const float* src, void* dst, long n, void* stream);

int dbn_bn_train_stats_t(int at, const void* y, int M, int C, const float* gamma, const float* beta, float eps, float momentum,
                         float* run_mean, float* run_var, float* scale, float* shift, float* save_mean, float* save_rstd,
                         float* ws, void* stream);
int dbn_bn_apply_t(int at, const void* y, const float* scale, const float* shift, const void* res, const float* res_scale,
                   const float* res_shift, void* out, long M, int C, int relu, void* stream);
int dbn_bn_backward_t(int at, const float* sums, int sums_parts, const void* y, const void* zmask, const float* mask_scale,
                      const float* mask_shift, const void* dout, const float* save_mean, const float* save_rstd, const float* gamma,
                      void* dy, void* gout, int gout_accumulate, float* dgamma, float* dbeta, float* dbias_conv, int M, int C,
                      float grad_scale, float* ws, void* stream);
int dbn_col_sum_t(int at, const void* x, int M, int C, float* out, float scale, float* ws, void* stream);
int dbn_bnrelu_maxpool_fwd_t(int at, const void* y, const float* scale, const float* shift, void* out, int N, int H, int W, int C,
                             void* stream);
int dbn_maxpool_bwd_parts(int N, int H, int W, int C);
int dbn_bnrelu_maxpool_bwd_t(int at, const void* y, const float* scale, const float* shift, const void* pooled, const void* dpool,
                             void* dz, int N, int H, int W, int C, const float* bn_mean, const float* bn_rstd, float* bn_part,
                             void* stream);
int dbn_bnrelu_maxpool_fwd_arg_t(int at, const void* y, const float* scale, const float* shift, void* out, void* idx, void* ypool, int N, int H,
                                 int W, int C, void* stream);
long dbn_maxpool_bn_backward_ws_floats(int N, int H, int W, int C);
int dbn_maxpool_bn_backward_t(int at, const void* y, const void* dpool, const void* idx, const void* ypool, const float* save_mean,
                              const float* save_rstd, const float* gamma, void* dy, float* dgamma, float* dbeta, int N, int H, int W, int C,
                              float grad_scale, float* ws, void* stream);
int dbn_nearest_up_fwd_t(int at, const void* src, const void* addend, void* dst, int N, int Hs, int Ws, int C, int H, int W, int Cdst,
                         int coff, void* stream);
int dbn_nearest_up_bwd_t(int at, const void* dbig, void* dsrc, int N, int Hs, int Ws, int C, int H, int W, int Cbig, int coff,
                         int accumulate, void* stream);
int dbn_nchw3_to_nhwc4_t(int at, const float* x, void* out, int N, int H, int W, void* stream);
int dbn_stem16_padded_h(int H);
int dbn_stem16_padded_w(int W);
int dbn_stem16_rows(void);
long dbn_stem16_panel_bytes(void);
int dbn_stem16_eligible(int at, int N, int H, int W);
int dbn_stem16_pack(int kind, const float* w_oihw, void* out, void* stream);
int dbn_nchw3_to_padded4_t(int at, const float* x, void* xp, void* x4, int N, int H, int W, void* stream);
int dbn_stem16_conv_bn_t(int at, const void* xp, const void* wpk, void* y, int N, int H, int W, const float* gamma, const float* beta, float eps,
                         float momentum, float* run_mean, float* run_var, float* scale, float* shift, float* save_mean, float* save_rstd,
                         float* ws, void* stream);
int dbn_stem16_pool_eligible(int at, int N, int H, int W);
int dbn_stem16_conv_bn_relu_pool_t(int at, const void* xp, const void* wpk, const float* scale, const float* shift, void* out, int N, int H, int W,
                                   void* stream);
int dbn_convt16_rows(void);
long dbn_convt16_panel_bytes(void);
int dbn_convt16_eligible(int at, int N, int H, int W, int Cin, int Cout);
int dbn_convt16_pack(int kind, const float* w_iohw, void* out, void* stream);
int dbn_convt16_bn_t(int at, const void* x, const void* wpk, const float* bias, void* y, int N, int H, int W, const float* gamma, const float* beta,
                     float eps, float momentum, float* run_mean, float* run_var, float* scale, float* shift, float* save_mean, float* save_rstd,
                     float* ws, void* stream);
int dbn_pw16_eligible(int at, int N, int H, int W, int Cin, int Cout);
long dbn_pw16_panel_bytes(void);
int dbn_pw16_pack(int kind, const float* w_oihw, int Cout, void* out, void* stream);
int dbn_pw16_act_t(int at, const void* x, const void* wpk, const float* bias, int relu, void* y, int N, int H, int W, int Cout, void* stream);
int dbn_head16_eligible(int at, int N, int Hq, int Wq);
int dbn_head16_tail_eval_t(int at, const void* x_b, const void* x_t, const void* panel_b, const void* panel_t, const float* bias1_b,
                           const float* bias1_t, const float* scale_b, const float* shift_b, const float* scale_t, const float* shift_t,
                           const float* w2_b, const float* w2_t, const float* bias2_b, const float* bias2_t, float* out, int N, int Hq, int Wq,
                           void* stream);

int dbn_nchw3_to_nhwc16_and_4_t(int at, const float* x, void* out16, void* out4, int N, int H, int W, void* stream);
int dbn_nchw3_to_nhwc4_packed_t(int at, const float* x, void* out, int N, int H, int W, void* stream);
int dbn_head_tail_fwd_t(int at, const void* xb, const void* xt, const float* wb, const float* wt, const float* bias_b,
                        const float* bias_t, const float* bn_scale_b, const float* bn_shift_b, const float* bn_scale_t,
                        const float* bn_shift_t, float* out, int N, int Hq, int Wq, int channels, float kstep, void* stream);
int dbn_set_head_tail_wide(int mode);
int dbn_head_tail_bwd_t(int at, const void* xb, const void* xt, const float* wb, const float* wt, const float* preds,
                        const float* dpreds, const float* bn_scale_b, const float* bn_shift_b, const float* bn_scale_t,
                        const float* bn_shift_t, const float* bn_mean_b, const float* bn_rstd_b, const float* bn_mean_t,
                        const float* bn_rstd_t, float* bn_sums, void* dxb, void* dxt, float* dw_b, float* dbias_b, float* dw_t,
                        float* dbias_t, int N, int Hq, int Wq, int channels, float kstep, float grad_scale, float* ws, void* stream);
int dbn_head_tail_bn_bwd_ws_floats(void);
int dbn_head_tail_bn_bwd_t(int at, int phases, const void* yb, const void* yt, const float* wb, const float* wt, const float* preds, const float* dpreds,
                           const float* bn_scale_b, const float* bn_shift_b, const float* bn_scale_t, const float* bn_shift_t,
                           const float* bn_mean_b, const float* bn_rstd_b, const float* bn_mean_t, const float* bn_rstd_t,
                           const float* bn_gamma_b, const float* bn_gamma_t, void* dyb, void* dyt, float* dgamma_b, float* dbeta_b,
                           float* dgamma_t, float* dbeta_t, float* dbias_conv_b, float* dbias_conv_t, float* dw_b, float* dbias_b, float* dw_t,
                           float* dbias_t, int N, int Hq, int Wq, int channels, float kstep, float grad_scale, float* ws, void* stream);

int dbn_jpeg_info(const unsigned char* data, long len, long long* out);
int dbn_jpeg_info_ex(const unsigned char* data, long len, int flags, long long* out);
long dbn_jpeg_coef_elems_ex(const unsigned char* blob, const long long* offs, int N, int flags, long long* per_image);
int dbn_jpeg_entropy_batch_ex(const unsigned char* blob, const long long* offs, int N, short* coef, long coef_elems, long long* desc,
                              unsigned short* qtabs, int* status, int* orientation, int threads, int flags);
int dbn_jpeg_pixels_ex(const short* coef, long coef_elems, const long long* desc, const unsigned short* qtabs, int N, const int* tab_idct,
                       int n_idct, const int* tab_rgb, int n_rgb, const int* orientation, const int* tab_tile, int n_tile,
                       unsigned char* planes, unsigned char* out, long out_bytes, void* stream);
long dbn_jpeg_coef_elems(const unsigned char* blob, const long long* offs, int N, long long* per_image);
int dbn_jpeg_entropy_batch(const unsigned char* blob, const long long* offs, int N, short* coef, long coef_elems, long long* desc,
                           unsigned short* qtabs, int* status, int threads);
int dbn_jpeg_pixels(const short* coef, long coef_elems, const long long* desc, const unsigned short* qtabs, int N, const int* tab_idct,
                    int n_idct, const int* tab_rgb, int n_rgb, unsigned char* planes, unsigned char* out, long out_bytes, void* stream);

int dbn_jpeg_forward(const unsigned char* pixels, long in_bytes, const long long* desc, const unsigned short* qtabs, int N,
// ... 34 lines not shown
```

Before: 745.2.

## Add dense 3-channel stem conv path packing five taps per k-tile

Adds a dense K-walk variant of the fp32 implicit-GEMM kernel for the stem convolution, where the input has 3 real channels padded to 4. Each k-tile of 16 now packs five filter taps of three channels each instead of four taps of four padded channels, so fewer K iterations run and the zero padding channel is no longer multiplied. This needs a new weight packing kernel, a thread-local flag that routes igemm to the new template mode, and per-thread gathering of five taps into shared memory. The path is on by default through DBN_STEM_DENSE and only applies to the stem, so its effect is limited to that one layer's forward pass.

```diff
diff --git a/db_text_minimal_amd/_lib.py b/db_text_minimal_amd/_lib.py
--- a/db_text_minimal_amd/_lib.py
+++ b/db_text_minimal_amd/_lib.py
@@ -193,6 +193,9 @@
     'dbn_cast_f32': 'ipplp',
     'dbn_pack_weights_t': 'ip' + 'i' * 7 + 'pp',
     'dbn_igemm_panel_floats_t': 'i' * 8,
+    'dbn_igemm_dense3_panel_floats': 'iii',
+    'dbn_pack_weights_dense3': 'piiiipp',
+    'dbn_igemm_set_dense3': 'i',
     'dbn_bn_train_stats_t': 'i' + SIGNATURES['dbn_bn_train_stats'],
     'dbn_bn_apply_t': 'i' + SIGNATURES['dbn_bn_apply'],
     'dbn_bn_backward_t': 'ipi' + SIGNATURES['dbn_bn_backward_ex'][1:],
@@ -226,7 +229,7 @@
     'dbn_head_tail_bn_bwd_ws_floats': '',
     'dbn_head_tail_bn_bwd_t': 'ii' + 'p' * 28 + 'iiii' + 'ff' + 'pp',
 })
-LONG_RETURN = {'dbn_jpeg_coef_elems', 'dbn_jpeg_coef_elems_ex', 'dbn_jpeg_dhuff_ws_bytes', 'dbn_jpeg_encode_bound', 'dbn_greedy_decode_ws_bytes', 'dbn_det_eval_ws_bytes', 'dbn_detect_ws_bytes', 'dbn_detect_poly_ws_bytes', 'dbn_detect_poly_verts_cap', 'dbn_mfma_sustained_flops', 'dbn_conv_bn_final_group_doubles', 'dbn_maxpool_bn_backward_ws_floats', 'dbn_pw16_panel_bytes', 'dbn_stem16_panel_bytes', 'dbn_convt16_panel_bytes', 'dbn_winograd_panel_floats', 'dbn_winograd_wgrad_slab_floats', 'dbn_winograd_ws_floats', 'dbn_igemm_splitk_slab_floats', 'dbn_deform_col2im_ws_bytes', 'dbn_deform_col2im_gather_ws_bytes', 'dbn_igemm_bn_final_counters', 'dbn_igemm_bn_final_group_floats', 'dbn_igemm_panel_floats_t', 'dbn_wgrad_slab_floats_hw', 'dbn_wgrad_slab_floats', 'dbn_igemm_panel_floats', 'dbn_igemm_bf16s_panel_floats', 'dbn_db_loss_ohem_ws_bytes', 'dbn_conv_bn_ws_floats', 'dbn_pyramid_conv_ws_floats'}
+LONG_RETURN = {'dbn_jpeg_coef_elems', 'dbn_jpeg_coef_elems_ex', 'dbn_jpeg_dhuff_ws_bytes', 'dbn_jpeg_encode_bound', 'dbn_greedy_decode_ws_bytes', 'dbn_det_eval_ws_bytes', 'dbn_detect_ws_bytes', 'dbn_detect_poly_ws_bytes', 'dbn_detect_poly_verts_cap', 'dbn_mfma_sustained_flops', 'dbn_conv_bn_final_group_doubles', 'dbn_maxpool_bn_backward_ws_floats', 'dbn_pw16_panel_bytes', 'dbn_stem16_panel_bytes', 'dbn_convt16_panel_bytes', 'dbn_winograd_panel_floats', 'dbn_winograd_wgrad_slab_floats', 'dbn_winograd_ws_floats', 'dbn_igemm_splitk_slab_floats', 'dbn_deform_col2im_ws_bytes', 'dbn_deform_col2im_gather_ws_bytes', 'dbn_igemm_bn_final_counters', 'dbn_igemm_bn_final_group_floats', 'dbn_igemm_panel_floats_t', 'dbn_igemm_dense3_panel_floats', 'dbn_wgrad_slab_floats_hw', 'dbn_wgrad_slab_floats', 'dbn_igemm_panel_floats', 'dbn_igemm_bf16s_panel_floats', 'dbn_db_loss_ohem_ws_bytes', 'dbn_conv_bn_ws_floats', 'dbn_pyramid_conv_ws_floats'}
 _KIND = {'p': _P, 'i': _I, 'l': _L, 'f': _F, 'd': _D}
 
 
diff --git a/db_text_minimal_amd/csrc/conv.hip b/db_text_minimal_amd/csrc/conv.hip
--- a/db_text_minimal_amd/csrc/conv.hip
+++ b/db_text_minimal_amd/csrc/conv.hip
@@ -244,8 +244,9 @@
                          int Wd, int Cd, int R, int S, int stride, int pad, int mode, int accumulate, int cfg, int ns,
                          hipStream_t st, float* stats, int stat_rows, int stat_row0, int ksplit, float* slab, int* rows_out, int at,
                          long plane_bytes, const IgemmBnb* bnb = nullptr, int tile_hint = -1, const void* res = nullptr, int relu = 0,
-                         const BnFin* bnf = nullptr) {
+                         const BnFin* bnf = nullptr, int dense3 = 0) {
     IgemmParams p{};
+    p.dense3 = dense3;
     if (bnf) {
         p.bnf_cnt = bnf->cnt; p.bnf_grp = bnf->grp; p.bnf_gamma = bnf->gamma; p.bnf_beta = bnf->beta; p.bnf_eps = bnf->eps;
         p.bnf_momentum = bnf->momentum; p.bnf_run_mean = bnf->run_mean; p.bnf_run_var = bnf->run_var; p.bnf_scale = bnf->scale;
@@ -335,10 +336,19 @@
     return rows;
 }
 
+static thread_local int g_dense3 = 0;
+int dbn_igemm_set_dense3(int on) {
+    g_dense3 = on != 0;
+    return DBN_OK;
+}
+
 static int igemm_run(const void* src, const float* wpk, const float* bias, void* dst, int N, int Hs, int Ws, int Cs, int Hd,
                      int Wd, int Cd, int R, int S, int stride, int pad, int mode, int accumulate, int tile_hint, int ns,
                      void* stream, float* stats = nullptr, int ksplit = 1, float* slab = nullptr, int stat_rows_total = 0, int at = 0,
                      const IgemmBnb* bnb = nullptr, const void* res = nullptr, int relu = 0, const BnFin* bnf = nullptr) {
+    const int dense3 = g_dense3;
+    g_dense3 = 0;
+    DBN_REQUIRE(!dense3 || (at == 0 && ns == 0 && mode == 0 && Cs == 4 && tile_hint == 2 && ksplit <= 1 && !bnb && !res && !relu));
     DBN_REQUIRE((!res && !relu) || (ksplit <= 1 && !stats && !bnb && !(mode == 1 && stride > 1)));
     DBN_REQUIRE(src && wpk && dst && (ns == 0 || ns == 1 || ns == 3));
     DBN_REQUIRE(at == 0 || ((at == 1 || at == 2) && ns == 1 && Cs % 16 == 0) || (at == 3 && ns == 3 && Cs % 16 == 0));
@@ -370,7 +380,7 @@
                                      reinterpret_cast<char*>(dst) + (long)n0 * Hd * Wd * Cd * des, n, Hs, Ws, Cs, Hd, Wd, Cd, R, S, stride,
                                      pad, mode, accumulate, cfg, ns, st, stats, stat_rows_total, row0, ksplit, slab, &rows, at, plane_bytes,
                                      bnb ? &b : nullptr, tile_hint,
-                                     res ? reinterpret_cast<const char*>(res) + (long)n0 * Hd * Wd * Cd * des : nullptr, relu, bnf);
+                                     res ? reinterpret_cast<const char*>(res) + (long)n0 * Hd * Wd * Cd * des : nullptr, relu, bnf, dense3);
         if (rc) return rc;
         row0 += rows;
     }
diff --git a/db_text_minimal_amd/csrc/igemm_common.h b/db_text_minimal_amd/csrc/igemm_common.h
--- a/db_text_minimal_amd/csrc/igemm_common.h
+++ b/db_text_minimal_amd/csrc/igemm_common.h
@@ -75,6 +75,7 @@
     unsigned long long* trace;
     int launch_rows;
     int patch;
+    int dense3;
     const void* seg_src[4];
     const float* seg_wpk[4];
     unsigned seg_bytes[4];
diff --git a/db_text_minimal_amd/csrc/igemm_kernel.h b/db_text_minimal_amd/csrc/igemm_kernel.h
--- a/db_text_minimal_amd/csrc/igemm_kernel.h
+++ b/db_text_minimal_amd/csrc/igemm_kernel.h
@@ -12,8 +12,11 @@
                                        ((EPI) == 1 && (AT) == 1 && (PATCH) && (BN) == 64) ? 4 : \
                                        ((EPI) == 0 && (NS) == 0 && (AT) == 0 && (BM) * (BN) == 4096 && (MODE) < 2) ? 7 : 1, 8)))
 
-template <int BM, int BN, int WM, int WN, int MODE, int NS, int AT = 0, bool PATCH = false, int EPI = 0, bool BLK = true>
-__global__ __launch_bounds__(WM* WN * 64) DBN_IGEMM_OCC(BM, BN, NS, MODE, PATCH, EPI, AT) void igemm_f32_kernel(const IgemmParams p) {
+template <int BM, int BN, int WM, int WN, int MODE_, int NS, int AT = 0, bool PATCH = false, int EPI = 0, bool BLK = true>
+__global__ __launch_bounds__(WM* WN * 64) DBN_IGEMM_OCC(BM, BN, NS, (MODE_ == 4 ? 0 : MODE_), PATCH, EPI, AT) void igemm_f32_kernel(const IgemmParams p) {
+    constexpr int MODE = MODE_ == 4 ? 0 : MODE_;
+    constexpr bool DENSE = MODE_ == 4;
+    static_assert(!DENSE || (!BLK && NS == 0 && AT == 0 && !PATCH && EPI == 0 && BM == WM * WN * 64), "dense stem walk: exact fp32, one row per thread");
     static_assert(EPI == 0 || ((AT == 0 || AT == 1) && MODE < 3), "BatchNorm-backward sums: fp32 or bf16 storage, no pyramid form");
     static_assert(BLK || (AT == 0 && MODE == 0 && !PATCH && EPI == 0), "non-blocked K walk: forward conv on fp32 tensors");
     static_assert(AT == 0 || ((AT == 1 || AT == 2) && NS == 1) || (AT == 3 && NS == 3), "storage type / matrix math combination");
@@ -30,7 +33,8 @@
     constexpr int NP = AT == 3 ? 3 : 1;
     constexpr int A_SH = AT == 0 ? 2 : 1;
     constexpr int A_CH = AT == 0 ? 4 : 8;
-    constexpr int A_PIECES = (BM << A_SH) * NP;
+    constexpr int DENSE_TAPS = 5;
+    constexpr int A_PIECES = DENSE ? DENSE_TAPS * BM : (BM << A_SH) * NP;
     constexpr int A_LD = (A_PIECES + NT - 1) / NT;
     constexpr bool A_FULL = A_PIECES % NT == 0;
     constexpr int AS = NS == 0 ? BM + 2 : BM + 4, BS = NS == 0 ? BN + 2 : BN + 4;
@@ -145,6 +149,10 @@
     } else {
         q.Hd = p.Hdf; q.Wd = p.Wdf; q.M = p.N * p.Hdf * p.Wdf; q.R = p.R; q.S = p.S;
         q.K = p.R * p.S * p.Cs; q.KT = (q.K + 15) / 16;
+        if constexpr (DENSE) {
+            q.KT = (p.R * p.S + DENSE_TAPS - 1) / DENSE_TAPS;
+            q.K = 16 * q.KT;
+        }
         q.pad_h = q.pad_w = p.pad; q.oh0 = q.ow0 = 0;
     }
     const int ntn = p.Cd / BN;
@@ -164,8 +172,8 @@
 
     __amdgpu_buffer_rsrc_t rsrc = __builtin_amdgcn_make_buffer_rsrc(const_cast<void*>(p.src), 0, p.src_bytes, 0x00020000);
 
-    const int a_chunk = tid & ((1 << A_SH) - 1);
-    auto a_row = [&](int j) { return AT == 0 ? (tid >> 2) + j * (NT / 4) : ((tid + j * NT) >> 1) % BM; };
+    const int a_chunk = DENSE ? 0 : tid & ((1 << A_SH) - 1);
+    auto a_row = [&](int j) { return DENSE ? tid : AT == 0 ? (tid >> 2) + j * (NT / 4) : ((tid + j * NT) >> 1) % BM; };
     auto a_plane = [&](int j) { return AT == 0 ? 0 : ((tid + j * NT) >> 1) / BM; };
     auto a_on = [&](int j) { return A_FULL || tid + j * NT < A_PIECES; };
     int a_hb[A_LD], a_wb[A_LD], a_nb[A_LD];
@@ -195,6 +203,7 @@
             a_hb[j] = ok ? hd * p.stride - q.pad_h : -(1 << 20);
             a_wb[j] = wd * p.stride - q.pad_w;
             if (SOFF) a_org[j] = (unsigned)(a_nb[j] + (hd * p.stride * p.Ws + wd * p.stride) * p.Cs + A_CH * a_chunk) * (unsigned)ES;
+            if (DENSE) a_org[j] = (unsigned)((a_nb[j] + ((hd * p.stride - q.pad_h) * p.Ws + wd * p.stride - q.pad_w) * p.Cs) * (int)ES);
         } else {
             a_hb[j] = ok ? hd + q.pad_h : -(1 << 20);
             a_wb[j] = wd + q.pad_w;
@@ -235,7 +244,21 @@
     unsigned asoff[KU];
     int kend = (MODE < 2 && p.ksplit > 1) ? min(qK, 16 * kt_end) : qK;
     auto next_offsets = [&](int u = 0) {
-        if constexpr (SOFF) {
+        if constexpr (DENSE) {
+#pragma unroll
+            for (int j = 0; j < A_LD; ++j) {
+                const int hs = a_hb[0] + k_r, ws = a_wb[0] + k_s;
+                const bool v = k_r < qR && (unsigned)hs < (unsigned)gHs && (unsigned)ws < (unsigned)gWs;
+                aoff[u][j] = v ? (unsigned)((int)a_org[0] + (k_r * gWs + k_s) * p.Cs * (int)ES) : OOB_OFFSET;
+                if (++k_s == qS) {
+                    k_s = 0;
+                    ++k_r;
+                }
+            }
+            asoff[u] = 0;
+            kidx += 16;
+            return;
+        } else if constexpr (SOFF) {
             const int tr = MODE == 0 ? k_r : qR - 1 - k_r, ts = MODE == 0 ? k_s : qS - 1 - k_s;
             asoff[u] = (unsigned)((tr * gWs + ts) * p.Cs + k_cb) * (unsigned)ES;
             const bool kv = kidx - A_CH * a_chunk < kend;
@@ -388,7 +411,15 @@
         f32x4* As = smem + buf * STAGE + u_ * UNIT;
         f32x4* Bs = As + A_IMG;
         if (DBN_DBG & 4) return;
-        if constexpr (NS == 0) {
+        if constexpr (DENSE) {
+            static_assert(A_LD == 5, "five taps per k-tile");
+#pragma unroll
+            for (int j = 0; j < A_LD; ++j) asm volatile("" ::"v"(ra[j][3]));
+            As[0 * AS + tid] = f32x4{ra[0][0], ra[0][1], ra[0][2], ra[1][0]};
+            As[1 * AS + tid] = f32x4{ra[1][1], ra[1][2], ra[2][0], ra[2][1]};
+            As[2 * AS + tid] = f32x4{ra[2][2], ra[3][0], ra[3][1], ra[3][2]};
+            As[3 * AS + tid] = f32x4{ra[4][0], ra[4][1], ra[4][2], 0.f};
+        } else if constexpr (NS == 0) {
 #pragma unroll
             for (int j = 0; j < A_LD; ++j) As[a_chunk * AS + (tid >> 2) + j * (NT / 4)] = ra[j];
         } else if constexpr (AT != 0) {
@@ -1743,6 +1774,15 @@
         }
     }
     if (p.patch) return DBN_ERR_ARG;
+    if (p.dense3) {
+        if constexpr (AT == 0 && NS == 0 && BM == WM * WN * 64) {
+            if (mode != 0 || p.Cs != 4 || p.bnb_part || gy != 1) return DBN_ERR_ARG;
+            hipLaunchKernelGGL((igemm_f32_kernel<BM, BN, WM, WN, 4, 0, 0, false, 0, false>), dim3(grid), dim3(WM * WN * 64), 0, st, p);
+            return dbn_status();
+        } else {
+            return DBN_ERR_ARG;
+        }
+    }
     if ((p.Cs & 15) != 0) {
         if constexpr (AT == 0) {
             if (mode != 0 || p.bnb_part || gy != 1) return DBN_ERR_ARG;
diff --git a/db_text_minimal_amd/csrc/pack.hip b/db_text_minimal_amd/csrc/pack.hip
--- a/db_text_minimal_amd/csrc/pack.hip
+++ b/db_text_minimal_amd/csrc/pack.hip
@@ -55,6 +55,18 @@
                 v = w[(((long)cs * I + cd) * R + r) * S + sx];
             }
         }
+        out[idx] = v;
+    }
+}
+
+__global__ void pack_weights_dense3_kernel(const float* __restrict__ w, int I, int R, int S, int Cd, int KT, float* __restrict__ out) {
+    const int total = KT * 16 * Cd;
+    for (int idx = blockIdx.x * blockDim.x + threadIdx.x; idx < total; idx += gridDim.x * blockDim.x) {
+        const int e = idx & 3, qd = idx >> 2;
+        const int cd = qd % Cd, k = 4 * (qd / Cd) + e;
+        const int kl = k & 15, tap = 5 * (k >> 4) + kl / 3, ci = kl % 3;
+        float v = 0.f;
+        if (kl < 15 && tap < R * S && ci < I) v = w[((cd * I + ci) * R + tap / S) * S + tap % S];
         out[idx] = v;
     }
 }
@@ -280,6 +292,15 @@
     return pack_run(w_oihw, O, I, R, S, mode, stride, kind == 2 ? 1 : kind, out, stream, cs, kind == 2);
 }
 
+long dbn_igemm_dense3_panel_floats(int O, int R, int S) { return (long)dbn_ceil_div(R * S, 5) * 16 * O; }
+int dbn_pack_weights_dense3(const float* w_oihw, int O, int I, int R, int S, float* out, void* stream) {
+    DBN_REQUIRE(w_oihw && out && O > 0 && O % 64 == 0 && I > 0 && I <= 3 && R > 0 && S > 0);
+    const int KT = dbn_ceil_div(R * S, 5);
+    hipLaunchKernelGGL(pack_weights_dense3_kernel, dim3(dbn_grid((long)KT * 16 * O, 256, 1024)), dim3(256), 0, (hipStream_t)stream, w_oihw, I, R,
+                       S, O, KT, out);
+    return dbn_status();
+}
+
 int dbn_pack_weights_batched(const void* jobs, int n, int ns, void* stream) {
     DBN_REQUIRE(jobs && n > 0 && (ns == 0 || ns == 1 || ns == 2 || ns == 3));
     const dim3 grid(DBN_PACK_GRID, n);
diff --git a/db_text_minimal_amd/engine.py b/db_text_minimal_amd/engine.py
--- a/db_text_minimal_amd/engine.py
+++ b/db_text_minimal_amd/engine.py
@@ -103,7 +103,7 @@
 
 
 class ConvPlan(object):
-    __slots__ = ('winograd', 'winograd_wgrad', 'apply_on_load', 'fold', 'pw16')
+    __slots__ = ('winograd', 'winograd_wgrad', 'apply_on_load', 'fold', 'pw16', 'stem_dense')
 
 
 class _Shape:
@@ -519,7 +519,8 @@
         N, H, W, C = shape
         dcn = bool(getattr(conv, 'with_dcn', False))
         key = (conv.cin, conv.cout, conv.k, conv.stride, conv.padding, dcn, N, H, W, C, bool(train), bool(fp32_tensors), self.at, self.ns,
-               self.winograd, self.winograd_wgrad, self.fold_eval_bn, self._use_planes, self.splitk, self.pw16, self.apply_on_load)
+               self.winograd, self.winograd_wgrad, self.fold_eval_bn, self._use_planes, self.splitk, self.pw16, self.apply_on_load,
+               self.stem_dense)
         pl = self._plans.get(key)
         if pl is None:
             L = self.L
@@ -536,8 +537,17 @@
                            and not (self.splitk and L.dbn_igemm_splitk_plan_ns(N * Ho * Wo, conv.cout, k * k * C, C, self.ns) > 1))
             pl.pw16 = bool(pl.fold and self.pw16 and self.at != 0 and (k, s_, p_) == (1, 1, 0) and C == conv.cin
                            and L.dbn_pw16_eligible(self.at, N, H, W, C, conv.cout))
+            pl.stem_dense = bool(self.stem_dense and exact and not self._use_planes and not dcn and C == 4 and conv.cin <= 3
+                                 and conv.cout % 64 == 0 and L.dbn_igemm_tile_config_ns(N * Ho * Wo, conv.cout, 0) == 2)
             self._plans[key] = pl
         return pl
+
+    stem_dense = os.environ.get('DBN_STEM_DENSE', '1') == '1'
+
+    def _dense3_panel(self, name, w):
+        O, I, R, S = w.shape
+        return self._derived((name, 'dense3'), self._weight_stamp(w), lambda: device_empty(self.L.dbn_igemm_dense3_panel_floats(O, R, S), w.device),
+                             lambda out: check(self.L.dbn_pack_weights_dense3(w.data_ptr(), O, I, R, S, out.data_ptr(), self.stream), 'pack_weights_dense3'))
 
     def _winograd_ok(self, x, conv):
         return self.plan(conv, x.shape, fp32_tensors=x.dtype == torch.float32).winograd
@@ -580,13 +590,16 @@
             self._winograd_conv(name, x, conv, y, x_act=x_act)
             return y
         assert x_act is None, name
-        wpk = self.pack(name, conv.weight, 0, version=version, cs=C)
+        dense = version is None and self.plan(conv, x.shape, fp32_tensors=x.dtype == torch.float32).stem_dense
+        wpk = self._dense3_panel(name, conv.weight) if dense else self.pack(name, conv.weight, 0, version=version, cs=C)
         y = self.buf(out_name, N, Ho, Wo, conv.cout)
         if self.prof:
             self._prof_igemm(N * Ho * Wo, conv.cout, 2.0 * N * Ho * Wo * conv.cout * conv.cin * k * k, 'fwd ' + name, 0,
-                             (N, H, W, C, Ho, Wo, k, s, p))
+                             (N, H, W, C, Ho, Wo, k, s, p), dense3=dense)
+        if dense:
+            check(self.L.dbn_igemm_set_dense3(1), 'igemm_set_dense3')
         self._igemm('igemm fwd ' + name, x.data_ptr(), wpk.data_ptr(), _p(conv.bias), y.data_ptr(), N, H, W, C, Ho, Wo, conv.cout, k,
-                    k, s, p, 0, 0, 0)
+                    k, s, p, 0, 0, 2 if dense else 0)
         if self.prof:
             self.prof.end()
         return y
@@ -618,12 +631,15 @@
         return sc, sh, (bn.weight.data_ptr(), bn.bias.data_ptr(), bn.eps, bn.momentum, bn.running_mean.data_ptr(), bn.running_var.data_ptr(),
                         sc.data_ptr(), sh.data_ptr(), mu.data_ptr(), rs.data_ptr(), ws.data_ptr())
 
-    def _conv_bn_call(self, what, bn_name, bn, y, args, mode, stride, accumulate=0):
+    def _conv_bn_call(self, what, bn_name, bn, y, args, mode, stride, accumulate=0, dense3=False):
+        hint = 2 if dense3 else 0
         N, Hd, Wd, C = y.shape
         sc, sh, bnargs = self._bn_train_args(bn_name, bn, C, self.L.dbn_conv_bn_ws_floats(N, Hd, Wd, C, mode, stride))
         at, srcp = self._src(args[0], args[7])
-        self._announce_bn_final(bn_name, self.L.dbn_igemm_bn_rows(at, self.ns, *args[4:15], mode, 0), C)
-        check(self.L.dbn_conv_bn_t(at, srcp, *args[1:], accumulate, 0, self.ns, *bnargs, self.stream), what)
+        self._announce_bn_final(bn_name, self.L.dbn_igemm_bn_rows(at, self.ns, *args[4:15], mode, hint), C)
+        if dense3:
+            check(self.L.dbn_igemm_set_dense3(1), 'igemm_set_dense3')
+        check(self.L.dbn_conv_bn_t(at, srcp, *args[1:], accumulate, hint, self.ns, *bnargs, self.stream), what)
         return sc, sh
 
     def conv_bn(self, name, x, conv, out_name, bn_name, bn, train, version=None, x_act=None):
@@ -642,14 +658,15 @@
             sc, sh = self._winograd_conv(name, x, conv, y, bn, bn_name, x_act=x_act)
             return y, sc, sh
         assert x_act is None, name
-        wpk = self.pack(name, conv.weight, 0, version=version, cs=C)
+        dense = version is None and self.plan(conv, x.shape, train, fp32_tensors=x.dtype == torch.float32).stem_dense
+        wpk = self._dense3_panel(name, conv.weight) if dense else self.pack(name, conv.weight, 0, version=version, cs=C)
         y = self.buf(out_name, N, Ho, Wo, conv.cout)
         if self.prof:
             self._prof_igemm(N * Ho * Wo, conv.cout, 2.0 * N * Ho * Wo * conv.cout * conv.cin * k * k, 'fwd ' + name, 0,
-                             (N, H, W, C, Ho, Wo, k, s, p))
+                             (N, H, W, C, Ho, Wo, k, s, p), dense3=dense)
         sc, sh = self._conv_bn_call('conv+bn ' + name, bn_name, bn, y,
                                     (x.data_ptr(), wpk.data_ptr(), _p(conv.bias), y.data_ptr(), N, H, W, C, Ho, Wo, conv.cout, k, k,
-                                     s, p, 0), 0, s)
+                                     s, p, 0), 0, s, dense3=dense)
         if self.prof:
             self.prof.end()
         return y, sc, sh
@@ -714,7 +731,11 @@
         else:
             self._prof_igemm(N * 4 * H * W, Co, flops, 'convT fwd ' + name, 2)
 
-    def _prof_igemm(self, M, Cd, flops, tag='', mode=0, geom=None, epi=0):
+    def _prof_igemm(self, M, Cd, flops, tag='', mode=0, geom=None, epi=0, dense3=False):
+        if dense3:
+            N, Hs, Ws, Cs, Hd, Wd = geom[:6]
+            self.prof.begin(IGEMM_TILE_NAMES[2] % (4, 0, 0, 'false', 0, 'false'), flops, 4.0 * N * (Hs * Ws * Cs + Hd * Wd * Cd), tag)
+            return
         cfg = self.L.dbn_igemm_tile_config_ns(M, Cd, self.ns)
         at = 3 if self._use_planes else self.at
         if geom is not None and mode < 2:
diff --git a/include/dbnet_hip.h b/include/dbnet_hip.h
--- a/include/dbnet_hip.h
+++ b/include/dbnet_hip.h
@@ -259,6 +259,9 @@
 
 long dbn_igemm_panel_floats_t(int kind, int O, int I, int R, int S, int mode, int stride, int cs);
 int dbn_pack_weights_t(int kind, const float* w_oihw, int O, int I, int R, int S, int mode, int stride, int cs, float* out, void* stream);
+long dbn_igemm_dense3_panel_floats(int O, int R, int S);
+int dbn_pack_weights_dense3(const float* w_oihw, int O, int I, int R, int S, float* out, void* stream);
+int dbn_igemm_set_dense3(int on);
 
 int dbn_igemm_t(int at, int ns, const void* src, const float* wpk, const float* bias, void* dst, int N, int Hs, int Ws, int Cs, int Hd,
                 int Wd, int Cd, int R, int S, int stride, int pad, int mode, int accumulate, int tile_hint, int ksplit, float* slab,
```

Result: no change. 749.4 (median of 6 runs) (+0.6%).
